# dhruvmetha/rapid-locomotion-rl

Measured on AMD Instinct MI355X. Metric: env-steps/sec, 4096 Mini Cheetah envs, 1/2/4/8 MI355X; PPO iters/sec, higher is better.
Workload: dtype f32; 1 GPU; 4096 Mini Cheetah envs flat terrain (4096 per GPU), PPO teacher policy (BASELINE configs[1]); envs_per_gpu=4096, global_envs=4096, global_batch_env_steps_per_iter=98304, parallelism=dp1, world_size=1, policy=ActorCritic 42/18/630->12, random init; teacher PPO + student adaptation update

## Files before the change

rapid-locomotion-rl_amd/csrc/lrl_gemm.h:

```cpp
#pragma once
#include <stdint.h>

#ifdef __HIPCC__
#define LRL_GHD __host__ __device__
#else
#define LRL_GHD
#endif

namespace lrl {

enum GemmEpi : int {
  EPI_STORE = 0,
  EPI_BIAS = 1,
  EPI_BIAS_ELU = 2,
  EPI_DELU = 3,
  EPI_PARTIAL = 4,
  EPI_BIAS_TANH = 5,
  EPI_DTANH = 6,
};

struct GemmP {
  const float* A;
  const float* B;
  float* C;
  const float* bias;
  const float* aux;
  const int64_t* a_rows;
  const int64_t* b_rows;
  float* bias_part;
  int M, N, K;
  int splits, kps;
  int avec, bvec;
  int groups;
  int64_t lda, ldb, ldc, ld_aux;
  int64_t ga, gb, gc, gbias, gaux;
  int64_t part_stride;
  const uint16_t* bpl;
  int64_t bpl_ld, bpl_ps, gbp;
};

struct PlaneJob {
  const float* W;
  int64_t ldw, gsrc;
  int rows, cols, trans, groups;
  uint16_t* dst;
};
constexpr int MAX_PLANE_JOBS = 8;
LRL_GHD inline int plane_kp(const PlaneJob& j) { return ((j.trans ? j.rows : j.cols) + 15) / 16 * 16; }
LRL_GHD inline int plane_n(const PlaneJob& j) { return j.trans ? j.cols : j.rows; }
LRL_GHD inline int64_t plane_elems(const PlaneJob& j) { return 3ll * j.groups * plane_n(j) * plane_kp(j); }
int x6_planes_launch(const PlaneJob* jobs, int n, void* stream);
bool gemm_x6p_enabled();
inline void gemm_use_planes(GemmP& p, const PlaneJob& j) {
  p.bpl = j.dst;
  p.bpl_ld = plane_kp(j);
  p.gbp = (int64_t)plane_n(j) * plane_kp(j);
  p.bpl_ps = p.gbp * j.groups;
}

enum GemmLayout : int { GEMM_NT = 0, GEMM_NN = 2, GEMM_TN = 3 };

int gemm_launch(const GemmP& p, int layout, int epi, int groups, void* stream);

struct GemmJob {
  GemmP p;
  int layout, epi, groups;
};
constexpr int MAX_MULTI_JOBS = 3;
int gemm_launch_multi(const GemmJob* jobs, int n, void* stream);

enum GemmFamily : int {
  FAM_NONE = 0, FAM_X6P = 1, FAM_X6T = 2, FAM_X6 = 3, FAM_X6D = 4, FAM_GLDS = 5, FAM_GLDS32 = 6, FAM_GLDS_TN = 7,
  FAM_THIN16 = 8, FAM_THIN32 = 9, FAM_STAGED = 10,
};
constexpr int gemm_path_id(int family, int bm, int bn, bool interior) {
  return family | (bm << 8) | (bn << 16) | (interior ? 1 << 24 : 0);
}
int gemm_last_path();

int gemm_pick_splits(int M, int N, int K, int groups);

}
```

rapid-locomotion-rl_amd/csrc/lrl_gemm.hip:

```cpp
#include <hip/hip_runtime.h>
#include <math.h>
#include <stdint.h>

#include <algorithm>
#include <tuple>
#include <type_traits>
#include <cstdio>
#include <cstdlib>

#include "../../include/lrl.h"
#include "lrl_gemm.h"

namespace lrl {

typedef float f32x16 __attribute__((ext_vector_type(16)));

#ifndef LRL_GBK
#define LRL_GBK 16
#endif
constexpr int GBK = LRL_GBK;
constexpr int KQ = GBK / 4;
constexpr int GTHREADS = 256;

static int g_path_off = 0;
static int path_off() { return __atomic_load_n(&g_path_off, __ATOMIC_RELAXED); }
static int env_switch(const char* name, int dflt) {
  const char* e = getenv(name);
  return e && e[0] >= '0' && e[0] <= '9' ? e[0] - '0' : dflt;
}

static thread_local int g_last_path = 0;
static inline void note_path(int family, int bm, int bn, bool interior = false) {
  g_last_path = gemm_path_id(family, bm, bn, interior);
}

template <int BM, int BN, int LAYOUT>
struct GemmTile {
  static constexpr bool AMC = (LAYOUT & 1) != 0;
  static constexpr bool BNC = (LAYOUT & 2) != 0;
  static constexpr int PK = GBK == 32 ? 1 : 2;
  static constexpr int PA = AMC ? 4 : PK;
  static constexpr int PB = BNC ? 4 : PK;
  static constexpr int IA = BM * GBK / 4, IB = BN * GBK / 4;
  static constexpr int NA = (IA + GTHREADS - 1) / GTHREADS;
  static constexpr int NB = (IB + GTHREADS - 1) / GTHREADS;
  static constexpr int WN = (BM >= 64 && BN >= 64) ? 2 : (BM == 32 ? 4 : 1);
  static constexpr int WM = 4 / WN;
  static constexpr int TM = BM / (32 * WM);
  static constexpr int TN = BN / (32 * WN);
  static_assert(TM >= 1 && TN >= 1, "tile shape");
};

static int tn_shape_tag(int M, int N, int groups) {
  if (M == 256 && N == 512) return 1;
  if (M == 128 && N == 256) return groups > 1 ? 2 : 6;
  if (M == 512 && N <= 64) return 3;
  if (M == 256 && N >= 600) return 4;
  if (M == 256 && N <= 64) return 5;
  return 0;
}

__device__ __forceinline__ float elu_f(float x) { return x > 0.f ? x : expm1f(x); }
__device__ __forceinline__ float tanh_f(float x) { return tanhf(x); }
__host__ __device__ constexpr bool epi_bias(int e) { return e == EPI_BIAS || e == EPI_BIAS_ELU || e == EPI_BIAS_TANH; }
__host__ __device__ constexpr bool epi_aux(int e) { return e == EPI_DELU || e == EPI_DTANH; }
template <int EPI>
__device__ __forceinline__ float epi_apply(float v, float bj, float x) {
  if constexpr (EPI == EPI_BIAS) return v + bj;
  else if constexpr (EPI == EPI_BIAS_ELU) return elu_f(v + bj);
  else if constexpr (EPI == EPI_BIAS_TANH) return tanh_f(v + bj);
  else if constexpr (EPI == EPI_DELU) return x > 0.f ? v : v * (x + 1.f);
  else if constexpr (EPI == EPI_DTANH) return v * (1.f - x * x);
  else return v;
}

template <int V>
using Int = std::integral_constant<int, V>;
template <int... V>
struct Ints {};
template <int... V, class F>
static int with_int(int v, Ints<V...>, F&& f) {
  int rc = LRL_E_INVALID;
  (void)((v == V && ((rc = f(Int<V>{})), true)) || ...);
  return rc;
}
template <int LAYOUT, bool STAGED>
struct Offered;
template <bool STAGED>
struct Offered<GEMM_NT, STAGED> { using epis = Ints<EPI_STORE, EPI_BIAS, EPI_BIAS_ELU, EPI_BIAS_TANH>; };
template <>
struct Offered<GEMM_NN, false> { using epis = Ints<EPI_STORE, EPI_DELU, EPI_DTANH>; };
template <>
struct Offered<GEMM_NN, true> { using epis = Ints<EPI_STORE, EPI_DELU, EPI_DTANH, EPI_PARTIAL>; };
template <bool STAGED>
struct Offered<GEMM_TN, STAGED> { using epis = Ints<EPI_PARTIAL>; };
using BatchMajor = Ints<GEMM_NT, GEMM_NN>;
using AnyLayout = Ints<GEMM_NT, GEMM_NN, GEMM_TN>;
template <bool STAGED = false, int... LAYOUTS, class F>
static int with_pair(int layout, int epi, Ints<LAYOUTS...> layouts, F&& f) {
  return with_int(layout, layouts, [&](auto L) {
    return with_int(epi, typename Offered<decltype(L)::value, STAGED>::epis{}, [&](auto E) { return f(L, E); });
  });
}

__device__ __forceinline__ float4 load4(const float* __restrict__ src, int vec) {
  if (vec == 4) return *reinterpret_cast<const float4*>(src);
  if (vec == 2) {
    const float2 a = reinterpret_cast<const float2*>(src)[0], b = reinterpret_cast<const float2*>(src)[1];
    return make_float4(a.x, a.y, b.x, b.y);
  }
  return make_float4(src[0], src[1], src[2], src[3]);
}

template <int R, int NI, bool RCONTIG>
struct Stager {
  static constexpr int ITEMS = R * GBK / 4;
  const float* rowp[NI];
  const float* P;
  const int64_t* rows;
  int64_t ld;
  int vec, r0, R_lim;

  __device__ __forceinline__ void init(const float* P_, int64_t ld_, const int64_t* rows_, int vec_, int r0_,
                                       int R_lim_) {
    P = P_; ld = ld_; rows = rows_; vec = vec_; r0 = r0_; R_lim = R_lim_;
    if (!RCONTIG) {
#pragma unroll
      for (int u = 0; u < NI; ++u) {
        const int i = threadIdx.x + u * GTHREADS;
        const int gr = r0 + i / KQ;
        rowp[u] = nullptr;
        if ((ITEMS % GTHREADS == 0 || i < ITEMS) && gr < R_lim)
          rowp[u] = P + (rows ? rows[gr] : (int64_t)gr) * ld + 4 * (i % KQ);
      }
    }
  }

  __device__ __forceinline__ void load(float4 (&reg)[NI], int k0, int k_lim) const {
#pragma unroll
    for (int u = 0; u < NI; ++u) {
      const int i = threadIdx.x + u * GTHREADS;
      float4 v = make_float4(0.f, 0.f, 0.f, 0.f);
      if (!RCONTIG) {
        const int k = k0 + 4 * (i % KQ);
        if (rowp[u]) {
          const float* src = rowp[u] + k0;
          if (k + 3 < k_lim) {
            v = load4(src, vec);
          } else {
            if (k + 0 < k_lim) v.x = src[0];
            if (k + 1 < k_lim) v.y = src[1];
            if (k + 2 < k_lim) v.z = src[2];
          }
        }
      } else if (ITEMS % GTHREADS == 0 || i < ITEMS) {
        const int r = 4 * (i % (R / 4)), k = k0 + i / (R / 4);
        const int gr = r0 + r;
        if (k < k_lim) {
          const int64_t row = rows ? rows[k] : (int64_t)k;
          const float* src = P + row * ld + gr;
          if (gr + 3 < R_lim) {
            v = load4(src, vec);
          } else {
            if (gr + 0 < R_lim) v.x = src[0];
            if (gr + 1 < R_lim) v.y = src[1];
            if (gr + 2 < R_lim) v.z = src[2];
          }
        }
      }
      reg[u] = v;
    }
  }

  __device__ __forceinline__ void load_fast(float4 (&reg)[NI], int k0) const {
#pragma unroll
    for (int u = 0; u < NI; ++u) {
      const int i = threadIdx.x + u * GTHREADS;
      if (ITEMS % GTHREADS != 0 && i >= ITEMS) continue;
      if (!RCONTIG) {
        reg[u] = *reinterpret_cast<const float4*>(rowp[u] + k0);
      } else {
        const int r = 4 * (i % (R / 4)), k = k0 + i / (R / 4);
        const int64_t row = rows ? rows[k] : (int64_t)k;
        reg[u] = *reinterpret_cast<const float4*>(P + row * ld + r0 + r);
      }
    }
  }
};

template <int R, int PAD, int NI, bool RCONTIG>
__device__ __forceinline__ void stage_store(float (*S)[R + PAD], const float4 (&reg)[NI]) {
  constexpr int ITEMS = R * GBK / 4;
#pragma unroll
  for (int u = 0; u < NI; ++u) {
    const int i = threadIdx.x + u * GTHREADS;
    if (ITEMS % GTHREADS != 0 && i >= ITEMS) {
    } else if (!RCONTIG) {
      const int r = i / KQ, k = 4 * (i % KQ);
      S[k + 0][r] = reg[u].x;
      S[k + 1][r] = reg[u].y;
      S[k + 2][r] = reg[u].z;
      S[k + 3][r] = reg[u].w;
    } else {
      const int r = 4 * (i % (R / 4)), k = i / (R / 4);
      *reinterpret_cast<float4*>(&S[k][r]) = reg[u];
    }
  }
}

template <int BM, int BN, int LAYOUT, int EPI>
__device__ __forceinline__ void gemm_staged_body(const GemmP& p, int vblock, int vgrid, uint8_t* smem) {
  using T = GemmTile<BM, BN, LAYOUT>;
  typedef float AStage[GBK][BM + T::PA];
  typedef float BStage[GBK][BN + T::PB];
  AStage* As = reinterpret_cast<AStage*>(smem);
  BStage* Bs = reinterpret_cast<BStage*>(smem + 2 * sizeof(AStage));
  const int mt = (p.M + BM - 1) / BM, nt = (p.N + BN - 1) / BN;
  int L;
  {
    const int nwg = vgrid, orig = vblock, xcd = orig & 7, q = nwg >> 3, r = nwg & 7;
    L = (xcd < r ? xcd * (q + 1) : r * (q + 1) + (xcd - r) * q) + (orig >> 3);
  }
  const int tn_ = L % nt, tm_ = (L / nt) % mt, zz = L / (nt * mt);
  const int groups = p.groups;
  const int g = zz / p.splits, s = zz - g * p.splits;
  const float* __restrict__ A = p.A + g * p.ga;
  const float* __restrict__ B = p.B + g * p.gb;
  const int m0 = tm_ * BM, n0 = tn_ * BN;
  const int kbeg = s * p.kps;
  const int kend = min(p.K, kbeg + p.kps);
  const int lane = threadIdx.x & 63, w = threadIdx.x >> 6;
  const int li = lane & 31, h = lane >> 5;
  constexpr int TM = T::TM, TN = T::TN;
  const int wm = (w / T::WN) * (BM / T::WM), wn = (w % T::WN) * (BN / T::WN);
  const int64_t* a_rows = T::AMC ? nullptr : p.a_rows;
  const int64_t* b_rows = T::BNC ? p.b_rows : nullptr;

#ifndef LRL_GEMM_SPLITACC
#define LRL_GEMM_SPLITACC 1
#endif
  constexpr int NACC = (LRL_GEMM_SPLITACC && TM * TN == 1) ? 2 : 1;
  f32x16 acc[TM][TN], acc2[TM][TN];
#pragma unroll
  for (int i = 0; i < TM; ++i)
#pragma unroll
    for (int j = 0; j < TN; ++j)
#pragma unroll
      for (int r = 0; r < 16; ++r) acc[i][j][r] = acc2[i][j][r] = 0.f;

  const bool do_bsum = EPI == EPI_PARTIAL && p.bias_part != nullptr && tn_ == 0;
  float bsum = 0.f;

  float4 ra[T::NA], rb[T::NB];
  Stager<BM, T::NA, T::AMC> sa;
  Stager<BN, T::NB, T::BNC> sb;
  sa.init(A, p.lda, a_rows, p.avec, m0, p.M);
  sb.init(B, p.ldb, b_rows, p.bvec, n0, p.N);
  const bool fast = m0 + BM <= p.M && n0 + BN <= p.N && ((kend - kbeg) % GBK) == 0 && p.avec == 4 && p.bvec == 4;
  float xaux[epi_aux(EPI) ? TM : 1][epi_aux(EPI) ? TN : 1][16];
  if constexpr (epi_aux(EPI)) {
    const float* __restrict__ ax = p.aux + g * p.gaux;
#pragma unroll
    for (int j = 0; j < TN; ++j) {
      const int col = min(n0 + wn + 32 * j + li, p.N - 1);
#pragma unroll
      for (int i = 0; i < TM; ++i)
#pragma unroll
        for (int r = 0; r < 16; ++r) {
          const int row = min(m0 + wm + 32 * i + (r & 3) + 8 * (r >> 2) + 4 * h, p.M - 1);
          xaux[i][j][r] = ax[(int64_t)row * p.ld_aux + col];
        }
    }
  }
  int k0 = kbeg;
  if (k0 < kend) {
    if (fast) {
      sa.load_fast(ra, k0);
      sb.load_fast(rb, k0);
    } else {
      sa.load(ra, k0, kend);
      sb.load(rb, k0, kend);
    }
    stage_store<BM, T::PA, T::NA, T::AMC>(As[0], ra);
    stage_store<BN, T::PB, T::NB, T::BNC>(Bs[0], rb);
  }
  __syncthreads();
  int buf = 0;
  for (; k0 < kend; k0 += GBK) {
    const int kn = k0 + GBK;
    if (kn < kend) {
      if (fast) {
        sa.load_fast(ra, kn);
        sb.load_fast(rb, kn);
      } else {
        sa.load(ra, kn, kend);
        sb.load(rb, kn, kend);
      }
    }
    if (do_bsum && threadIdx.x < BM) {
#pragma unroll
      for (int k = 0; k < GBK; ++k) bsum += As[buf][k][threadIdx.x];
    }
    float a[GBK / 2][TM], b[GBK / 2][TN];
#pragma unroll
    for (int kk = 0; kk < GBK / 2; ++kk) {
#pragma unroll
      for (int i = 0; i < TM; ++i) a[kk][i] = As[buf][2 * kk + h][wm + 32 * i + li];
#pragma unroll
      for (int j = 0; j < TN; ++j) b[kk][j] = Bs[buf][2 * kk + h][wn + 32 * j + li];
    }
    __builtin_amdgcn_sched_barrier(0);
    __builtin_amdgcn_s_setprio(1);
#pragma unroll
    for (int kk = 0; kk < GBK / 2; ++kk)
#pragma unroll
      for (int i = 0; i < TM; ++i)
#pragma unroll
        for (int j = 0; j < TN; ++j) {
          if (NACC == 2 && (kk & 1))
            acc2[i][j] = __builtin_amdgcn_mfma_f32_32x32x2f32(a[kk][i], b[kk][j], acc2[i][j], 0, 0, 0);
          else
            acc[i][j] = __builtin_amdgcn_mfma_f32_32x32x2f32(a[kk][i], b[kk][j], acc[i][j], 0, 0, 0);
        }
    __builtin_amdgcn_s_setprio(0);
    __builtin_amdgcn_sched_barrier(0);
    if (kn < kend) {
      stage_store<BM, T::PA, T::NA, T::AMC>(As[buf ^ 1], ra);
      stage_store<BN, T::PB, T::NB, T::BNC>(Bs[buf ^ 1], rb);
    }
    __syncthreads();
    buf ^= 1;
  }

  float* __restrict__ C = p.C + g * p.gc;
  if (EPI == EPI_PARTIAL) C += (int64_t)s * p.part_stride;
  const float* __restrict__ bias = p.bias ? p.bias + g * p.gbias : nullptr;
#pragma unroll
  for (int j = 0; j < TN; ++j) {
    const int col = n0 + wn + 32 * j + li;
    if (col >= p.N) continue;
    float bj = 0.f;
    if (epi_bias(EPI)) bj = bias[col];
#pragma unroll
    for (int i = 0; i < TM; ++i) {
#pragma unroll
      for (int r = 0; r < 16; ++r) {
        const int row = m0 + wm + 32 * i + (r & 3) + 8 * (r >> 2) + 4 * h;
        if (row < p.M) {
          const float v = NACC == 2 ? acc[i][j][r] + acc2[i][j][r] : acc[i][j][r];
          C[(int64_t)row * p.ldc + col] = epi_apply<EPI>(v, bj, epi_aux(EPI) ? xaux[i][j][r] : 0.f);
        }
      }
    }
  }
  if (do_bsum && threadIdx.x < BM && m0 + (int)threadIdx.x < p.M)
    p.bias_part[((int64_t)s * groups + g) * p.M + m0 + threadIdx.x] = bsum;
}
template <int BM, int BN, int LAYOUT, int EPI>
struct StagedBody {
  using T = GemmTile<BM, BN, LAYOUT>;
  static constexpr int LDS = 2 * GBK * (BM + T::PA + BN + T::PB) * (int)sizeof(float);
  static_assert((2 * GBK * (BM + T::PA) * sizeof(float)) % 16 == 0, "B stages 16-B aligned");
  static __device__ __forceinline__ void run(const GemmP& p, int vblock, int vgrid, uint8_t* smem) {
    gemm_staged_body<BM, BN, LAYOUT, EPI>(p, vblock, vgrid, smem);
  }
};
template <int BM, int BN, int LAYOUT, int EPI>
__global__ __launch_bounds__(GTHREADS) void gemm_kernel(GemmP p) {
  using Body = StagedBody<BM, BN, LAYOUT, EPI>;
  __shared__ __attribute__((aligned(16))) uint8_t S[Body::LDS];
  Body::run(p, blockIdx.x, gridDim.x, S);
}

typedef __attribute__((address_space(3))) void* lds_ptr_t;

template <int LAYOUT, int EPI, int BKD>
__global__ __launch_bounds__(GTHREADS) void gemm_glds_kernel(GemmP p) {
// ... 170 lines not shown
#pragma unroll
      for (int s = 0; s < 16; ++s) {
        const float av = (s & 3) == 0 ? cur[s >> 2].x : (s & 3) == 1 ? cur[s >> 2].y : (s & 3) == 2 ? cur[s >> 2].z : cur[s >> 2].w;
        if (s & 1) acc2 = __builtin_amdgcn_mfma_f32_32x32x2f32(av, breg[kb][s], acc2, 0, 0, 0);
        else acc = __builtin_amdgcn_mfma_f32_32x32x2f32(av, breg[kb][s], acc, 0, 0, 0);
      }
#pragma unroll
      for (int v = 0; v < 4; ++v) cur[v] = nxt[v];
    }
    ar = arn;
    if (w > 0) {
#pragma unroll
      for (int r = 0; r < 16; ++r) red[((w - 1) * 16 + r) * 64 + lane] = acc[r] + acc2[r];
    }
    __syncthreads();
    if (w == 0) {
      float bj = 0.f;
      if constexpr (epi_bias(EPI)) bj = colv ? p.bias[g * p.gbias + li] : 0.f;
#pragma unroll
      for (int r = 0; r < 16; ++r) {
        float v = acc[r] + acc2[r];
        v += red[r * 64 + lane];
        v += red[(16 + r) * 64 + lane];
        v += red[(32 + r) * 64 + lane];
        v = epi_apply<EPI>(v, bj, 0.f);
        const int orow = t * 32 + (r & 3) + 8 * (r >> 2) + 4 * h;
        if (colv && orow < M) C[(int64_t)orow * p.ldc + li] = v;
      }
    }
    __syncthreads();
  }
}

typedef float f32x4v __attribute__((ext_vector_type(4)));
template <int LAYOUT, int EPI, int NBK>
__global__ __launch_bounds__(GTHREADS, 2) void gemm_thin16_kernel(GemmP p) {
  __shared__ float red[3 * 8 * 64];
  constexpr bool BNC = (LAYOUT & 2) != 0;
  constexpr int KS = 2 * NBK;
  const int N = p.N, M = p.M;
  const int g = blockIdx.y;
  const float* __restrict__ A = p.A + g * p.ga;
  const float* __restrict__ B = p.B + g * p.gb;
  float* __restrict__ C = p.C + g * p.gc;
  const int lane = threadIdx.x & 63, w = threadIdx.x >> 6, i = lane & 15, h = lane >> 4;
  const int kbeg = w * 32 * NBK;
  float breg[KS][2][4];
#pragma unroll
  for (int s = 0; s < KS; ++s)
#pragma unroll
    for (int cb = 0; cb < 2; ++cb)
#pragma unroll
      for (int u = 0; u < 4; ++u) {
        const int k = kbeg + 16 * s + 4 * h + u, col = i + 16 * cb;
        breg[s][cb][u] = col < N ? (BNC ? B[(int64_t)k * p.ldb + col] : B[(int64_t)col * p.ldb + k]) : 0.f;
      }
  const int mt = (M + 15) >> 4;
  auto rowp = [&](int t) -> const float* {
    const int row = t * 16 + i;
    if (t >= mt || row >= M) return nullptr;
    return A + (p.a_rows ? p.a_rows[row] : (int64_t)row) * p.lda + kbeg + 4 * h;
  };
  auto load = [&](const float* ar, int s0, float4* dst) {
#pragma unroll
    for (int v = 0; v < 4; ++v)
      dst[v] = ar ? *reinterpret_cast<const float4*>(ar + 16 * (s0 + v)) : make_float4(0.f, 0.f, 0.f, 0.f);
  };
  const float* ar = rowp(blockIdx.x);
  float4 cur[4];
  load(ar, 0, cur);
  for (int t = blockIdx.x; t < mt; t += gridDim.x) {
    const float* arn = rowp(t + gridDim.x);
    f32x4v acc0 = {0.f, 0.f, 0.f, 0.f}, acc1 = {0.f, 0.f, 0.f, 0.f};
#pragma unroll
    for (int s0 = 0; s0 < KS; s0 += 4) {
      float4 nxt[4];
      if (s0 + 4 < KS) load(ar, s0 + 4, nxt);
      else load(arn, 0, nxt);
#pragma unroll
      for (int v = 0; v < 4; ++v) {
        const float av[4] = {cur[v].x, cur[v].y, cur[v].z, cur[v].w};
#pragma unroll
        for (int u = 0; u < 4; ++u) {
          acc0 = __builtin_amdgcn_mfma_f32_16x16x4f32(av[u], breg[s0 + v][0][u], acc0, 0, 0, 0);
          acc1 = __builtin_amdgcn_mfma_f32_16x16x4f32(av[u], breg[s0 + v][1][u], acc1, 0, 0, 0);
        }
      }
#pragma unroll
      for (int v = 0; v < 4; ++v) cur[v] = nxt[v];
    }
    ar = arn;
    if (w > 0) {
#pragma unroll
      for (int r = 0; r < 4; ++r) {
        red[((w - 1) * 8 + r) * 64 + lane] = acc0[r];
        red[((w - 1) * 8 + 4 + r) * 64 + lane] = acc1[r];
      }
    }
    __syncthreads();
    if (w == 0) {
#pragma unroll
      for (int cb = 0; cb < 2; ++cb) {
        const int col = i + 16 * cb;
        float bj = 0.f;
        if constexpr (epi_bias(EPI)) bj = col < N ? p.bias[g * p.gbias + col] : 0.f;
#pragma unroll
        for (int r = 0; r < 4; ++r) {
          float v = cb ? acc1[r] : acc0[r];
          v += red[(4 * cb + r) * 64 + lane];
          v += red[(8 + 4 * cb + r) * 64 + lane];
          v += red[(16 + 4 * cb + r) * 64 + lane];
          v = epi_apply<EPI>(v, bj, 0.f);
          const int orow = t * 16 + 4 * h + r;
          if (col < N && orow < M) C[(int64_t)orow * p.ldc + col] = v;
        }
      }
    }
    __syncthreads();
  }
}

static bool thin16_enabled() {
  static const int on = env_switch("LRL_THIN16", 1);
  return on != 0 && !(path_off() & 32);
}

template <int LAYOUT, int EPI, int NBK>
static int launch_thin_k(const GemmP& p, int groups, hipStream_t st) {
  static int ncu = 0;
  if (!ncu) {
    int dev = 0;
    hipDeviceProp_t prop;
    if (hipGetDevice(&dev) != hipSuccess || hipGetDeviceProperties(&prop, dev) != hipSuccess) return LRL_E_HIP;
    ncu = prop.multiProcessorCount;
  }
  if (thin16_enabled()) {
    const int mt = (p.M + 15) / 16;
    const int gx = std::max(1, std::min(mt, 2 * ncu / std::max(1, groups)));
    hipLaunchKernelGGL((gemm_thin16_kernel<LAYOUT, EPI, NBK>), dim3(gx, groups), dim3(GTHREADS), 0, st, p);
    note_path(FAM_THIN16, 16, 32);
    return 0;
  }
  const int mt = (p.M + 31) / 32;
  const int gx = std::max(1, std::min(mt, 2 * ncu / std::max(1, groups)));
  hipLaunchKernelGGL((gemm_thin_kernel<LAYOUT, EPI, NBK>), dim3(gx, groups), dim3(GTHREADS), 0, st, p);
  note_path(FAM_THIN32, 32, 32);
  return 0;
}
template <int LAYOUT, int EPI>
static int launch_thin(const GemmP& p, int groups, hipStream_t st) {
  switch (p.K / 128) {
    case 4: return launch_thin_k<LAYOUT, EPI, 4>(p, groups, st);
    case 8: return launch_thin_k<LAYOUT, EPI, 8>(p, groups, st);
  }
  return LRL_E_INVALID;
}

template <int NST, int BN, int SHAPE>
__global__ __launch_bounds__(GTHREADS, 2) void gemm_glds_tn_kernel(GemmP p) {
  constexpr int BM = 128, BKD = 16, IMGA = BKD * BM, IMGB = BKD * BN, TN = BN / 64;
  constexpr int NB_DMA = IMGB / 256;
  extern __shared__ __attribute__((aligned(16))) float S[];
  const int mt = p.M / BM, nt = (p.N + BN - 1) / BN;
  int L;
  {
    const int nwg = gridDim.x, orig = blockIdx.x, xcd = orig & 7, q = nwg >> 3, r = nwg & 7;
    L = (xcd < r ? xcd * (q + 1) : r * (q + 1) + (xcd - r) * q) + (orig >> 3);
  }
  const int tn_ = L % nt, tm_ = (L / nt) % mt, zz = L / (nt * mt);
  const int g = zz / p.splits, sp = zz - g * p.splits;
  const int m0 = tm_ * BM, n0 = tn_ * BN;
  const int kbeg = sp * p.kps, kend = min(p.K, kbeg + p.kps);
  const int ns = (kend - kbeg) / BKD;
  const float* __restrict__ A = p.A + g * p.ga;
  const float* __restrict__ B = p.B + g * p.gb;
  const int lane = threadIdx.x & 63;
  const int w = __builtin_amdgcn_readfirstlane(threadIdx.x >> 6);
  const int li = lane & 31, h = lane >> 5;
  const int wm = (w >> 1) * 64, wn = (w & 1) * (BN / 2);
  constexpr int STG = IMGA + IMGB;
  int* rows = reinterpret_cast<int*>(S + NST * STG);
  if (p.b_rows) {
    for (int i = threadIdx.x; i < kend - kbeg; i += GTHREADS) rows[i] = (int)p.b_rows[kbeg + i];
    __syncthreads();
  }
  const uint32_t s_lds = (uint32_t)(uintptr_t)(lds_ptr_t)S;
  auto dma = [&](const float* src, uint32_t lds_off) {
    uint32_t keep;
    asm volatile("s_mov_b32 %0, m0\n\ts_mov_b32 m0, %2\n\ts_nop 0\n\tglobal_load_lds_dwordx4 %1, off\n\ts_mov_b32 m0, %0"
                 : "=&s"(keep)
                 : "v"(src), "s"(lds_off)
                 : "memory");
  };
  auto issue = [&](int st, int s) {
    const int kl = s * BKD;
    const uint32_t sbase = s_lds + (uint32_t)(st * STG * 4);
#pragma unroll
    for (int i = 0; i < 2; ++i) {
      const int d = 4 * i + w, kr = kl + 2 * d + h;
      dma(A + (int64_t)(kbeg + kr) * p.lda + m0 + 4 * li, __builtin_amdgcn_readfirstlane(sbase + d * 1024));
    }
#pragma unroll
    for (int i = 0; i < NB_DMA / 4; ++i) {
      constexpr int CPR = BN / 4;
      const int d = 4 * i + w, kr = kl + d * (64 / CPR) + lane / CPR;
      const int64_t brow = p.b_rows ? (int64_t)rows[kr] : (int64_t)(kbeg + kr);
      dma(B + brow * p.ldb + n0 + 4 * (lane % CPR), __builtin_amdgcn_readfirstlane(sbase + IMGA * 4 + d * 1024));
    }
  };
  const bool do_bsum = p.bias_part != nullptr && tn_ == 0;
  float bsum = 0.f;
  f32x16 acc[2][TN];
#pragma unroll
  for (int a = 0; a < 2; ++a)
#pragma unroll
    for (int c = 0; c < TN; ++c)
#pragma unroll
      for (int r = 0; r < 16; ++r) acc[a][c][r] = 0.f;
  static_assert(NST == 3, "the counted waits below assume a 3-deep ring");
  if (ns > 0) issue(0, 0);
  if (ns > 1) issue(1, 1);
  for (int s = 0; s < ns; ++s) {
    if (s + 1 < ns) {
      if constexpr (NB_DMA == 8) asm volatile("s_waitcnt vmcnt(4)" ::: "memory");
      else asm volatile("s_waitcnt vmcnt(3)" ::: "memory");
    } else {
      asm volatile("s_waitcnt vmcnt(0)" ::: "memory");
    }
    __builtin_amdgcn_s_barrier();
    if (s + 2 < ns) issue((s + 2) % NST, s + 2);
    const float* As = S + (s % NST) * STG;
    const float* Bs = As + IMGA;
    if (do_bsum && threadIdx.x < BM) {
#pragma unroll
      for (int k = 0; k < BKD; ++k) bsum += As[k * BM + threadIdx.x];
    }
    float av[8][2], bv[8][TN];
#pragma unroll
    for (int t = 0; t < 8; ++t) {
#pragma unroll
      for (int a = 0; a < 2; ++a) av[t][a] = As[(2 * t + h) * BM + wm + 32 * a + li];
#pragma unroll
      for (int c = 0; c < TN; ++c) bv[t][c] = Bs[(2 * t + h) * BN + wn + 32 * c + li];
    }
    asm volatile("s_waitcnt lgkmcnt(0)" ::: "memory");
    __builtin_amdgcn_sched_barrier(0);
    __builtin_amdgcn_s_setprio(1);
#pragma unroll
    for (int t = 0; t < 8; ++t)
#pragma unroll
      for (int a = 0; a < 2; ++a)
#pragma unroll
        for (int c = 0; c < TN; ++c)
          acc[a][c] = __builtin_amdgcn_mfma_f32_32x32x2f32(av[t][a], bv[t][c], acc[a][c], 0, 0, 0);
    __builtin_amdgcn_s_setprio(0);
    __builtin_amdgcn_sched_barrier(0);
  }
  float* __restrict__ C = p.C + g * p.gc + (int64_t)sp * p.part_stride;
#pragma unroll
  for (int c = 0; c < TN; ++c) {
    const int col = n0 + wn + 32 * c + li;
    if (col >= p.N) continue;
#pragma unroll
    for (int a = 0; a < 2; ++a)
#pragma unroll
      for (int r = 0; r < 16; ++r) {
        const int row = m0 + wm + 32 * a + (r & 3) + 8 * (r >> 2) + 4 * h;
        C[(int64_t)row * p.ldc + col] = acc[a][c][r];
      }
  }
  if (do_bsum && threadIdx.x < BM)
    p.bias_part[((int64_t)sp * p.groups + g) * p.M + m0 + threadIdx.x] = bsum;
}

template <int BN, int SHAPE>
static int launch_glds_tn_tag(const GemmP& p, int groups, hipStream_t st) {
  const size_t lds = (size_t)3 * 16 * (128 + BN) * sizeof(float) + (p.b_rows ? (size_t)p.kps * sizeof(int) : 0);
  static bool attr = false;
  if (!attr) {
    if (hipFuncSetAttribute(reinterpret_cast<const void*>(&gemm_glds_tn_kernel<3, BN, SHAPE>),
                            hipFuncAttributeMaxDynamicSharedMemorySize, 160 * 1024) != hipSuccess)
      return LRL_E_HIP;
    attr = true;
  }
  dim3 gt((p.M / 128) * ((p.N + BN - 1) / BN) * groups * p.splits);
  hipLaunchKernelGGL((gemm_glds_tn_kernel<3, BN, SHAPE>), gt, dim3(GTHREADS), lds, st, p);
  note_path(FAM_GLDS_TN, 128, BN);
  return hipGetLastError() == hipSuccess ? 0 : LRL_E_HIP;
}

template <int BN>
static int launch_glds_tn(const GemmP& p, int groups, hipStream_t st) {
  switch (tn_shape_tag(p.M, p.N, groups)) {
    case 1: return launch_glds_tn_tag<BN, 1>(p, groups, st);
    case 2: return launch_glds_tn_tag<BN, 2>(p, groups, st);
    case 3: return launch_glds_tn_tag<BN, 3>(p, groups, st);
    case 4: return launch_glds_tn_tag<BN, 4>(p, groups, st);
    case 5: return launch_glds_tn_tag<BN, 5>(p, groups, st);
    case 6: return launch_glds_tn_tag<BN, 6>(p, groups, st);
    default: return launch_glds_tn_tag<BN, 0>(p, groups, st);
  }
}

constexpr int XBK = 16;
#ifndef LRL_X6_PIPE
#define LRL_X6_PIPE 1
#endif
#ifndef LRL_X6_PIPE_VALU
#define LRL_X6_PIPE_VALU 4
#endif

__device__ __forceinline__ uint32_t x6_hi_pair(uint32_t u0, uint32_t u1) {
  return __builtin_amdgcn_perm(u1, u0, 0x07060302u);
}
__device__ __forceinline__ void x6_split2(float x0, float x1, uint32_t& h, uint32_t& m, uint32_t& l) {
  uint32_t u0 = __float_as_uint(x0), u1 = __float_as_uint(x1);
  h = x6_hi_pair(u0, u1);
  float r0 = x0 - __uint_as_float(u0 & 0xffff0000u), r1 = x1 - __uint_as_float(u1 & 0xffff0000u);
  u0 = __float_as_uint(r0);
  u1 = __float_as_uint(r1);
  m = x6_hi_pair(u0, u1);
  r0 = r0 - __uint_as_float(u0 & 0xffff0000u);
  r1 = r1 - __uint_as_float(u1 & 0xffff0000u);
  l = x6_hi_pair(__float_as_uint(r0), __float_as_uint(r1));
}
__device__ __forceinline__ int x6_off(int r, int c) { return r * XBK + 8 * (c ^ ((r >> 3) & 1)); }

typedef short bf16x8_t __attribute__((ext_vector_type(8)));

__device__ __forceinline__ f32x16 x6_mma(const bf16x8_t (&a)[3], const bf16x8_t (&b)[3], f32x16 c) {
  c = __builtin_amdgcn_mfma_f32_32x32x16_bf16(a[2], b[0], c, 0, 0, 0);
  c = __builtin_amdgcn_mfma_f32_32x32x16_bf16(a[1], b[1], c, 0, 0, 0);
  c = __builtin_amdgcn_mfma_f32_32x32x16_bf16(a[0], b[2], c, 0, 0, 0);
  c = __builtin_amdgcn_mfma_f32_32x32x16_bf16(a[1], b[0], c, 0, 0, 0);
  c = __builtin_amdgcn_mfma_f32_32x32x16_bf16(a[0], b[1], c, 0, 0, 0);
  c = __builtin_amdgcn_mfma_f32_32x32x16_bf16(a[0], b[0], c, 0, 0, 0);
  return c;
}

template <int R, bool KC, bool KGATHER = false>
struct X6Op {
  static constexpr int PLANE = R * XBK;
  static constexpr int NI = KC ? R / 64 : 1;
  static constexpr int KR = KC ? 4 : R / 16;
  static constexpr int NV = KC ? 4 * NI : KR;
  const float* rowp[NI];
  const float* P;
  const int64_t* krows;
  int64_t ld;
  int ldi, roff;
  int rr, kb;
  bool rok;
  bool vec4;

  __device__ __forceinline__ void init(const float* P_, int64_t ld_, const int64_t* rows, const int64_t* krows_,
                                       int r0, int R_lim, bool vec4_ = true) {
    P = P_; ld = ld_; krows = krows_; vec4 = vec4_;
    const int t = threadIdx.x;
    if (KC) {
#pragma unroll
      for (int u = 0; u < NI; ++u) {
        const int r = (t >> 2) + 64 * u, gr = r0 + r;
        rowp[u] = gr < R_lim ? P_ + (rows ? rows[gr] : (int64_t)gr) * ld_ + 4 * (t & 3) : nullptr;
      }
    } else {
      rr = t % R;
      kb = __builtin_amdgcn_readfirstlane(KR * (t / R));
      rok = r0 + rr < R_lim;
      ldi = (int)ld_;
      roff = r0 + rr;
    }
  }
  __device__ __forceinline__ void load(float (&v)[NV], int k0, int k_lim, bool fast) const {
    if (KC) {
#pragma unroll
      for (int u = 0; u < NI; ++u) {
        const int k = k0 + 4 * (threadIdx.x & 3);
        float4 q = make_float4(0.f, 0.f, 0.f, 0.f);
        if (fast) {
          q = *reinterpret_cast<const float4*>(rowp[u] + k0);
        } else if (rowp[u]) {
          const float* s = rowp[u] + k0;
          if (k + 3 < k_lim && vec4) {
            q = *reinterpret_cast<const float4*>(s);
          } else if (k + 3 < k_lim) {
            q = make_float4(s[0], s[1], s[2], s[3]);
          } else {
            if (k + 0 < k_lim) q.x = s[0];
            if (k + 1 < k_lim) q.y = s[1];
            if (k + 2 < k_lim) q.z = s[2];
          }
        }
        v[4 * u] = q.x; v[4 * u + 1] = q.y; v[4 * u + 2] = q.z; v[4 * u + 3] = q.w;
      }
    } else {
#pragma unroll
      for (int e = 0; e < KR; ++e) {
        const int k = k0 + kb + e;
        if constexpr (KGATHER) {
          const int64_t o = krows[k] * ld + roff;
          if (fast) v[e] = P[o];
          else v[e] = (rok && k < k_lim) ? P[o] : 0.f;
        } else if (fast) {
          v[e] = P[k * ldi + roff];
        } else {
          v[e] = (rok && k < k_lim) ? P[k * ldi + roff] : 0.f;
        }
      }
    }
  }
  __device__ __forceinline__ void store(const float (&v)[NV], uint16_t* img) const {
    const int t = threadIdx.x;
    if (KC) {
#pragma unroll
      for (int u = 0; u < NI; ++u) {
        const int r = (t >> 2) + 64 * u, j = t & 3;
        uint32_t h0, m0, l0, h1, m1, l1;
        x6_split2(v[4 * u], v[4 * u + 1], h0, m0, l0);
        x6_split2(v[4 * u + 2], v[4 * u + 3], h1, m1, l1);
        const int off = x6_off(r, j >> 1) + 4 * (j & 1);
        *reinterpret_cast<uint2*>(img + off) = make_uint2(h0, h1);
        *reinterpret_cast<uint2*>(img + PLANE + off) = make_uint2(m0, m1);
        *reinterpret_cast<uint2*>(img + 2 * PLANE + off) = make_uint2(l0, l1);
      }
    } else if (KR == 8) {
      uint32_t h[4], m[4], l[4];
#pragma unroll
      for (int e = 0; e < 4; ++e) x6_split2(v[2 * e], v[2 * e + 1], h[e], m[e], l[e]);
      const int off = x6_off(rr, kb >> 3);
      *reinterpret_cast<uint4*>(img + off) = make_uint4(h[0], h[1], h[2], h[3]);
      *reinterpret_cast<uint4*>(img + PLANE + off) = make_uint4(m[0], m[1], m[2], m[3]);
      *reinterpret_cast<uint4*>(img + 2 * PLANE + off) = make_uint4(l[0], l[1], l[2], l[3]);
    } else {
      uint32_t h[2], m[2], l[2];
#pragma unroll
      for (int e = 0; e < 2; ++e) x6_split2(v[2 * e], v[2 * e + 1], h[e], m[e], l[e]);
      const int off = x6_off(rr, kb >> 3) + (kb & 4);
      *reinterpret_cast<uint2*>(img + off) = make_uint2(h[0], h[1]);
      *reinterpret_cast<uint2*>(img + PLANE + off) = make_uint2(m[0], m[1]);
      *reinterpret_cast<uint2*>(img + 2 * PLANE + off) = make_uint2(l[0], l[1]);
    }
  }
  __device__ __forceinline__ static float vsum(const float (&v)[NV]) {
    float s = 0.f;
#pragma unroll
    for (int e = 0; e < NV; ++e) s += v[e];
    return s;
  }
};

template <int BM, int BN, int LAYOUT, int EPI, bool FAST, bool BGATHER>
__device__ __forceinline__ void gemm_x6_body(const GemmP& p, int vblock, int vgrid, uint8_t* smem) {
  constexpr bool AKC = (LAYOUT & 1) == 0, BKC = (LAYOUT & 2) == 0;
  constexpr int PA = BM * XBK, PB = BN * XBK, STG = 3 * (PA + PB);
  constexpr int TM = BM / 64, TN = BN / 64;
  uint16_t* S = reinterpret_cast<uint16_t*>(smem);
  const int mt = (p.M + BM - 1) / BM, nt = (p.N + BN - 1) / BN;
  int L;
  {
    const int nwg = vgrid, orig = vblock, xcd = orig & 7, q = nwg >> 3, r = nwg & 7;
    L = (xcd < r ? xcd * (q + 1) : r * (q + 1) + (xcd - r) * q) + (orig >> 3);
  }
  const int tn_ = L % nt, tm_ = (L / nt) % mt, zz = L / (nt * mt);
  const int g = zz / p.splits, sp = zz - g * p.splits;
  const int m0 = tm_ * BM, n0 = tn_ * BN;
  const int kbeg = sp * p.kps, kend = min(p.K, kbeg + p.kps);
  const int lane = threadIdx.x & 63, w = threadIdx.x >> 6, li = lane & 31, h = lane >> 5;
  const int wm = (w >> 1) * (BM / 2), wn = (w & 1) * (BN / 2);
  X6Op<BM, AKC> oa;
  X6Op<BN, BKC, BGATHER && !BKC> ob;
  oa.init(p.A + g * p.ga, p.lda, AKC ? p.a_rows : nullptr, nullptr, m0, p.M, p.avec == 4);
  ob.init(p.B + g * p.gb, p.ldb, nullptr, BKC ? nullptr : p.b_rows, n0, p.N, p.bvec == 4);
  constexpr bool fast = FAST;
  const bool do_bsum = EPI == EPI_PARTIAL && p.bias_part != nullptr && tn_ == 0;
  float bsum = 0.f;
  f32x16 acc[TM][TN];
#pragma unroll
  for (int i = 0; i < TM; ++i)
#pragma unroll
    for (int j = 0; j < TN; ++j)
#pragma unroll
      for (int r = 0; r < 16; ++r) acc[i][j][r] = 0.f;
  using OA = decltype(oa);
  using OB = decltype(ob);
  auto compute = [&](const uint16_t* As) {
    const uint16_t* Bs = As + 3 * PA;
    bf16x8_t a[TM][3], b[TN][3];
#pragma unroll
    for (int i = 0; i < TM; ++i)
#pragma unroll
      for (int pl = 0; pl < 3; ++pl)
        a[i][pl] = *reinterpret_cast<const bf16x8_t*>(As + pl * PA + x6_off(wm + 32 * i + li, h));
#pragma unroll
    for (int j = 0; j < TN; ++j)
#pragma unroll
      for (int pl = 0; pl < 3; ++pl)
        b[j][pl] = *reinterpret_cast<const bf16x8_t*>(Bs + pl * PB + x6_off(wn + 32 * j + li, h));
#pragma unroll
    for (int i = 0; i < TM; ++i)
#pragma unroll
      for (int j = 0; j < TN; ++j) acc[i][j] = x6_mma(a[i], b[j], acc[i][j]);
  };
  if constexpr (LRL_X6_PIPE && FAST) {
  float va[2][OA::NV], vb[2][OB::NV];
  const int ns = (kend - kbeg + XBK - 1) / XBK;
  if (ns > 0) {
    oa.load(va[0], kbeg, kend, fast);
    ob.load(vb[0], kbeg, kend, fast);
    if (ns > 1) {
      oa.load(va[1], kbeg + XBK, kend, fast);
      ob.load(vb[1], kbeg + XBK, kend, fast);
    }
    if (do_bsum) bsum += OA::vsum(va[0]);
    oa.store(va[0], S);
    ob.store(vb[0], S + 3 * PA);
    if (ns > 2) {
      oa.load(va[0], kbeg + 2 * XBK, kend, fast);
      ob.load(vb[0], kbeg + 2 * XBK, kend, fast);
    }
  }
  __syncthreads();
  auto step = [&](int s, auto par, auto full) {
    constexpr int P = decltype(par)::value;
    constexpr bool F = decltype(full)::value;
    compute(S + P * STG);
    if (F || s + 1 < ns) {
      if (do_bsum) bsum += OA::vsum(va[P ^ 1]);
      oa.store(va[P ^ 1], S + (P ^ 1) * STG);
      ob.store(vb[P ^ 1], S + (P ^ 1) * STG + 3 * PA);
    }
    if (F || s + 3 < ns) {
      oa.load(va[P ^ 1], kbeg + (s + 3) * XBK, kend, fast);
      ob.load(vb[P ^ 1], kbeg + (s + 3) * XBK, kend, fast);
    }
    if constexpr (F) {
      constexpr int NMF = TM * TN * 6;
      __builtin_amdgcn_sched_group_barrier(0x100, 3 * (TM + TN), 0);
#pragma unroll
      for (int q = 0; q < NMF; ++q) {
        __builtin_amdgcn_sched_group_barrier(0x008, 1, 0);
        __builtin_amdgcn_sched_group_barrier(0x002, LRL_X6_PIPE_VALU, 0);
      }
    }
    __syncthreads();
  };
  using I0 = std::integral_constant<int, 0>;
  using I1 = std::integral_constant<int, 1>;
  using BT = std::integral_constant<bool, true>;
  using BF = std::integral_constant<bool, false>;
  int s = 0;
  for (; s + 4 < ns; s += 2) {
    step(s, I0{}, BT{});
    step(s + 1, I1{}, BT{});
  }
  for (; s < ns; s += 2) {
    step(s, I0{}, BF{});
    if (s + 1 < ns) step(s + 1, I1{}, BF{});
  }
  } else {
  float va[OA::NV], vb[OB::NV];
  if (kbeg < kend) {
    oa.load(va, kbeg, kend, fast);
    ob.load(vb, kbeg, kend, fast);
    if (do_bsum) bsum += OA::vsum(va);
    oa.store(va, S);
    ob.store(vb, S + 3 * PA);
  }
  __syncthreads();
  int buf = 0;
  for (int k0 = kbeg; k0 < kend; k0 += XBK) {
    const bool more = k0 + XBK < kend;
    if (more) {
      oa.load(va, k0 + XBK, kend, fast);
      ob.load(vb, k0 + XBK, kend, fast);
    }
    compute(S + buf * STG);
    if (more) {
      if (do_bsum) bsum += OA::vsum(va);
      oa.store(va, S + (buf ^ 1) * STG);
      ob.store(vb, S + (buf ^ 1) * STG + 3 * PA);
    }
    __syncthreads();
    buf ^= 1;
  }
  }

  float* __restrict__ C = p.C + g * p.gc;
  if (EPI == EPI_PARTIAL) C += (int64_t)sp * p.part_stride;
  const float* __restrict__ bias = p.bias ? p.bias + g * p.gbias : nullptr;
  const float* __restrict__ ax = epi_aux(EPI) ? p.aux + g * p.gaux : nullptr;
#pragma unroll
  for (int j = 0; j < TN; ++j) {
    const int col = n0 + wn + 32 * j + li;
    if (!FAST && col >= p.N) continue;
    float bj = 0.f;
    if (epi_bias(EPI)) bj = bias[col];
#pragma unroll
    for (int i = 0; i < TM; ++i)
#pragma unroll
      for (int q = 0; q < 4; ++q) {
        const int row0 = m0 + wm + 32 * i + 8 * q + 4 * h;
        const int ldc = (int)p.ldc, ldx = (int)p.ld_aux;
        float* __restrict__ crow = C + (int64_t)row0 * p.ldc + col;
        float xa[4];
        if constexpr (epi_aux(EPI)) {
          const float* __restrict__ xrow = ax + (int64_t)row0 * p.ld_aux + col;
#pragma unroll
          for (int r = 0; r < 4; ++r) xa[r] = (FAST || row0 + r < p.M) ? xrow[r * ldx] : 0.f;
        }
#pragma unroll
        for (int r = 0; r < 4; ++r) {
          if (FAST || row0 + r < p.M) crow[r * ldc] = epi_apply<EPI>(acc[i][j][4 * q + r], bj, epi_aux(EPI) ? xa[r] : 0.f);
        }
        asm volatile("" ::: "memory");
      }
  }
  if constexpr (EPI == EPI_PARTIAL && !AKC) {
    if (do_bsum) {
      float* red = reinterpret_cast<float*>(S);
      red[threadIdx.x] = bsum;
      __syncthreads();
      if (threadIdx.x < BM && m0 + (int)threadIdx.x < p.M) {
        float s = 0.f;
#pragma unroll
        for (int q = 0; q < GTHREADS / BM; ++q) s += red[q * BM + threadIdx.x];
        p.bias_part[((int64_t)sp * p.groups + g) * p.M + m0 + threadIdx.x] = s;
      }
    }
  }
}
template <int BM, int BN, int LAYOUT, int EPI, bool FAST, bool BGATHER>
struct X6Body {
  static constexpr int LDS = 2 * 3 * (BM + BN) * XBK * (int)sizeof(uint16_t);
  static __device__ __forceinline__ void run(const GemmP& p, int vblock, int vgrid, uint8_t* smem) {
    gemm_x6_body<BM, BN, LAYOUT, EPI, FAST, BGATHER>(p, vblock, vgrid, smem);
  }
};
template <int BM, int BN, int LAYOUT, int EPI, bool FAST, bool BGATHER, int TAG = 0>
__global__ __launch_bounds__(GTHREADS, 3) void gemm_x6_kernel(GemmP p) {
  using Body = X6Body<BM, BN, LAYOUT, EPI, FAST, BGATHER>;
  __shared__ __attribute__((aligned(16))) uint8_t S[Body::LDS];
  Body::run(p, blockIdx.x, gridDim.x, S);
}

static bool x6_interior(const GemmP& p, int layout, int bm, int bn) {
  const bool akc = (layout & 1) == 0, bkc = (layout & 2) == 0;
  return p.M % bm == 0 && p.N % bn == 0 && p.K % XBK == 0 && p.kps % XBK == 0 && (!akc || p.avec == 4) &&
         (!bkc || p.bvec == 4);
}
template <int BM, int BN>
static int launch_x6_tile(const GemmP& p, int layout, int epi, int groups, hipStream_t st) {
  dim3 grid(((p.M + BM - 1) / BM) * ((p.N + BN - 1) / BN) * groups * p.splits);
  const bool interior = x6_interior(p, layout, BM, BN);
  const bool bg = p.b_rows != nullptr;
  if (layout == GEMM_TN) {
    auto tn = [&](auto F, auto G, auto T) {
      hipLaunchKernelGGL((gemm_x6_kernel<BM, BN, GEMM_TN, EPI_PARTIAL, F(), G(), T()>), grid, dim3(GTHREADS), 0, st, p);
    };
    const std::true_type yes;
    const std::false_type no;
    const int tag = (BM == 128 && BN == 128 && interior) ? tn_shape_tag(p.M, p.N, groups) : 0;
    if (tag == 1) tn(yes, no, Int<1>{});
    else if (tag == 2) tn(yes, no, Int<2>{});
    else if (tag == 4 && bg) tn(yes, yes, Int<4>{});
    else if (tag == 4) tn(yes, no, Int<4>{});
    else if (tag == 6) tn(yes, no, Int<6>{});
    else if (interior && bg) tn(yes, yes, Int<0>{});
    else if (interior) tn(yes, no, Int<0>{});
    else if (bg) tn(no, yes, Int<0>{});
    else tn(no, no, Int<0>{});
  } else {
    const int rc = with_pair(layout, epi, BatchMajor{}, [&](auto L, auto E) {
      if (interior) hipLaunchKernelGGL((gemm_x6_kernel<BM, BN, L(), E(), true, false>), grid, dim3(GTHREADS), 0, st, p);
      else hipLaunchKernelGGL((gemm_x6_kernel<BM, BN, L(), E(), false, false>), grid, dim3(GTHREADS), 0, st, p);
      return 0;
    });
    if (rc) return rc;
  }
  note_path(FAM_X6, BM, BN, interior);
  return hipGetLastError() == hipSuccess ? 0 : LRL_E_HIP;
}

static bool x6_enabled() {
  static const int on = env_switch("LRL_GEMM_X6", 1);
  return on != 0 && !(path_off() & 16);
}

static int try_x6d(const GemmP& p, int layout, int epi, int groups, int bm, int bn, hipStream_t st);
static bool x6d_fits(const GemmP& p, int layout, int bm, int bn);

static bool x6_tile(const GemmP& p, int layout, int epi, int groups, int& bm, int& bn) {
  if (!x6_enabled()) return false;
  static const int min_side = getenv("LRL_X6_MIN") ? atoi(getenv("LRL_X6_MIN")) : 16;
  if (p.N < min_side || (layout == GEMM_TN && p.M < min_side)) return false;
  const int64_t lim = int64_t(1) << 31;
  if ((layout & 1) && (int64_t)p.K * p.lda >= lim) return false;
  if ((layout & 2) && p.b_rows == nullptr && (int64_t)p.K * p.ldb >= lim) return false;
  if ((int64_t)p.M * p.ldc >= lim || (epi_aux(epi) && (int64_t)p.M * p.ld_aux >= lim)) return false;
  if (layout == GEMM_TN) {
    if (epi != EPI_PARTIAL || p.M < 16 || p.N < 16 || p.kps % XBK) return false;
    bm = p.M <= 64 ? 64 : 128;
    bn = p.N <= 64 ? 64 : 128;
    return true;
  }
  if (p.splits != 1 || p.N < 16 || p.M < 64 || epi == EPI_PARTIAL) return false;
  if (p.K < 32) return false;
  if (p.N <= 32 && p.K % 128 == 0 && (p.K / 128 == 4 || p.K / 128 == 8) && p.avec == 4 && p.M >= 256) return false;
  static const int small_wg = getenv("LRL_X6_SMALL_WG") ? atoi(getenv("LRL_X6_SMALL_WG")) : 1024;
  bn = p.N > 64 ? 128 : 64;
  if (bn == 128 && (int64_t)((p.M + 63) / 64) * ((p.N + 127) / 128) * groups < small_wg) bn = 64;
  const int64_t wg128 = (int64_t)((p.M + 127) / 128) * ((p.N + bn - 1) / bn) * groups;
  bm = wg128 >= 512 ? 128 : 64;
  return true;
}

static int try_x6(const GemmP& p, int layout, int epi, int groups, hipStream_t st) {
  int bm, bn;
  if (!x6_tile(p, layout, epi, groups, bm, bn)) return 0;
  if (int dr = try_x6d(p, layout, epi, groups, bm, bn, st)) return dr;
  int rc;
  if (bm == 128 && bn == 128) rc = launch_x6_tile<128, 128>(p, layout, epi, groups, st);
  else if (bm == 128) rc = launch_x6_tile<128, 64>(p, layout, epi, groups, st);
  else if (bn == 128) rc = launch_x6_tile<64, 128>(p, layout, epi, groups, st);
  else rc = launch_x6_tile<64, 64>(p, layout, epi, groups, st);
  return rc ? rc : 1;
}

template <int BM, int EPI, bool GATHER>
__global__ __launch_bounds__(GTHREADS, 2) void gemm_x6p_kernel(GemmP p) {
  constexpr int BN = 128, NST = 3, TM = BM / 64, TN = 2;
  constexpr int AIMG = BM * 64, BIMG = BN * 32, STB = AIMG + 3 * BIMG;
  constexpr int NA = BM / 64, NB = 3;
  constexpr int NPW = NA + NB;
  static_assert(NPW == 4 || NPW == 5, "vmcnt table");
  __shared__ __attribute__((aligned(16))) uint8_t S[NST * STB];
  const int mt = p.M / BM, nt = p.N / BN;
  int L;
  {
    const int nwg = gridDim.x, orig = blockIdx.x, xcd = orig & 7, q = nwg >> 3, r = nwg & 7;
    L = (xcd < r ? xcd * (q + 1) : r * (q + 1) + (xcd - r) * q) + (orig >> 3);
  }
  const int tn_ = L % nt, tm_ = (L / nt) % mt, g = L / (nt * mt);
  const int m0 = tm_ * BM, n0 = tn_ * BN;
  const int lane = threadIdx.x & 63;
  const int w = __builtin_amdgcn_readfirstlane(threadIdx.x >> 6);
  const int li = lane & 31, h = lane >> 5;
  const int wm = (w >> 1) * (BM / 2), wn = (w & 1) * (BN / 2);
  const float* __restrict__ A = p.A + g * p.ga;
  const uint16_t* __restrict__ Bp = p.bpl + g * p.gbp;
  const float* asrc[NA];
#pragma unroll
  for (int d = 0; d < NA; ++d) {
    const int r = (w * NA + d) * 16 + (lane >> 2), ch = (lane & 3) ^ ((r >> 2) & 3);
    asrc[d] = A + (GATHER ? p.a_rows[m0 + r] : (int64_t)(m0 + r)) * p.lda + 4 * ch;
  }
  const uint16_t* bsrc[NB];
#pragma unroll
  for (int d = 0; d < NB; ++d) {
    const int j = w * NB + d, r = (j & 3) * 32 + (lane >> 1), ch = (lane & 1) ^ ((r >> 3) & 1);
    bsrc[d] = Bp + (j >> 2) * p.bpl_ps + (int64_t)(n0 + r) * p.bpl_ld + 8 * ch;
  }
  const uint32_t s_lds = (uint32_t)(uintptr_t)(lds_ptr_t)S;
  auto dma = [&](const void* src, uint32_t lds_off) {
    uint32_t keep;
    asm volatile("s_mov_b32 %0, m0\n\ts_mov_b32 m0, %2\n\ts_nop 0\n\tglobal_load_lds_dwordx4 %1, off\n\ts_mov_b32 m0, %0"
                 : "=&s"(keep)
                 : "v"(src), "s"(lds_off)
                 : "memory");
  };
  auto issue = [&](int st, int k0) {
    const uint32_t base = s_lds + (uint32_t)(st * STB);
#pragma unroll
    for (int d = 0; d < NA; ++d) dma(asrc[d] + k0, __builtin_amdgcn_readfirstlane(base + (w * NA + d) * 1024));
#pragma unroll
    for (int d = 0; d < NB; ++d) dma(bsrc[d] + k0, __builtin_amdgcn_readfirstlane(base + AIMG + (w * NB + d) * 1024));
  };

  f32x16 acc[TM][TN];
#pragma unroll
  for (int i = 0; i < TM; ++i)
#pragma unroll
    for (int j = 0; j < TN; ++j)
#pragma unroll
      for (int r = 0; r < 16; ++r) acc[i][j][r] = 0.f;

  const int ns = p.K / 16;
  issue(0, 0);
  if (ns > 1) issue(1, 16);
  for (int s = 0; s < ns; ++s) {
    if (s + 1 < ns) {
      if constexpr (NPW == 5) asm volatile("s_waitcnt vmcnt(5)" ::: "memory");
      else asm volatile("s_waitcnt vmcnt(4)" ::: "memory");
    } else {
      asm volatile("s_waitcnt vmcnt(0)" ::: "memory");
    }
    __builtin_amdgcn_s_barrier();
    if (s + 2 < ns) issue((s + 2) % NST, (s + 2) * 16);
    const uint8_t* As = S + (s % NST) * STB;
    const uint8_t* Bs = As + AIMG;
    bf16x8_t a[TM][3], b[TN][3];
#pragma unroll
    for (int j = 0; j < TN; ++j) {
      const int r = wn + 32 * j + li, off = r * 32 + 16 * (h ^ ((r >> 3) & 1));
#pragma unroll
      for (int pl = 0; pl < 3; ++pl) b[j][pl] = *reinterpret_cast<const bf16x8_t*>(Bs + pl * BIMG + off);
    }
#pragma unroll
    for (int i = 0; i < TM; ++i) {
      const int r = wm + 32 * i + li, sw = (r >> 2) & 3;
      const float4 x0 = *reinterpret_cast<const float4*>(As + r * 64 + 16 * ((2 * h) ^ sw));
      const float4 x1 = *reinterpret_cast<const float4*>(As + r * 64 + 16 * ((2 * h + 1) ^ sw));
      uint32_t hh[4], mm[4], ll[4];
      x6_split2(x0.x, x0.y, hh[0], mm[0], ll[0]);
      x6_split2(x0.z, x0.w, hh[1], mm[1], ll[1]);
      x6_split2(x1.x, x1.y, hh[2], mm[2], ll[2]);
      x6_split2(x1.z, x1.w, hh[3], mm[3], ll[3]);
      uint4 vh = make_uint4(hh[0], hh[1], hh[2], hh[3]), vm = make_uint4(mm[0], mm[1], mm[2], mm[3]),
            vl = make_uint4(ll[0], ll[1], ll[2], ll[3]);
      a[i][0] = *reinterpret_cast<bf16x8_t*>(&vh);
      a[i][1] = *reinterpret_cast<bf16x8_t*>(&vm);
      a[i][2] = *reinterpret_cast<bf16x8_t*>(&vl);
    }
#pragma unroll
    for (int i = 0; i < TM; ++i)
#pragma unroll
      for (int j = 0; j < TN; ++j) acc[i][j] = x6_mma(a[i], b[j], acc[i][j]);
  }

  float* __restrict__ C = p.C + g * p.gc;
  const float* __restrict__ bias = p.bias ? p.bias + g * p.gbias : nullptr;
  const float* __restrict__ ax = epi_aux(EPI) ? p.aux + g * p.gaux : nullptr;
#pragma unroll
  for (int j = 0; j < TN; ++j) {
    const int col = n0 + wn + 32 * j + li;
    float bj = 0.f;
    if (epi_bias(EPI)) bj = bias[col];
#pragma unroll
    for (int i = 0; i < TM; ++i)
#pragma unroll
      for (int q = 0; q < 4; ++q) {
        const int row0 = m0 + wm + 32 * i + 8 * q + 4 * h;
        float* __restrict__ crow = C + (int64_t)row0 * p.ldc + col;
        float xa[4];
        if constexpr (epi_aux(EPI)) {
          const float* __restrict__ xrow = ax + (int64_t)row0 * p.ld_aux + col;
#pragma unroll
          for (int r = 0; r < 4; ++r) xa[r] = xrow[r * p.ld_aux];
        }
#pragma unroll
        for (int r = 0; r < 4; ++r) crow[r * p.ldc] = epi_apply<EPI>(acc[i][j][4 * q + r], bj, epi_aux(EPI) ? xa[r] : 0.f);
      }
  }
}

constexpr int X6T_MAX_GATHER_KPS = 1024;
template <int BN, bool BGATHER>
__device__ __forceinline__ void gemm_x6t_body(const GemmP& p, int vblock, int vgrid, uint8_t* S) {
  constexpr int BM = 128, NST = 3, TM = 2, TN = BN / 64;
  constexpr int IMG = 16 * 128 * 4, STB = IMG + 16 * BN * 4;
  constexpr int NAP = IMG / 1024, NBP = BN / 16;
  constexpr int NPW = (NAP + NBP) / 4;
  constexpr int KPP = 256 / BN;
  const int mt = p.M / BM, nt = (p.N + BN - 1) / BN;
  int L;
  {
    const int nwg = vgrid, orig = vblock, xcd = orig & 7, q = nwg >> 3, r = nwg & 7;
    L = (xcd < r ? xcd * (q + 1) : r * (q + 1) + (xcd - r) * q) + (orig >> 3);
  }
  const int tn_ = L % nt, tm_ = (L / nt) % mt, zz = L / (nt * mt);
  const int g = zz / p.splits, sp = zz - g * p.splits;
  const int m0 = tm_ * BM, n0 = tn_ * BN;
  const int kbeg = sp * p.kps, kend = min(p.K, kbeg + p.kps);
  const int lane = threadIdx.x & 63;
  const int w = __builtin_amdgcn_readfirstlane(threadIdx.x >> 6);
  const int li = lane & 31, h = lane >> 5;
  const int wm = (w >> 1) * (BM / 2), wn = (w & 1) * (BN / 2);
  const float* __restrict__ A = p.A + g * p.ga;
  const float* __restrict__ Bm = p.B + g * p.gb;
  const float* src[NPW];
  int64_t kstep[NPW];
  int bkr[NPW];
  int* xrows = reinterpret_cast<int*>(S + NST * STB);
  if constexpr (BGATHER) {
    for (int t = threadIdx.x; t < kend - kbeg; t += GTHREADS) xrows[t] = (int)p.b_rows[kbeg + t];
    __syncthreads();
  }
#pragma unroll
  for (int d = 0; d < NPW; ++d) {
    const int j = NPW * w + d;
    if (j < NAP) {
      const int kr = 2 * j + (lane >> 5), ch = (lane & 31) ^ (8 * ((kr >> 3) & 1));
      src[d] = A + (int64_t)(kbeg + kr) * p.lda + m0 + 4 * ch;
      kstep[d] = (int64_t)16 * p.lda;
      bkr[d] = -1;
    } else {
      const int kr = KPP * (j - NAP) + lane / (BN / 4), ch = (lane % (BN / 4)) ^ (8 * ((kr >> 3) & 1));
      src[d] = BGATHER ? Bm + n0 + 4 * ch : Bm + (int64_t)(kbeg + kr) * p.ldb + n0 + 4 * ch;
      kstep[d] = (int64_t)16 * p.ldb;
      bkr[d] = kr;
    }
  }
  const uint32_t s_lds = (uint32_t)(uintptr_t)(lds_ptr_t)S;
  auto dma = [&](const void* src, uint32_t lds_off) {
    uint32_t keep;
    asm volatile("s_mov_b32 %0, m0\n\ts_mov_b32 m0, %2\n\ts_nop 0\n\tglobal_load_lds_dwordx4 %1, off\n\ts_mov_b32 m0, %0"
                 : "=&s"(keep)
                 : "v"(src), "s"(lds_off)
                 : "memory");
  };
  auto issue = [&](int st, int s) {
    const uint32_t base = s_lds + (uint32_t)(st * STB);
#pragma unroll
    for (int d = 0; d < NPW; ++d) {
      const float* sr = (BGATHER && bkr[d] >= 0) ? src[d] + (int64_t)xrows[16 * s + bkr[d]] * p.ldb : src[d] + s * kstep[d];
      dma(sr, __builtin_amdgcn_readfirstlane(base + (NPW * w + d) * 1024));
    }
  };
  const bool do_bsum = p.bias_part != nullptr && tn_ == 0 && wn == 0;
  float bsum[TM] = {0.f, 0.f};
  f32x16 acc[TM][TN];
#pragma unroll
  for (int i = 0; i < TM; ++i)
#pragma unroll
    for (int j = 0; j < TN; ++j)
#pragma unroll
      for (int r = 0; r < 16; ++r) acc[i][j][r] = 0.f;

  const int ns = (kend - kbeg) / 16;
  if (ns > 0) issue(0, 0);
  if (ns > 1) issue(1, 1);
  const int sw = 32 * h;
  static_assert(NPW == 3 || NPW == 4, "vmcnt below");
  for (int s = 0; s < ns; ++s) {
    if (s + 1 < ns) {
      if constexpr (NPW == 4) asm volatile("s_waitcnt vmcnt(4)" ::: "memory");
      else asm volatile("s_waitcnt vmcnt(3)" ::: "memory");
    } else {
      asm volatile("s_waitcnt vmcnt(0)" ::: "memory");
    }
    __builtin_amdgcn_s_barrier();
    if (s + 2 < ns) issue((s + 2) % NST, s + 2);
    const float* As = reinterpret_cast<const float*>(S + (s % NST) * STB);
    const float* Bs = As + IMG / 4;
    bf16x8_t a[TM][3], b[TN][3];
    auto gather_split = [&](const float* img, int pitch, int r, bf16x8_t (&o)[3], float* vs) {
      const float* p0 = img + 8 * h * pitch + (r ^ sw);
      float v[8];
#pragma unroll
      for (int t = 0; t < 8; ++t) v[t] = p0[pitch * t];
      if (vs) {
        float s8 = 0.f;
#pragma unroll
        for (int t = 0; t < 8; ++t) s8 += v[t];
        *vs += s8;
      }
      uint32_t hh[4], mm[4], ll[4];
#pragma unroll
      for (int e = 0; e < 4; ++e) x6_split2(v[2 * e], v[2 * e + 1], hh[e], mm[e], ll[e]);
      uint4 vh = make_uint4(hh[0], hh[1], hh[2], hh[3]), vm = make_uint4(mm[0], mm[1], mm[2], mm[3]),
            vl = make_uint4(ll[0], ll[1], ll[2], ll[3]);
      o[0] = *reinterpret_cast<bf16x8_t*>(&vh);
      o[1] = *reinterpret_cast<bf16x8_t*>(&vm);
      o[2] = *reinterpret_cast<bf16x8_t*>(&vl);
    };
#pragma unroll
    for (int i = 0; i < TM; ++i) gather_split(As, 128, wm + 32 * i + li, a[i], do_bsum ? &bsum[i] : nullptr);
#pragma unroll
    for (int j = 0; j < TN; ++j) gather_split(Bs, BN, wn + 32 * j + li, b[j], nullptr);
#pragma unroll
    for (int i = 0; i < TM; ++i)
#pragma unroll
      for (int j = 0; j < TN; ++j) acc[i][j] = x6_mma(a[i], b[j], acc[i][j]);
  }

  float* __restrict__ C = p.C + g * p.gc + (int64_t)sp * p.part_stride;
#pragma unroll
  for (int j = 0; j < TN; ++j) {
    const int col = n0 + wn + 32 * j + li;
    if (col >= p.N) continue;
#pragma unroll
    for (int i = 0; i < TM; ++i)
#pragma unroll
      for (int q = 0; q < 4; ++q) {
        const int row0 = m0 + wm + 32 * i + 8 * q + 4 * h;
        float* __restrict__ crow = C + (int64_t)row0 * p.ldc + col;
#pragma unroll
        for (int r = 0; r < 4; ++r) crow[r * p.ldc] = acc[i][j][4 * q + r];
      }
  }
  if (p.bias_part != nullptr && tn_ == 0) {
    __syncthreads();
    float* red = reinterpret_cast<float*>(S);
    if (wn == 0) {
#pragma unroll
      for (int i = 0; i < TM; ++i) red[h * BM + wm + 32 * i + li] = bsum[i];
    }
    __syncthreads();
    if (threadIdx.x < BM) {
      float s = 0.f;
      s += red[threadIdx.x];
      s += red[BM + threadIdx.x];
      p.bias_part[((int64_t)sp * p.groups + g) * p.M + m0 + threadIdx.x] = s;
    }
  }
}
template <int BN, bool BGATHER>
struct X6tBody {
  static constexpr int LDS = 3 * (16 * 128 * 4 + 16 * BN * 4) + (BGATHER ? 4 * X6T_MAX_GATHER_KPS : 0);
// ... 565 lines not shown
```

rapid-locomotion-rl_amd/csrc/lrl_ppo.hip:

```cpp
#include <hip/hip_runtime.h>
#include <math.h>
#include <stdint.h>
#include <stdlib.h>
#include <string.h>

#include <algorithm>
#include <initializer_list>
#include <mutex>
#include <vector>

#include "../../include/lrl.h"
#include "../../include/lrl_philox.h"
#include "lrl_gemm.h"
#include "lrl_launch.h"

namespace lrl {

constexpr float LOG_SQRT_2PI = 0.91893853320467274178f;
constexpr int HEAD_ROWS = 32;
constexpr int HEAD_THREADS = 256;
constexpr int HEAD_W = 128;
constexpr int MAX_ACT = 16;
constexpr int HEAD_NA = 12;
constexpr int MAX_LAT = 32;

__device__ __forceinline__ float delu(float h) { return h > 0.f ? 1.f : h + 1.f; }

constexpr int PREP_R = 4;
__global__ void ppo_prep_kernel(const float* __restrict__ obs, const int64_t* __restrict__ rows, int B, int no,
                                int xs, float* __restrict__ X) {
  const int64_t i = (int64_t)blockIdx.x * blockDim.x + threadIdx.x;
  const int64_t ng = ((int64_t)B + PREP_R - 1) / PREP_R;
  if (i >= ng * xs) return;
  const int g = (int)(i / xs), c = (int)(i - (int64_t)g * xs);
  int64_t src[PREP_R];
  float v[PREP_R];
#pragma unroll
  for (int u = 0; u < PREP_R; ++u) {
    const int b = g * PREP_R + u;
    src[u] = b < B ? (rows ? rows[b] : (int64_t)b) : -1;
  }
#pragma unroll
  for (int u = 0; u < PREP_R; ++u) v[u] = (c < no && src[u] >= 0) ? obs[src[u] * no + c] : 0.f;
#pragma unroll
  for (int u = 0; u < PREP_R; ++u) {
    const int b = g * PREP_R + u;
    if (b < B) X[(int64_t)b * xs + c] = v[u];
  }
}

inline unsigned prep_blocks(int64_t rows, int xs) {
  return (unsigned)((((rows + PREP_R - 1) / PREP_R) * xs + 255) / 256);
}

struct HeadArgs {
  const float* h3;
  float* dh3;
  const float *w4a, *b4a, *w4c, *b4c, *stdv;
  const float *actions, *old_mu, *old_sigma, *tv, *ret, *adv, *old_logp;
  const int64_t* rows;
  int B, na;
  float clip, ent_coef, vcoef;
  int clipped_value;
  float* part;
  int part_len;
};

__host__ __device__ constexpr int hp_w4a(int) { return 0; }
__host__ __device__ constexpr int hp_b4a(int na) { return na * HEAD_W; }
__host__ __device__ constexpr int hp_w4c(int na) { return na * HEAD_W + na; }
__host__ __device__ constexpr int hp_b4c(int na) { return na * HEAD_W + na + HEAD_W; }
__host__ __device__ constexpr int hp_std(int na) { return na * HEAD_W + na + HEAD_W + 1; }
__host__ __device__ constexpr int hp_kl(int na) { return na * HEAD_W + na + HEAD_W + 1 + na; }
__host__ __device__ constexpr int hp_len(int na) { return hp_kl(na) + 3; }

template <int NA, bool TANH>
__global__ __launch_bounds__(HEAD_THREADS) void ppo_head_kernel(HeadArgs a) {
  constexpr int HP = 2 * HEAD_W + 4;
  constexpr int NAP = (NA + 3) / 4 * 4;
  static_assert(NA <= 16 && HEAD_W % 16 == 0, "float4 rows");
  constexpr int NG = (HEAD_ROWS * NA + HEAD_THREADS - 1) / HEAD_THREADS;
  __shared__ __attribute__((aligned(16))) float H[HEAD_ROWS][HP];
  __shared__ __attribute__((aligned(16))) float W4[NA + 1][HEAD_W];
  __shared__ float MU[HEAD_ROWS][NA + 1];
  __shared__ float VP[HEAD_ROWS][8];
  __shared__ __attribute__((aligned(16))) float LP[HEAD_ROWS][NAP];
  __shared__ float KT[HEAD_ROWS][NA];
  __shared__ float DR[HEAD_ROWS][2];
  __shared__ float SC[HEAD_ROWS][3];
  __shared__ float SD[3][NA];
  __shared__ float GA[3][HEAD_ROWS][NA];
  __shared__ float GR[4][HEAD_ROWS];
  __shared__ int64_t RW[HEAD_ROWS];
  const int t = threadIdx.x;
  const int r0 = blockIdx.x * HEAD_ROWS;
  const int nrows = min(HEAD_ROWS, a.B - r0);
  if (t < HEAD_ROWS) RW[t] = t < nrows ? a.rows[r0 + t] : a.rows[r0];
  if (t < NA) {
    const float sd = a.stdv[t];
    SD[0][t] = sd;
    SD[1][t] = logf(sd);
    SD[2][t] = 1.f / (sd * sd);
  }
  {
    constexpr int NV = HEAD_ROWS * 2 * HEAD_W / 4 / HEAD_THREADS;
    float4 v[NV];
#pragma unroll
    for (int u = 0; u < NV; ++u) {
      const int i = t + u * HEAD_THREADS, r = i / (HEAD_W / 2), c = 4 * (i % (HEAD_W / 2));
      v[u] = r < nrows ? *reinterpret_cast<const float4*>(a.h3 + (int64_t)(r0 + r) * (2 * HEAD_W) + c)
                       : make_float4(0.f, 0.f, 0.f, 0.f);
    }
#pragma unroll
    for (int u = 0; u < NV; ++u) {
      const int i = t + u * HEAD_THREADS, r = i / (HEAD_W / 2), c = 4 * (i % (HEAD_W / 2));
      *reinterpret_cast<float4*>(&H[r][c]) = v[u];
    }
  }
  for (int i = t; i < (NA + 1) * HEAD_W; i += HEAD_THREADS) {
    const int j = i / HEAD_W, k = i - j * HEAD_W;
    W4[j][k] = j < NA ? a.w4a[j * HEAD_W + k] : a.w4c[k];
  }
  __syncthreads();
  float ga[3][NG], gr = 0.f;
#pragma unroll
  for (int u = 0; u < NG; ++u) {
    const int i = t + u * HEAD_THREADS;
    const int r = i / NA, j = i - r * NA;
    const bool ok = i < HEAD_ROWS * NA;
    const int64_t o = RW[ok ? r : 0] * NA + j;
    ga[0][u] = ok ? a.actions[o] : 0.f;
    ga[1][u] = ok ? a.old_mu[o] : 0.f;
    ga[2][u] = ok ? a.old_sigma[o] : 1.f;
  }
  if (t < 4 * HEAD_ROWS) {
    const int q = t / HEAD_ROWS, r = t - q * HEAD_ROWS;
    const float* src = q == 0 ? a.adv : q == 1 ? a.old_logp : q == 2 ? a.tv : a.ret;
    gr = src[RW[r]];
  }
  {
    const int r = t & (HEAD_ROWS - 1), q = t / HEAD_ROWS;
    const float4* hr = reinterpret_cast<const float4*>(&H[r][0]);
    auto dot4 = [](float s, float4 h, float4 w) {
      s = fmaf(h.x, w.x, s);
      s = fmaf(h.y, w.y, s);
      s = fmaf(h.z, w.z, s);
      return fmaf(h.w, w.w, s);
    };
    for (int j = q; j < NA; j += 8) {
      const float4* wr = reinterpret_cast<const float4*>(&W4[j][0]);
      float s = 0.f;
#pragma unroll 8
      for (int k4 = 0; k4 < HEAD_W / 4; ++k4) s = dot4(s, hr[k4], wr[k4]);
      MU[r][j] = s + a.b4a[j];
    }
    const float4* wv = reinterpret_cast<const float4*>(&W4[NA][q * (HEAD_W / 8)]);
    const float4* hv = hr + (HEAD_W + q * (HEAD_W / 8)) / 4;
    float s = 0.f;
#pragma unroll
    for (int k4 = 0; k4 < HEAD_W / 32; ++k4) s = dot4(s, hv[k4], wv[k4]);
    VP[r][q] = s;
  }
#pragma unroll
  for (int u = 0; u < NG; ++u) {
    const int i = t + u * HEAD_THREADS;
    if (i < HEAD_ROWS * NA) {
      const int r = i / NA, j = i - r * NA;
      GA[0][r][j] = ga[0][u];
      GA[1][r][j] = ga[1][u];
      GA[2][r][j] = ga[2][u];
    }
  }
  if (t < 4 * HEAD_ROWS) GR[t / HEAD_ROWS][t & (HEAD_ROWS - 1)] = gr;
  __syncthreads();
  for (int i = t; i < HEAD_ROWS * NA; i += HEAD_THREADS) {
    const int r = i / NA, j = i - r * NA;
    float lp = 0.f, kt = 0.f, d = 0.f;
    if (r < nrows) {
      const float s = SD[0][j], mu = MU[r][j];
      d = GA[0][r][j] - mu;
      lp = -(d * d) / (2.f * (s * s)) - SD[1][j] - LOG_SQRT_2PI;
      const float so = GA[2][r][j], dm = GA[1][r][j] - mu;
      kt = logf(s / so + 1.e-5f) + (so * so + dm * dm) / (2.f * (s * s)) - 0.5f;
    }
    MU[r][j] = d;
    LP[r][j] = lp;
    KT[r][j] = kt;
  }
  __syncthreads();
  const float invB = 1.f / (float)a.B;
  if (t < HEAD_ROWS) {
    const int r = t;
    float kl = 0.f, surr_loss = 0.f, vloss = 0.f, dv = 0.f, dlogp = 0.f;
    if (r < nrows) {
      const float v = (((VP[r][0] + VP[r][1]) + (VP[r][2] + VP[r][3])) + ((VP[r][4] + VP[r][5]) + (VP[r][6] + VP[r][7]))) +
                      a.b4c[0];
      float logp = 0.f;
#pragma unroll
      for (int j = 0; j < NA; ++j) {
        logp += LP[r][j];
        kl += KT[r][j];
      }
      const float adv = GR[0][r];
      const float ratio = expf(logp - GR[1][r]);
      const float surr = -adv * ratio;
      const float rc = fminf(fmaxf(ratio, 1.f - a.clip), 1.f + a.clip);
      const float surr_c = -adv * rc;
      surr_loss = fmaxf(surr, surr_c);
      const float ga = surr > surr_c ? invB : (surr == surr_c ? 0.5f * invB : 0.f);
      const float gb = surr_c > surr ? invB : (surr == surr_c ? 0.5f * invB : 0.f);
      const bool in_rng = ratio >= 1.f - a.clip && ratio <= 1.f + a.clip;
      const float dratio = -adv * ga + (in_rng ? -adv * gb : 0.f);
      dlogp = dratio * ratio;
      const float tv = GR[2][r], ret = GR[3][r];
      const float gv = a.vcoef * invB;
      if (a.clipped_value) {
        const float dvt = v - tv;
        const float vc = tv + fminf(fmaxf(dvt, -a.clip), a.clip);
        const float l1 = (v - ret) * (v - ret), l2 = (vc - ret) * (vc - ret);
        vloss = fmaxf(l1, l2);
        const float g1 = l1 > l2 ? gv : (l1 == l2 ? 0.5f * gv : 0.f);
        const float g2 = l2 > l1 ? gv : (l1 == l2 ? 0.5f * gv : 0.f);
        const bool vin = dvt >= -a.clip && dvt <= a.clip;
        dv = g1 * 2.f * (v - ret) + (vin ? g2 * 2.f * (vc - ret) : 0.f);
      } else {
        vloss = (ret - v) * (ret - v);
        dv = gv * 2.f * (v - ret);
      }
    }
    DR[r][0] = dlogp;
    DR[r][1] = dv;
    SC[r][0] = kl;
    SC[r][1] = surr_loss;
    SC[r][2] = vloss;
  }
  __syncthreads();
  for (int i = t; i < HEAD_ROWS * NA; i += HEAD_THREADS) {
    const int r = i / NA, j = i - r * NA;
    float dm = 0.f, ds = 0.f;
    if (r < nrows) {
      const float d = MU[r][j], dl = DR[r][0], s = SD[0][j], ivar = SD[2][j];
      dm = dl * (d * ivar);
      ds = dl * (d * d * ivar - 1.f) / s - a.ent_coef * invB / s;
    }
    LP[r][j] = dm;
    KT[r][j] = ds;
  }
  __syncthreads();
  float* P = a.part + (int64_t)blockIdx.x * a.part_len;
  {
    const int k = t;
    if (k < HEAD_W) {
      float wk[NA], accw[NA];
#pragma unroll
      for (int j = 0; j < NA; ++j) {
        wk[j] = W4[j][k];
        accw[j] = 0.f;
      }
#pragma unroll 2
      for (int r = 0; r < nrows; ++r) {
        const float h = H[r][k];
        float dmr[NAP];
#pragma unroll
        for (int j4 = 0; j4 < NAP / 4; ++j4) {
          const float4 v = reinterpret_cast<const float4*>(&LP[r][0])[j4];
          dmr[4 * j4] = v.x; dmr[4 * j4 + 1] = v.y; dmr[4 * j4 + 2] = v.z; dmr[4 * j4 + 3] = v.w;
        }
        float s = 0.f;
#pragma unroll
        for (int j = 0; j < NA; ++j) {
          const float dm = dmr[j];
          s = fmaf(dm, wk[j], s);
          accw[j] = fmaf(dm, h, accw[j]);
        }
        a.dh3[(int64_t)(r0 + r) * (2 * HEAD_W) + k] = s * (TANH ? 1.f - h * h : delu(h));
      }
#pragma unroll
      for (int j = 0; j < NA; ++j) P[hp_w4a(NA) + j * HEAD_W + k] = accw[j];
    } else {
      const int kk = k - HEAD_W;
      const float wk = W4[NA][kk];
      float accc = 0.f;
      for (int r = 0; r < nrows; ++r) {
        const float h = H[r][k];
        const float d = DR[r][1];
        accc = fmaf(d, h, accc);
        a.dh3[(int64_t)(r0 + r) * (2 * HEAD_W) + k] = (d * wk) * (TANH ? 1.f - h * h : delu(h));
      }
      P[hp_w4c(NA) + kk] = accc;
    }
  }
  if (t < NA) {
    float sb = 0.f, ss = 0.f;
    for (int r = 0; r < nrows; ++r) {
      sb += LP[r][t];
      ss += KT[r][t];
    }
    P[hp_b4a(NA) + t] = sb;
    P[hp_std(NA) + t] = ss;
  } else if (t == 16) {
    float sb = 0.f;
    for (int r = 0; r < nrows; ++r) sb += DR[r][1];
    P[hp_b4c(NA)] = sb;
  } else if (t >= 32 && t < 35) {
    const int c = t - 32;
    float s = 0.f;
    for (int r = 0; r < nrows; ++r) s += SC[r][c];
    P[hp_kl(NA) + c] = s;
  }
}

struct ActHeadArgs {
  const float* h3;
  const float *w4a, *b4a, *w4c, *b4c, *stdv;
  const float *obs, *priv, *hist, *eps;
  int n, na, no, np;
  uint64_t seed, counter;
  int64_t row_offset;
  float *actions, *mu, *values, *logp;
  lrl_rollout_store store;
  int store_row, do_store;
  float* xa_out;
};

__device__ __forceinline__ void copy_rows(const float* __restrict__ src, int64_t sld, float* __restrict__ dst,
                                          int64_t dld, int nrows, int cols, int t) {
  if (((((uintptr_t)src | (uintptr_t)dst) & 7) == 0) && (((sld | dld | cols) & 1) == 0)) {
    const int c2 = cols / 2, n = nrows * c2;
    for (int i0 = t; i0 < n; i0 += 8 * HEAD_THREADS) {
      float2 v[8];
#pragma unroll
      for (int u = 0; u < 8; ++u) {
        const int i = i0 + u * HEAD_THREADS, r = i / c2, c = i - r * c2;
        if (i < n) v[u] = reinterpret_cast<const float2*>(src + r * sld)[c];
      }
#pragma unroll
      for (int u = 0; u < 8; ++u) {
        const int i = i0 + u * HEAD_THREADS, r = i / c2, c = i - r * c2;
        if (i < n) reinterpret_cast<float2*>(dst + r * dld)[c] = v[u];
      }
    }
  } else {
    const int n = nrows * cols;
    for (int i0 = t; i0 < n; i0 += 8 * HEAD_THREADS) {
      float v[8];
#pragma unroll
      for (int u = 0; u < 8; ++u) {
        const int i = i0 + u * HEAD_THREADS, r = i / cols, c = i - r * cols;
        if (i < n) v[u] = src[r * sld + c];
      }
#pragma unroll
      for (int u = 0; u < 8; ++u) {
        const int i = i0 + u * HEAD_THREADS, r = i / cols, c = i - r * cols;
        if (i < n) dst[r * dld + c] = v[u];
      }
    }
  }
}

constexpr int ACT_ROWS = 16, ACT_Q = HEAD_THREADS / ACT_ROWS;
__global__ __launch_bounds__(HEAD_THREADS) void act_head_kernel(ActHeadArgs a) {
  constexpr int HP = 2 * HEAD_W + 1;
  __shared__ float H[ACT_ROWS][HP];
  __shared__ float W4[MAX_ACT + 1][HEAD_W];
  __shared__ float MU[ACT_ROWS][MAX_ACT + 1];
  __shared__ float VP[ACT_ROWS][ACT_Q];
  const int t = threadIdx.x, na = a.na;
  const int r0 = blockIdx.x * ACT_ROWS;
  const int nrows = min(ACT_ROWS, a.n - r0);
  {
    constexpr int NV = ACT_ROWS * 2 * HEAD_W / 4 / HEAD_THREADS;
    float4 v[NV];
#pragma unroll
    for (int u = 0; u < NV; ++u) {
      const int i = t + u * HEAD_THREADS, r = i / (HEAD_W / 2), c = 4 * (i % (HEAD_W / 2));
      v[u] = r < nrows ? *reinterpret_cast<const float4*>(a.h3 + (int64_t)(r0 + r) * (2 * HEAD_W) + c)
                       : make_float4(0.f, 0.f, 0.f, 0.f);
    }
#pragma unroll
    for (int u = 0; u < NV; ++u) {
      const int i = t + u * HEAD_THREADS, r = i / (HEAD_W / 2), c = 4 * (i % (HEAD_W / 2));
      *reinterpret_cast<float4*>(&H[r][c]) = v[u];
    }
  }
  for (int i = t; i < (na + 1) * HEAD_W; i += HEAD_THREADS) {
    const int j = i / HEAD_W, k = i - j * HEAD_W;
    W4[j][k] = j < na ? a.w4a[j * HEAD_W + k] : a.w4c[k];
  }
  __syncthreads();
  {
    const int r = t & (ACT_ROWS - 1), q = t / ACT_ROWS;
    for (int j = q; j < na; j += ACT_Q) {
      float s = 0.f;
      for (int k = 0; k < HEAD_W; ++k) s = fmaf(H[r][k], W4[j][k], s);
      MU[r][j] = s + a.b4a[j];
    }
    float s = 0.f;
    for (int k = q * (HEAD_W / ACT_Q); k < (q + 1) * (HEAD_W / ACT_Q); ++k) s = fmaf(H[r][HEAD_W + k], W4[na][k], s);
    VP[r][q] = s;
  }
  __syncthreads();
  const int64_t so = (int64_t)a.store_row * a.n;
  for (int i = t; i < nrows * na; i += HEAD_THREADS) {
    const int r = i / na, j = i - r * na, g = r0 + r;
    float e;
    if (a.eps) {
      e = a.eps[(int64_t)g * na + j];
    } else {
      lrl_u32x4 u = lrl_philox((uint32_t)(a.row_offset + g), (uint32_t)a.counter, (LRL_RNG_POLICY << 16) ^ (uint32_t)(a.counter >> 32),
                               (uint32_t)(j >> 1), a.seed);
      const float u1 = fmaxf(lrl_u01(u.v[0]), 1e-7f), u2 = lrl_u01(u.v[1]);
      const float rad = sqrtf(-2.f * logf(u1)), th = 6.283185307179586f * u2;
      e = (j & 1) ? rad * sinf(th) : rad * cosf(th);
    }
    const float m = MU[r][j], sd = a.stdv[j];
    const float act = m + sd * e;
    const float d = act - m;
    MU[r][j] = -(d * d) / (2.f * (sd * sd)) - logf(sd) - LOG_SQRT_2PI;
    a.actions[(int64_t)g * na + j] = act;
    if (a.mu) a.mu[(int64_t)g * na + j] = m;
    if (a.do_store) {
      const int64_t o = (so + g) * na + j;
      a.store.actions[o] = act;
      a.store.mu[o] = m;
      a.store.sigma[o] = sd;
    }
  }
  __syncthreads();
  if (t < nrows) {
    const int g = r0 + t;
    float lp = 0.f;
    for (int j = 0; j < na; ++j) lp += MU[t][j];
    float vs[ACT_Q];
#pragma unroll
    for (int q = 0; q < ACT_Q; ++q) vs[q] = VP[t][q];
#pragma unroll
    for (int w = ACT_Q / 2; w >= 1; w /= 2)
#pragma unroll
      for (int q = 0; q < w; ++q) vs[q] = vs[2 * q] + vs[2 * q + 1];
    const float v = vs[0] + a.b4c[0];
    if (a.values) a.values[g] = v;
    if (a.logp) a.logp[g] = lp;
    if (a.do_store) {
      a.store.values[so + g] = v;
      a.store.logp[so + g] = lp;
    }
  }
  if (a.do_store) {
    const int64_t b = so + r0;
    copy_rows(a.obs + (int64_t)r0 * a.no, a.no, a.store.obs + b * a.no, a.no, nrows, a.no, t);
    if (a.priv)
      copy_rows(a.priv + (int64_t)r0 * a.np, a.np, a.store.priv + b * a.np, a.np, nrows, a.np, t);
    if (a.hist && a.store.hist) {
      const int hd = a.store.hist_dim, ld = a.store.hist_ld > hd ? a.store.hist_ld : hd;
      copy_rows(a.hist + (int64_t)r0 * hd, hd, a.store.hist + b * ld, ld, nrows, hd, t);
    }
  }
}

constexpr int FA_R = 16, FA_THREADS = 256;
constexpr int FA_D = 2;
constexpr int FA_XP = 260;
constexpr int FA_BIGP = 1028;
constexpr int FA_MIDP = 516;
constexpr int FA_HW_FLOATS = (HEAD_NA + 1) * HEAD_W;
constexpr int FA_LDS_FLOATS = FA_R * (FA_XP + FA_BIGP + FA_MIDP) + FA_HW_FLOATS;
constexpr int FA_ENC_MIDP = 260;
constexpr int FA_ENC_LDS_FLOATS = FA_R * (FA_XP + FA_XP + FA_ENC_MIDP);

#ifdef LRL_ACT_PROFILE
__device__ unsigned long long g_act_prof[12];
#define FA_PROF_DECL unsigned long long fa_t = clock64();
#define FA_PROF(i)                                                  \
  if (threadIdx.x == 0) {                                           \
    const unsigned long long t_ = clock64();                        \
    atomicAdd(&g_act_prof[i], t_ - fa_t);                           \
    fa_t = t_;                                                      \
  }
#else
#define FA_PROF_DECL
#define FA_PROF(i)
#endif

typedef float fa_f32x4 __attribute__((ext_vector_type(4)));

struct FaLayer {
  const float* A;
  int pa, ga, K;
  const float* W;
  int ldw, Kw, Nw;
  int64_t gw;
  const float* b;
  float* C;
  int pc, coff, Ng, groups;
  int elu, vec;
};

template <int NB, bool VEC>
__device__ __forceinline__ void fa_tiles(const FaLayer& L, int t0) {
  const int lane = threadIdx.x & 63, i = lane & 15, q = lane >> 4;
  const int tpg = L.Ng >> 4, g = t0 / tpg;
  const float* A = L.A + i * L.pa + g * L.ga + 8 * q;
  const float* W = L.W + g * L.gw;
  const float* rowp[NB];
  bool rok[NB];
#pragma unroll
  for (int j = 0; j < NB; ++j) {
    const int n = (t0 + j - g * tpg) * 16 + i;
    rok[j] = n < L.Nw;
    rowp[j] = W + (int64_t)(rok[j] ? n : L.Nw - 1) * L.ldw;
  }
  fa_f32x4 acc[NB];
#pragma unroll
  for (int j = 0; j < NB; ++j) acc[j] = fa_f32x4{0.f, 0.f, 0.f, 0.f};
  auto load_b = [&](float4 (&bv)[NB][2], int k0) {
    const int k = k0 + 8 * q;
#pragma unroll
    for (int j = 0; j < NB; ++j) {
      if constexpr (VEC) {
        const int k1 = min(k, L.Kw - 4), k2 = min(k + 4, L.Kw - 4);
        float4 v0 = *reinterpret_cast<const float4*>(rowp[j] + k1);
        float4 v1 = *reinterpret_cast<const float4*>(rowp[j] + k2);
        const bool o0 = rok[j] && k < L.Kw, o1 = rok[j] && k + 4 < L.Kw;
        bv[j][0] = o0 ? v0 : make_float4(0.f, 0.f, 0.f, 0.f);
        bv[j][1] = o1 ? v1 : make_float4(0.f, 0.f, 0.f, 0.f);
      } else {
        float v[8];
#pragma unroll
        for (int u = 0; u < 8; ++u) {
          const float x = rowp[j][min(k + u, L.Kw - 1)];
          v[u] = (rok[j] && k + u < L.Kw) ? x : 0.f;
        }
        bv[j][0] = make_float4(v[0], v[1], v[2], v[3]);
        bv[j][1] = make_float4(v[4], v[5], v[6], v[7]);
      }
    }
  };
  const int nck = L.K >> 5;
  float4 ring[FA_D][NB][2];
#pragma unroll
  for (int d = 0; d < FA_D; ++d) load_b(ring[d], 32 * min(d, nck - 1));
  for (int c0 = 0; c0 < nck; c0 += FA_D) {
#pragma unroll
    for (int d = 0; d < FA_D; ++d) {
      const int c = c0 + d;
      if (c < nck) {
        const float4 a0 = *reinterpret_cast<const float4*>(A + 32 * c);
        const float4 a1 = *reinterpret_cast<const float4*>(A + 32 * c + 4);
        const float av[8] = {a0.x, a0.y, a0.z, a0.w, a1.x, a1.y, a1.z, a1.w};
#pragma unroll
        for (int u = 0; u < 8; ++u) {
#pragma unroll
          for (int j = 0; j < NB; ++j) {
            const float4& bq = ring[d][j][u >> 2];
            const float b = (u & 3) == 0 ? bq.x : (u & 3) == 1 ? bq.y : (u & 3) == 2 ? bq.z : bq.w;
            acc[j] = __builtin_amdgcn_mfma_f32_16x16x4f32(av[u], b, acc[j], 0, 0, 0);
          }
        }
        load_b(ring[d], 32 * min(c + FA_D, nck - 1));
      }
    }
  }
#pragma unroll
  for (int j = 0; j < NB; ++j) {
    const int n = (t0 + j - g * tpg) * 16 + i;
    if (n < L.Nw) {
      const float bias = L.b[g * L.Nw + n];
      float* c = L.C + (4 * q) * L.pc + L.coff + g * L.Ng + n;
#pragma unroll
      for (int r = 0; r < 4; ++r) {
        float v = acc[j][r] + bias;
        if (L.elu) v = v > 0.f ? v : expm1f(v);
        c[r * L.pc] = v;
      }
    }
  }
}

template <int NBC, bool VEC>
__device__ __forceinline__ void fa_layer(const FaLayer& L) {
  const int w = threadIdx.x >> 6, T = L.groups * (L.Ng >> 4);
  const int tpw = T >= 4 ? T / 4 : 1;
  if (w * tpw >= T) return;
  const int t0 = w * tpw;
  if constexpr (NBC == 16) {
    fa_tiles<8, VEC>(L, t0);
    fa_tiles<8, VEC>(L, t0 + 8);
  } else if constexpr (NBC > 0) {
    fa_tiles<NBC, VEC>(L, t0);
  } else {
    switch (tpw) {
      case 1: fa_tiles<1, VEC>(L, t0); break;
      case 2: fa_tiles<2, VEC>(L, t0); break;
      case 4: fa_tiles<4, VEC>(L, t0); break;
      case 8: fa_tiles<8, VEC>(L, t0); break;
      case 16: fa_tiles<8, VEC>(L, t0); fa_tiles<8, VEC>(L, t0 + 8); break;
      default:
        for (int t = t0; t < t0 + tpw; ++t) fa_tiles<1, VEC>(L, t);
    }
  }
}

struct FusedActArgs {
  const float* w;
  lrl_ppo_net net;
  const float *obs, *priv, *hist, *eps;
  int n, xs;
  uint32_t vec;
  uint64_t seed, counter;
  int64_t row_offset;
  float *actions, *mu, *values, *logp;
  lrl_rollout_store store;
  int store_row, do_store;
  float* xa_out;
};

template <bool PRESET, bool ENC_ONLY = false>
__global__ __launch_bounds__(FA_THREADS) void act_fused_kernel(FusedActArgs a) {
  extern __shared__ __attribute__((aligned(16))) float fa_lds[];
  float* X = fa_lds;
  float* BIG = X + FA_R * FA_XP;
  float* MID = BIG + FA_R * (ENC_ONLY ? FA_XP : FA_BIGP);
  float* HW = MID + FA_R * FA_MIDP;
  FA_PROF_DECL
  const lrl_ppo_net& nt = a.net;
  const int t = threadIdx.x, r0 = blockIdx.x * FA_R, nrows = min(FA_R, a.n - r0);
  const int no = nt.num_obs, np = nt.num_priv, PP = 36, EP2 = nt.enc_h1 + 4;
  for (int e = t; e < FA_R * a.xs; e += FA_THREADS) {
    const int r = e / a.xs, c = e - r * a.xs;
    X[r * FA_XP + c] = (r < nrows && c < no) ? a.obs[(int64_t)(r0 + r) * no + c] : 0.f;
  }
  for (int e = t; e < FA_R * 32; e += FA_THREADS) {
    const int r = e >> 5, c = e & 31;
    MID[r * PP + c] = (r < nrows && c < np) ? a.priv[(int64_t)(r0 + r) * np + c] : 0.f;
  }
  if constexpr (!ENC_ONLY)
    for (int e = t; e < FA_HW_FLOATS; e += FA_THREADS)
      HW[e] = e < HEAD_NA * HEAD_W ? a.w[nt.w4a + e] : a.w[nt.w4c + (e - HEAD_NA * HEAD_W)];
  __syncthreads();
  FA_PROF(0)
  const float* w = a.w;
  FaLayer L;
  L = FaLayer{MID, PP, 0, 32, w + nt.e1w, np, np, nt.enc_h0, 0, w + nt.e1b, BIG, FA_XP, 0, nt.enc_h0, 1, 1, 0};
  fa_layer<PRESET ? 4 : 0, false>(L);
  __syncthreads();
  FA_PROF(1)
  L = FaLayer{BIG, FA_XP, 0, nt.enc_h0, w + nt.e2w, nt.enc_h0, nt.enc_h0, nt.enc_h1, 0, w + nt.e2b, MID, EP2, 0,
              nt.enc_h1, 1, 1, (int)(a.vec >> 1) & 1};
  if (PRESET || (a.vec & 2u)) fa_layer<PRESET ? 2 : 0, true>(L);
  else fa_layer<0, false>(L);
  __syncthreads();
  FA_PROF(2)
  L = FaLayer{MID, EP2, 0, nt.enc_h1, w + nt.e3w, nt.enc_h1, nt.enc_h1, nt.latent, 0, w + nt.e3b, X, FA_XP, no,
              (nt.latent + 15) / 16 * 16, 1, 0, (int)(a.vec >> 2) & 1};
  if (PRESET || (a.vec & 4u)) fa_layer<PRESET ? 1 : 0, true>(L);
  else fa_layer<0, false>(L);
  __syncthreads();
  FA_PROF(3)
  if constexpr (ENC_ONLY) {
    const int q4 = a.xs >> 2;
    for (int e = t; e < nrows * q4; e += FA_THREADS) {
      const int r = e / q4, c = 4 * (e - r * q4);
      *reinterpret_cast<float4*>(a.xa_out + (int64_t)(r0 + r) * a.xs + c) = *reinterpret_cast<const float4*>(X + r * FA_XP + c);
    }
    return;
  }
  const int nx = no + nt.latent;
  L = FaLayer{X, FA_XP, 0, a.xs, w + nt.w1, nx, nx, 2 * nt.ac_h0, 0, w + nt.b1, BIG, FA_BIGP, 0, 2 * nt.ac_h0, 1, 1,
              (int)(a.vec >> 3) & 1};
  if (PRESET || (a.vec & 8u)) fa_layer<PRESET ? 16 : 0, true>(L);
  else fa_layer<0, false>(L);
  __syncthreads();
  FA_PROF(4)
  L = FaLayer{BIG, FA_BIGP, nt.ac_h0, nt.ac_h0, w + nt.w2, nt.ac_h0, nt.ac_h0, nt.ac_h1, (int64_t)nt.ac_h1 * nt.ac_h0,
              w + nt.b2, MID, FA_MIDP, 0, nt.ac_h1, 2, 1, (int)(a.vec >> 4) & 1};
  if (PRESET || (a.vec & 16u)) fa_layer<PRESET ? 8 : 0, true>(L);
  else fa_layer<0, false>(L);
  __syncthreads();
  FA_PROF(5)
  L = FaLayer{MID, FA_MIDP, nt.ac_h1, nt.ac_h1, w + nt.w3, nt.ac_h1, nt.ac_h1, nt.ac_h2, (int64_t)nt.ac_h2 * nt.ac_h1,
              w + nt.b3, BIG, FA_XP, 0, nt.ac_h2, 2, 1, (int)(a.vec >> 5) & 1};
  if (PRESET || (a.vec & 32u)) fa_layer<PRESET ? 4 : 0, true>(L);
  else fa_layer<0, false>(L);
  __syncthreads();
  FA_PROF(6)
  constexpr int NA = HEAD_NA;
  float* MU = X;
  if (t < FA_R * (NA + 1)) {
    const int r = t / (NA + 1), j = t - r * (NA + 1);
    const float* h = BIG + r * FA_XP + (j < NA ? 0 : HEAD_W);
    const float* wr = HW + j * HEAD_W;
    float s = 0.f;
#pragma unroll 8
    for (int k = 0; k < HEAD_W; ++k) s = fmaf(h[k], wr[k], s);
    s += j < NA ? w[nt.b4a + j] : w[nt.b4c];
    MU[r * 16 + j] = s;
  }
  __syncthreads();
  FA_PROF(7)
  const int64_t so = (int64_t)a.store_row * a.n;
  if (t < FA_R * NA) {
    const int r = t / NA, j = t - r * NA, g = r0 + r;
    if (r < nrows) {
      float e;
      if (a.eps) {
        e = a.eps[(int64_t)g * NA + j];
      } else {
        lrl_u32x4 u = lrl_philox((uint32_t)(a.row_offset + g), (uint32_t)a.counter,
                                 (LRL_RNG_POLICY << 16) ^ (uint32_t)(a.counter >> 32), (uint32_t)(j >> 1), a.seed);
        const float u1 = fmaxf(lrl_u01(u.v[0]), 1e-7f), u2 = lrl_u01(u.v[1]);
        const float rad = sqrtf(-2.f * logf(u1)), th = 6.283185307179586f * u2;
        e = (j & 1) ? rad * sinf(th) : rad * cosf(th);
      }
      const float m = MU[r * 16 + j], sd = w[nt.std_off + j];
      const float act = m + sd * e;
      const float d = act - m;
      MU[r * 16 + j] = -(d * d) / (2.f * (sd * sd)) - logf(sd) - LOG_SQRT_2PI;
      a.actions[(int64_t)g * NA + j] = act;
      if (a.mu) a.mu[(int64_t)g * NA + j] = m;
      if (a.do_store) {
        const int64_t o = (so + g) * NA + j;
        a.store.actions[o] = act;
        a.store.mu[o] = m;
        a.store.sigma[o] = sd;
      }
    }
  }
  __syncthreads();
  if (t < nrows) {
    const int g = r0 + t;
    float lp = 0.f;
    for (int j = 0; j < NA; ++j) lp += MU[t * 16 + j];
    const float v = MU[t * 16 + NA];
    if (a.values) a.values[g] = v;
    if (a.logp) a.logp[g] = lp;
    if (a.do_store) {
      a.store.values[so + g] = v;
      a.store.logp[so + g] = lp;
    }
  }
  FA_PROF(8)
  if (a.do_store) {
    const int64_t b = so + r0;
    copy_rows(a.obs + (int64_t)r0 * no, no, a.store.obs + b * no, no, nrows, no, t);
    copy_rows(a.priv + (int64_t)r0 * np, np, a.store.priv + b * np, np, nrows, np, t);
    if (a.hist && a.store.hist) {
      const int hd = a.store.hist_dim, ld = a.store.hist_ld > hd ? a.store.hist_ld : hd;
      copy_rows(a.hist + (int64_t)r0 * hd, hd, a.store.hist + b * ld, ld, nrows, hd, t);
    }
  }
  FA_PROF(9)
}

struct AdaptHeadArgs {
  const float* hd2;
  int ldh;
  const float* tgt;
  int ldt;
  float* dhd2;
  const float *w, *b;
  int B, H, L;
  float* part;
  int part_len;
};

template <int CH, int CL>
__global__ __launch_bounds__(HEAD_THREADS) void adapt_head_kernel(AdaptHeadArgs a) {
  const int H = CH ? CH : a.H, L = CL ? CL : a.L;
  __shared__ float HS[HEAD_ROWS][MAX_LAT + 1];
  __shared__ float DP[HEAD_ROWS][MAX_LAT + 1];
  __shared__ float WS[MAX_LAT][MAX_LAT + 1];
  __shared__ float TG[HEAD_ROWS][MAX_LAT + 1];
  __shared__ float ERR[HEAD_ROWS];
  const int t = threadIdx.x;
  const int r0 = blockIdx.x * HEAD_ROWS;
  const int nrows = min(HEAD_ROWS, a.B - r0);
  for (int i = t; i < HEAD_ROWS * H; i += HEAD_THREADS) {
    const int r = i / H, c = i - r * H;
    HS[r][c] = r < nrows ? a.hd2[(int64_t)(r0 + r) * a.ldh + c] : 0.f;
  }
  for (int i = t; i < L * H; i += HEAD_THREADS) WS[i / H][i % H] = a.w[i];
  for (int i = t; i < HEAD_ROWS * L; i += HEAD_THREADS) {
    const int r = i / L, j = i - r * L;
    TG[r][j] = r < nrows ? a.tgt[(int64_t)(r0 + r) * a.ldt + j] : 0.f;
  }
  __syncthreads();
  const float scale = 2.f / ((float)a.B * (float)L);
  for (int i = t; i < HEAD_ROWS * L; i += HEAD_THREADS) {
    const int r = i / L, j = i - r * L;
    float d = 0.f;
    if (r < nrows) {
      float s = 0.f;
      for (int k = 0; k < H; ++k) s = fmaf(HS[r][k], WS[j][k], s);
      const float pred = s + a.b[j];
      d = pred - TG[r][j];
    }
    TG[r][j] = d * d;
    DP[r][j] = scale * d;
  }
  __syncthreads();
  if (t < HEAD_ROWS) {
    float e = 0.f;
    for (int j = 0; j < L; ++j) e += TG[t][j];
    ERR[t] = e;
  }
  __syncthreads();
  float* P = a.part + (int64_t)blockIdx.x * a.part_len;
  for (int i = t; i < nrows * H; i += HEAD_THREADS) {
    const int r = i / H, k = i - r * H;
    float s = 0.f;
    for (int j = 0; j < L; ++j) s = fmaf(DP[r][j], WS[j][k], s);
    a.dhd2[(int64_t)(r0 + r) * a.ldh + k] = s * delu(HS[r][k]);
  }
  const int nr = CH ? HEAD_ROWS : nrows;
  for (int i = t; i < L * H; i += HEAD_THREADS) {
    const int j = i / H, k = i - j * H;
    float s = 0.f;
    for (int r = 0; r < nr; ++r) s = fmaf(DP[r][j], HS[r][k], s);
    P[i] = s;
  }
  if (t < L) {
    float s = 0.f;
    for (int r = 0; r < nr; ++r) s += DP[r][t];
    P[L * H + t] = s;
  } else if (t == 64) {
    float s = 0.f;
    for (int r = 0; r < nr; ++r) s += ERR[r];
    P[L * H + L] = s;
  }
}

struct Seg {
  const float* src;
  float* dst;
  int64_t len, stride;
  int parts;
  float scale;
  int lpg;
  int blk0, nblk;
};
constexpr int MAX_SEGS = 24;
struct SegList {
  Seg s[MAX_SEGS];
  int n;
};

__global__ __launch_bounds__(256) void seg_reduce_kernel(SegList L) {
  int si = 0;
  while (si + 1 < L.n && (int)blockIdx.x >= L.s[si + 1].blk0) ++si;
  const Seg& sg = L.s[si];
  const int lpg = sg.lpg, pg = 1 << lpg, E = 256 >> lpg;
  const int e = threadIdx.x & (E - 1), g = threadIdx.x >> (8 - lpg);
  __shared__ float red[256];
  for (int64_t base = (int64_t)(blockIdx.x - sg.blk0) * E; base < sg.len; base += (int64_t)sg.nblk * E) {
    const int64_t i = base + e;
    float acc = 0.f;
    if (i < sg.len) {
      const float* p = sg.src + i;
      int q = g;
      for (; q + 7 * pg < sg.parts; q += 8 * pg) {
        float v[8];
#pragma unroll
        for (int u = 0; u < 8; ++u) v[u] = __builtin_nontemporal_load(p + (int64_t)(q + u * pg) * sg.stride);
#pragma unroll
        for (int u = 0; u < 8; ++u) acc += v[u];
      }
      for (; q < sg.parts; q += pg) acc += p[(int64_t)q * sg.stride];
    }
    if (pg == 1) {
      if (i < sg.len) sg.dst[i] = acc * sg.scale;
      continue;
    }
    red[threadIdx.x] = acc;
    __syncthreads();
    if (g == 0 && i < sg.len) {
      float t = 0.f;
      for (int k = 0; k < pg; ++k) t += red[k * E + e];
      sg.dst[i] = t * sg.scale;
    }
    __syncthreads();
  }
}

constexpr int NORM_BLOCKS = 256;
__global__ void sumsq_kernel(const float* __restrict__ g, int64_t n, double* __restrict__ part) {
  double s = 0.0;
  for (int64_t i = (int64_t)blockIdx.x * blockDim.x + threadIdx.x; i < n; i += (int64_t)gridDim.x * blockDim.x) {
    const double x = g[i];
    s += x * x;
  }
  for (int off = 32; off > 0; off >>= 1) s += __shfl_down(s, off, 64);
  __shared__ double red[4];
  if ((threadIdx.x & 63) == 0) red[threadIdx.x >> 6] = s;
  __syncthreads();
  if (threadIdx.x == 0) part[blockIdx.x] = (red[0] + red[1]) + (red[2] + red[3]);
}

__global__ void ppo_finalize_kernel(const double* __restrict__ part, int nparts, const float* __restrict__ kl_slot,
                                    float grad_scale, float max_norm, float desired_kl, int adaptive, double bc1,
                                    float inv_B, lrl_ppo_ctrl* ctrl) {
  __shared__ double red[64];
  double s = 0.0;
  for (int i = threadIdx.x; i < nparts; i += 64) s += part[i];
  red[threadIdx.x] = s;
  __syncthreads();
  if (threadIdx.x != 0) return;
  double tot = 0.0;
  for (int i = 0; i < 64; ++i) tot += red[i];
  const float total_norm = (float)sqrt(tot) * grad_scale;
  float clip = max_norm / (total_norm + 1e-6f);
  clip = fminf(clip, 1.f);
  double lr = ctrl->lr;
  const float kl = kl_slot[0] * grad_scale;
  if (adaptive) {
    const double k = (double)kl;
    if (k > (double)desired_kl * 2.0) lr = fmax(1e-5, lr / 1.5);
    else if (k < (double)desired_kl / 2.0 && k > 0.0) lr = fmin(1e-2, lr * 1.5);
  }
  ctrl->lr = lr;
  ctrl->mb[3] = kl;
  ctrl->clip_scale = clip;
  ctrl->total_norm = total_norm;
  ctrl->step_size = (float)(lr / bc1);
  ctrl->loss_sum[0] += (double)ctrl->mb[0];
  ctrl->loss_sum[1] += (double)ctrl->mb[1];
}

__global__ void adam_kernel(float* __restrict__ p, const float* __restrict__ g, float* __restrict__ m,
                            float* __restrict__ v, int64_t n, float grad_scale, const lrl_ppo_ctrl* __restrict__ ctrl,
                            float step_size_host, float one_minus_b1, float b2, float one_minus_b2, float bc2_sqrt,
                            float eps, lrl_ppo_ctrl* acc_ctrl) {
  const float clip = ctrl ? ctrl->clip_scale : 1.f;
  const float step = ctrl ? ctrl->step_size : step_size_host;
  for (int64_t i = (int64_t)blockIdx.x * blockDim.x + threadIdx.x; i < n; i += (int64_t)gridDim.x * blockDim.x) {
    float gi = g[i] * grad_scale;
    gi = gi * clip;
    float mi = m[i];
    mi = mi + one_minus_b1 * (gi - mi);
    float vi = v[i] * b2;
    vi = vi + one_minus_b2 * gi * gi;
    m[i] = mi;
    v[i] = vi;
    const float denom = sqrtf(vi) / bc2_sqrt + eps;
    p[i] = p[i] + (-step) * (mi / denom);
  }
  if (acc_ctrl && blockIdx.x == 0 && threadIdx.x == 0) acc_ctrl->loss_sum[2] += (double)acc_ctrl->mb[2];
}

__global__ void pad_cols_kernel(const float* __restrict__ W, int rows, int h, int hp, float* __restrict__ Wp) {
  const int64_t n = (int64_t)rows * hp;
  for (int64_t i = (int64_t)blockIdx.x * blockDim.x + threadIdx.x; i < n; i += (int64_t)gridDim.x * blockDim.x) {
    const int r = (int)(i / hp), c = (int)(i - (int64_t)r * hp);
    Wp[i] = c < h ? W[(int64_t)r * h + c] : 0.f;
  }
}


static int xs_of(const lrl_ppo_net& n) {
  if (n.plain) return (n.num_obs + 15) / 16 * 16;
  const int nx = n.num_obs + n.latent;
  return nx <= 64 ? 64 : (nx + 15) / 16 * 16;
}
constexpr int LATS = 32;
constexpr int HD2S = 32;
static int hist_pad(int h) { return (h + 15) / 16 * 16; }

enum MainPlane { PL_W1, PL_W2, PL_W3, PL_E2, PL_W2T, PL_W3T, PL_E2T, PL_MAIN };
constexpr int PL_FWD = PL_E2 + 1;
enum AdaptPlane { PL_D1, PL_AE2, PL_D2T, PL_ADAPT };

struct Layer {
  int64_t w, b;
  int out, in;
  int64_t ldw;
  int kf;
  int groups;
  int fwd, bwd;
};
static Layer layer(int64_t w, int64_t b, int out, int in, int groups = 1, int fwd = -1, int bwd = -1) {
  return Layer{w, b, out, in, in, in, groups, fwd, bwd};
}
struct Net {
  Layer enc[3];
  Layer body[3];
  Layer ad[3];
  Layer tgt[3];
  Layer mean;
  Layer dlat;
};
static Net layers_of(const lrl_ppo_net& n, bool actor_only = false) {
  Net L{};
  const int g = actor_only ? 1 : 2;
  L.body[0] = layer(n.w1, n.b1, g * n.ac_h0, n.num_obs + n.latent, 1, PL_W1);
  L.body[0].kf = xs_of(n);
  L.body[1] = layer(n.w2, n.b2, n.ac_h1, n.ac_h0, g, PL_W2, PL_W2T);
  L.body[2] = layer(n.w3, n.b3, n.ac_h2, n.ac_h1, g, PL_W3, PL_W3T);
  L.mean = layer(n.w4a, n.b4a, n.num_actions, n.ac_h2);
  if (n.plain) return L;
  L.enc[0] = layer(n.e1w, n.e1b, n.enc_h0, n.num_priv);
  L.enc[1] = layer(n.e2w, n.e2b, n.enc_h1, n.enc_h0, 1, PL_E2, PL_E2T);
  L.enc[2] = layer(n.e3w, n.e3b, n.latent, n.enc_h1);
  for (int i = 0; i < 3; ++i) L.tgt[i] = L.enc[i];
  L.tgt[1].fwd = PL_AE2;
  L.tgt[1].bwd = -1;
  L.ad[0] = layer(n.d1w, n.d1b, n.ad_h0, n.num_hist, 1, PL_D1);
  L.ad[1] = layer(n.d2w, n.d2b, n.ad_h1, n.ad_h0, 1, -1, PL_D2T);
  L.ad[2] = layer(n.d3w, n.d3b, n.latent, n.ad_h1);
  L.dlat = L.body[0];
  L.dlat.w += n.num_obs;
  L.dlat.in = n.latent;
  L.dlat.bwd = -1;
  return L;
}

static PlaneJob plane_job(const float* B, int64_t ldb, int layout, int N, int K, int groups, int64_t gb) {
  PlaneJob j{};
  j.W = B; j.ldw = ldb; j.gsrc = gb; j.groups = groups; j.trans = layout == GEMM_NN ? 1 : 0;
  j.rows = j.trans ? K : N; j.cols = j.trans ? N : K;
  return j;
}
static void layer_planes(const Layer& l, const float* w, PlaneJob* j) {
  const float* W = w ? w + l.w : nullptr;
  const int64_t gb = l.groups > 1 ? l.out * l.ldw : 0;
  if (l.fwd >= 0) j[l.fwd] = plane_job(W, l.ldw, GEMM_NT, l.out, l.in, l.groups, gb);
  if (l.bwd >= 0) j[l.bwd] = plane_job(W, l.ldw, GEMM_NN, l.in, l.out, l.groups, gb);
}
static int64_t place_planes(PlaneJob* j, int n, uint16_t* base) {
  int64_t off = 0;
  for (int i = 0; i < n; ++i) {
    j[i].dst = base ? base + off : nullptr;
    off += (plane_elems(j[i]) + 127) / 128 * 128;
  }
  return off;
}
static int64_t main_plane_jobs(const lrl_ppo_net& n, const float* w, uint16_t* base, PlaneJob (&j)[PL_MAIN]) {
  const Net L = layers_of(n);
  for (auto& l : L.enc) layer_planes(l, w, j);
  for (auto& l : L.body) layer_planes(l, w, j);
  return place_planes(j, PL_MAIN, base);
}
static int64_t adapt_plane_jobs(const lrl_ppo_net& n, const float* w, const float* we, uint16_t* base,
                                PlaneJob (&j)[PL_ADAPT]) {
  const Net L = layers_of(n);
  for (auto& l : L.ad) layer_planes(l, w, j);
  for (auto& l : L.tgt) layer_planes(l, we, j);
  return place_planes(j, PL_ADAPT, base);
}

struct In { const float* p; int64_t ld; };
struct Buf { float* p; int64_t ld; operator In() const { return In{p, ld}; } };
static Buf cols_from(Buf b, int col) { return Buf{b.p ? b.p + col : nullptr, b.ld}; }

struct Arena {
  char* base;
// ... 56 lines not shown
    p.wd1p = a.take(n.ad_h0, hist_pad(n.num_hist));
    ph1 += part_floats_of(L.enc[2], B) + part_floats_of(L.enc[1], B) + part_floats_of(L.enc[0], B);
    ph3 = part_floats_of(L.ad[1], B) + part_floats_of(L.ad[0], B) +
          (int64_t)hb * (n.latent * n.ad_h1 + n.latent + 1) + 64 * 4;
  }
  p.part_floats = std::max(ph1, ph3);
  p.part = a.take(p.part_floats);
  if (!n.plain) {
    PlaneJob m[PL_MAIN], d[PL_ADAPT];
    const int64_t elems = std::max(main_plane_jobs(n, nullptr, nullptr, m), adapt_plane_jobs(n, nullptr, nullptr, nullptr, d));
    p.wpl = reinterpret_cast<uint16_t*>(a.take((elems + 1) / 2));
  }
  p.bytes = a.off;
  return p;
}

static Plan make_act_plan(const lrl_ppo_net& n, int rows, char* base) {
  Plan p{};
  Arena a{base};
  take_forward(a, p, n, rows, 2);
  if (!n.plain) {
    PlaneJob j[PL_MAIN];
    main_plane_jobs(n, nullptr, nullptr, j);
    p.wpl = reinterpret_cast<uint16_t*>(a.take((place_planes(j, PL_FWD, nullptr) + 1) / 2));
  }
  p.bytes = a.off;
  return p;
}

static Plan make_student_plan(const lrl_ppo_net& n, int rows, char* base) {
  Plan p{};
  Arena a{base};
  p.xa = a.take(rows, xs_of(n));
  p.hd1 = a.take(rows, n.ad_h0);
  p.hd2 = a.take(rows, HD2S);
  p.h1 = a.take(rows, n.ac_h0);
  p.h2 = a.take(rows, n.ac_h1);
  p.h3 = a.take(rows, n.ac_h2);
  p.wd1p = a.take(n.ad_h0, hist_pad(n.num_hist));
  p.bytes = a.off;
  return p;
}

static int check_net(const lrl_ppo_net* n) {
  if (!n) return lrl_set_error(LRL_E_INVALID, "lrl_ppo: null net");
  if (n->ac_h2 != HEAD_W) return lrl_set_error(LRL_E_INVALID, "lrl_ppo: last actor/critic hidden width must be 128");
  if ((n->activation != 0 && n->activation != 1) || (n->plain != 0 && n->plain != 1))
    return lrl_set_error(LRL_E_INVALID, "lrl_ppo: activation / plain must be 0 or 1");
  if (n->plain) {
    if (n->activation != 1) return lrl_set_error(LRL_E_INVALID, "lrl_ppo: a plain net must use tanh (activation = 1)");
    if (n->num_actions != 3 && n->num_actions != HEAD_NA)
      return lrl_set_error(LRL_E_INVALID, "lrl_ppo: a plain net's num_actions must be 3 or 12");
    if (n->latent || n->enc_h0 || n->enc_h1 || n->ad_h0 || n->ad_h1 || n->adapt_begin != n->adapt_end)
      return lrl_set_error(LRL_E_INVALID, "lrl_ppo: a plain net has no encoder, latent or adaptation module");
    if (n->num_obs <= 0 || n->ac_h0 <= 0 || n->ac_h1 <= 0)
      return lrl_set_error(LRL_E_INVALID, "lrl_ppo: a plain net needs num_obs, ac_h0, ac_h1 > 0");
    return 0;
  }
  if (n->activation != 0)
    return lrl_set_error(LRL_E_INVALID, "lrl_ppo: tanh is implemented for plain nets only (activation = 1 needs plain = 1)");
  if (n->num_actions != HEAD_NA) return lrl_set_error(LRL_E_INVALID, "lrl_ppo: num_actions must be 12");
  if (n->latent > MAX_LAT || n->ad_h1 > MAX_LAT) return lrl_set_error(LRL_E_INVALID, "lrl_ppo: latent/adaptation widths > 32");
  return 0;
}

struct GemmTimer {
  bool on = false;
  std::vector<std::pair<hipEvent_t, hipEvent_t>> ev;
  size_t used = 0;
};
static GemmTimer g_timer;
static hipEvent_t timer_event() {
  hipEvent_t e = nullptr;
  if (hipEventCreate(&e) != hipSuccess) return nullptr;
  return e;
}
static void timer_begin(hipStream_t st) {
  if (!g_timer.on) return;
  if (g_timer.used == g_timer.ev.size()) g_timer.ev.emplace_back(timer_event(), timer_event());
  auto& pr = g_timer.ev[g_timer.used];
  if (pr.first) (void)hipEventRecord(pr.first, st);
}
static void timer_end(hipStream_t st) {
  if (!g_timer.on) return;
  auto& pr = g_timer.ev[g_timer.used++];
  if (pr.second) (void)hipEventRecord(pr.second, st);
}

struct SplitK { GemmP p; Seg s[2]; };
static bool splitk_job(int M, int N, int K, int groups, int splits, In dY, int64_t gy, In X, int64_t gx,
                       const int64_t* rows, float* dw, float* db, float*& part, const float* end, SplitK& o) {
  if (!splits) splits = gemm_pick_splits(M, N, K, groups);
  const int64_t gmn = (int64_t)groups * M * N, gm = (int64_t)groups * M;
  if (splitk_floats(M, N, splits, groups) > end - part) return false;
  GemmP p{};
  p.A = dY.p; p.lda = dY.ld; p.ga = gy; p.B = X.p; p.ldb = X.ld; p.gb = gx; p.b_rows = rows;
  p.M = M; p.N = N; p.K = K; p.splits = splits; p.kps = (K + splits - 1) / splits;
  p.gc = (int64_t)M * N; p.ldc = N; p.part_stride = gmn;
  p.C = part;
  p.bias_part = part + splits * gmn;
  o.p = p;
  o.s[0] = Seg{part, dw, gmn, gmn, splits, 1.f};
  o.s[1] = Seg{p.bias_part, db, gm, gm, splits, 1.f};
  part = p.bias_part + splits * gm;
  return true;
}

struct G {
  hipStream_t st;
  const float* w;
  int m;
  float* part = nullptr;
  float* part_end = nullptr;
  int rc = 0;
  const PlaneJob* planes = nullptr;
  bool tanh_act = false;
  GemmJob* jobs = nullptr;
  int njobs = 0, max_jobs = 0;
  void with(const PlaneJob* chain) { planes = chain; }
  void collect(GemmJob* list, int first, int max) { jobs = list; njobs = first; max_jobs = max; }
  void launch(GemmP& p, int image, int layout, int epi, int groups) {
    if (planes && image >= 0) gemm_use_planes(p, planes[image]);
    if (!jobs) rc = gemm_launch(p, layout, epi, groups, st);
    else if (njobs < max_jobs) jobs[njobs++] = GemmJob{p, layout, epi, groups};
    else rc = LRL_E_INVALID;
  }
  void forward(const Layer& l, In x, const int64_t* rows, Buf y, bool act, const float* Wsub = nullptr) {
    if (rc) return;
    GemmP p{};
    p.A = x.p; p.lda = x.ld; p.a_rows = rows; p.B = Wsub ? Wsub : w + l.w; p.ldb = l.ldw; p.C = y.p; p.ldc = y.ld;
    p.bias = w + l.b;
    p.M = m; p.N = l.out; p.K = l.kf; p.splits = 1;
    if (l.groups > 1) { p.ga = l.in; p.gb = l.out * l.ldw; p.gc = l.out; p.gbias = l.out; }
    launch(p, l.fwd, GEMM_NT, act ? (tanh_act ? EPI_BIAS_TANH : EPI_BIAS_ELU) : EPI_BIAS, l.groups);
  }
  void backward_data(const Layer& l, In dY, Buf dX, In aux) {
    if (rc) return;
    GemmP p{};
    p.A = dY.p; p.lda = dY.ld; p.B = w + l.w; p.ldb = l.ldw; p.C = dX.p; p.ldc = dX.ld; p.aux = aux.p; p.ld_aux = aux.ld;
    p.M = m; p.N = l.in; p.K = l.out; p.splits = 1;
    if (l.groups > 1) { p.ga = l.out; p.gb = l.out * l.ldw; p.gc = l.in; p.gaux = l.in; }
    launch(p, l.bwd, GEMM_NN, aux.p ? (tanh_act ? EPI_DTANH : EPI_DELU) : EPI_STORE, l.groups);
  }
  void weight_grad(const Layer& l, In dY, In X, const int64_t* rows, float* grads, SegList& L) {
    if (rc) return;
    const bool grouped = l.groups > 1;
    SplitK k;
    if (L.n + 2 > MAX_SEGS || !splitk_job(l.out, l.in, m, l.groups, 0, dY, grouped ? l.out : 0, X, grouped ? l.in : 0,
                                          rows, grads + l.w, grads + l.b, part, part_end, k)) {
      rc = LRL_E_INVALID;
      return;
    }
    launch(k.p, -1, GEMM_TN, EPI_PARTIAL, l.groups);
    if (rc) return;
    L.s[L.n++] = k.s[0];
    L.s[L.n++] = k.s[1];
    part = reinterpret_cast<float*>(((reinterpret_cast<uintptr_t>(part) + 255) / 256) * 256);
  }
};

static int launch_jobs(const GemmJob* all, const int* idx, int n, hipStream_t st) {
  GemmJob js[MAX_MULTI_JOBS];
  if (n > MAX_MULTI_JOBS) return LRL_E_INVALID;
  for (int i = 0; i < n; ++i) js[i] = all[idx[i]];
  if (n > 1) {
    const int r = gemm_launch_multi(js, n, st);
    if (r) return r < 0 ? r : 0;
  }
  for (int i = 0; i < n; ++i)
    if (int rc = gemm_launch(js[i].p, js[i].layout, js[i].epi, js[i].groups, st)) return rc;
  return 0;
}

static int bwd_multi_mode() {
  const char* e = getenv("LRL_PPO_BWD_MULTI");
  return e && e[0] >= '0' && e[0] <= '3' ? e[0] - '0' : 1;
}

struct Fork {
  hipStream_t st = nullptr;
  hipEvent_t go = nullptr, done = nullptr;
};
static Fork* fork_for_device(hipStream_t caller) {
  const char* e = getenv("LRL_PPO_FORK");
  if (e && e[0] == '0') return nullptr;
  static Fork forks[64];
  static std::mutex mu;
  int dev = 0;
  if (caller) {
    hipDevice_t d = 0;
    if (hipStreamGetDevice(caller, &d) != hipSuccess) return nullptr;
    dev = (int)d;
  } else if (hipGetDevice(&dev) != hipSuccess) {
    return nullptr;
  }
  if (dev < 0 || dev >= 64) return nullptr;
  std::lock_guard<std::mutex> lock(mu);
  Fork& f = forks[dev];
  if (!f.st) {
    int cur = 0;
    if (hipGetDevice(&cur) != hipSuccess) return nullptr;
    const bool sw = cur != dev;
    if (sw && hipSetDevice(dev) != hipSuccess) return nullptr;
    Fork nf;
    const bool ok = hipStreamCreateWithFlags(&nf.st, hipStreamNonBlocking) == hipSuccess &&
                    hipEventCreateWithFlags(&nf.go, hipEventDisableTiming) == hipSuccess &&
                    hipEventCreateWithFlags(&nf.done, hipEventDisableTiming) == hipSuccess;
    if (sw) (void)hipSetDevice(cur);
    if (!ok) return nullptr;
    f = nf;
  }
  return &f;
}

static void launch_seg(const SegList& L0, hipStream_t st) {
  SegList L = L0;
  int total = 0;
  for (int i = 0; i < L.n; ++i) {
    Seg& s = L.s[i];
    int lpg = 0;
    while (lpg < 6 && (4 << (lpg + 1)) <= s.parts && (s.len << lpg) < 2048 * 256) ++lpg;
    s.lpg = lpg;
    s.nblk = (int)std::min<int64_t>((s.len + (256 >> lpg) - 1) / (256 >> lpg), 2048);
    s.blk0 = total;
    total += s.nblk;
  }
  if (total > 0) hipLaunchKernelGGL(seg_reduce_kernel, dim3(total), dim3(256), 0, st, L);
}

template <int NJ>
static int split_planes(PlaneJob (&j)[NJ], int n, bool on, hipStream_t st) {
  if (on) return x6_planes_launch(j, n, st);
  for (auto& q : j) q.dst = nullptr;
  return 0;
}

static void prep_x(const lrl_ppo_net& n, const float* obs, const int64_t* rows, int m, Buf xa, hipStream_t st) {
  hipLaunchKernelGGL(ppo_prep_kernel, dim3(prep_blocks(m, (int)xa.ld)), dim3(256), 0, st, obs, rows, m, n.num_obs,
                     (int)xa.ld, xa.p);
}
static void encoder_forward(G& g, const Layer (&e)[3], In priv, const int64_t* rows, const Plan& P, Buf latent) {
  g.forward(e[0], priv, rows, P.he1, true);
  g.forward(e[1], P.he1, nullptr, P.he2, true);
  g.forward(e[2], P.he2, nullptr, latent, false);
}
static void body_forward(G& g, const Layer (&b)[3], const Plan& P) {
  g.forward(b[0], P.xa, nullptr, P.h1, true);
  g.forward(b[1], P.h1, nullptr, P.h2, true);
  g.forward(b[2], P.h2, nullptr, P.h3, true);
}
static void adaptation_l1_forward(G& g, Layer l, In hist, const int64_t* rows, const Plan& P) {
  const int h = l.in, hpad = hist_pad(h);
  if (hist.ld >= hpad && hist.ld % 4 == 0 && ((uintptr_t)hist.p & 15) == 0 && hpad != h) {
    const int64_t cnt = (int64_t)l.out * hpad;
    hipLaunchKernelGGL(pad_cols_kernel, dim3((unsigned)std::min<int64_t>((cnt + 255) / 256, 1024)), dim3(256), 0, g.st,
                       g.w + l.w, l.out, h, hpad, P.wd1p.p);
    l.kf = hpad;
    l.ldw = hpad;
    g.forward(l, hist, rows, P.hd1, true, P.wd1p.p);
  } else {
    l.fwd = -1;
    g.forward(l, hist, rows, P.hd1, true);
  }
}

static void launch_loss_head(const lrl_ppo_net& n, const float* w, float* grads, const lrl_ppo_batch* bt,
                             const lrl_ppo_hparams* hp, lrl_ppo_ctrl* ctrl, const Plan& P, float*& part, SegList& L,
                             hipStream_t st) {
  const int B = bt->batch, na = n.num_actions, hb = (B + HEAD_ROWS - 1) / HEAD_ROWS;
  HeadArgs ha{};
  ha.h3 = P.h3.p; ha.dh3 = P.dh3.p;
  ha.w4a = w + n.w4a; ha.b4a = w + n.b4a; ha.w4c = w + n.w4c; ha.b4c = w + n.b4c; ha.stdv = w + n.std_off;
  ha.actions = bt->actions; ha.old_mu = bt->mu; ha.old_sigma = bt->sigma; ha.tv = bt->values; ha.ret = bt->returns;
  ha.adv = bt->adv; ha.old_logp = bt->logp; ha.rows = bt->rows;
  ha.B = B; ha.na = na; ha.clip = hp->clip_param; ha.ent_coef = hp->entropy_coef; ha.vcoef = hp->value_loss_coef;
  ha.clipped_value = hp->use_clipped_value_loss;
  ha.part = part; ha.part_len = hp_len(na);
  if (n.plain && na == 3) hipLaunchKernelGGL((ppo_head_kernel<3, true>), dim3(hb), dim3(HEAD_THREADS), 0, st, ha);
  else if (n.plain) hipLaunchKernelGGL((ppo_head_kernel<HEAD_NA, true>), dim3(hb), dim3(HEAD_THREADS), 0, st, ha);
  else hipLaunchKernelGGL((ppo_head_kernel<HEAD_NA, false>), dim3(hb), dim3(HEAD_THREADS), 0, st, ha);
  const int64_t pl = hp_len(na);
  const float invB = 1.f / (float)B;
  L.s[L.n++] = Seg{part + hp_w4a(na), grads + n.w4a, (int64_t)na * HEAD_W, pl, hb, 1.f};
  L.s[L.n++] = Seg{part + hp_b4a(na), grads + n.b4a, na, pl, hb, 1.f};
  L.s[L.n++] = Seg{part + hp_w4c(na), grads + n.w4c, HEAD_W, pl, hb, 1.f};
  L.s[L.n++] = Seg{part + hp_b4c(na), grads + n.b4c, 1, pl, hb, 1.f};
  L.s[L.n++] = Seg{part + hp_std(na), grads + n.std_off, na, pl, hb, 1.f};
  L.s[L.n++] = Seg{part + hp_kl(na), grads + n.kl_slot, 1, pl, hb, invB};
  L.s[L.n++] = Seg{part + hp_kl(na) + 1, &ctrl->mb[1], 1, pl, hb, invB};
  L.s[L.n++] = Seg{part + hp_kl(na) + 2, &ctrl->mb[0], 1, pl, hb, invB};
  part += ((hb * pl + 63) / 64) * 64;
}

}

using namespace lrl;

static bool act_planes_on() {
  const char* e = getenv("LRL_ACT_PLANES");
  return e && e[0] == '1' && gemm_x6p_enabled();
}

static bool fused_envelope(const lrl_ppo_net& n, bool body) {
  auto run_ok = [](int groups, int Ng) {
    if (Ng % 16) return false;
    const int T = groups * (Ng / 16), tpg = Ng / 16;
    const int tpw = T >= 4 ? T / 4 : 1;
    if (T >= 4 && T % 4) return false;
    return tpg % std::min(tpw, 8) == 0;
  };
  if (!(xs_of(n) % 32 == 0 && xs_of(n) <= 256 && n.num_priv <= 32 && n.enc_h0 <= 256 && n.enc_h0 % 32 == 0 &&
        n.enc_h1 % 32 == 0 && n.enc_h1 + 4 <= (body ? FA_MIDP : FA_ENC_MIDP) && n.latent <= 32 && run_ok(1, n.enc_h0) &&
        run_ok(1, n.enc_h1) && run_ok(1, (n.latent + 15) / 16 * 16)))
    return false;
  return !body || (n.ac_h0 % 32 == 0 && n.ac_h1 % 32 == 0 && 2 * n.ac_h0 <= 1024 && 2 * n.ac_h1 <= 512 &&
                   2 * n.ac_h2 <= 256 && run_ok(1, 2 * n.ac_h0) && run_ok(2, n.ac_h1) && run_ok(2, n.ac_h2));
}
static bool act_enc_fused(const lrl_ppo_net& n) {
  const char* e = getenv("LRL_ACT_ENC_FUSED");
  return !(e && e[0] == '0') && fused_envelope(n, false);
}
static bool fused_act_fits(const lrl_ppo_net& n) {
  const char* e = getenv("LRL_ACT_FUSED");
  return e && e[0] == '1' && fused_envelope(n, true);
}
static void launch_act_fused(FusedActArgs& fa, bool body, hipStream_t st) {
  const lrl_ppo_net& n = fa.net;
  auto al = [&](int64_t off, int ld) { return (reinterpret_cast<uintptr_t>(fa.w + off) & 15) == 0 && ld % 4 == 0; };
  fa.vec = (al(n.e2w, n.enc_h0) ? 2u : 0u) | (al(n.e3w, n.enc_h1) ? 4u : 0u);
  if (body)
    fa.vec |= (al(n.w1, n.num_obs + n.latent) ? 8u : 0u) | (al(n.w2, n.ac_h0) ? 16u : 0u) | (al(n.w3, n.ac_h1) ? 32u : 0u);
  const bool preset = n.enc_h0 == 256 && n.enc_h1 == 128 && n.latent <= 32 &&
                      (body ? n.ac_h0 == 512 && n.ac_h1 == 256 && n.ac_h2 == 128 && fa.vec == 62u : fa.vec == 6u);
  const dim3 grid((fa.n + FA_R - 1) / FA_R), block(FA_THREADS);
  const size_t lds = (body ? FA_LDS_FLOATS : FA_ENC_LDS_FLOATS) * sizeof(float);
  if (body && preset) hipLaunchKernelGGL(act_fused_kernel<true>, grid, block, lds, st, fa);
  else if (body) hipLaunchKernelGGL(act_fused_kernel<false>, grid, block, lds, st, fa);
  else if (preset) hipLaunchKernelGGL((act_fused_kernel<true, true>), grid, block, lds, st, fa);
  else hipLaunchKernelGGL((act_fused_kernel<false, true>), grid, block, lds, st, fa);
}

extern "C" int64_t lrl_ppo_act_workspace_bytes(const lrl_ppo_net* net, int32_t n) {
  if (check_net(net) || n <= 0) return -1;
  return make_act_plan(*net, n, nullptr).bytes;
}

extern "C" int lrl_debug_act_profile(unsigned long long* out, int reset) {
#ifdef LRL_ACT_PROFILE
  if (hipMemcpyFromSymbol(out, HIP_SYMBOL(g_act_prof), sizeof(unsigned long long) * 12) != hipSuccess) return -2;
  if (reset) {
    unsigned long long z[12] = {0};
    if (hipMemcpyToSymbol(HIP_SYMBOL(g_act_prof), z, sizeof(z)) != hipSuccess) return -2;
  }
  return 12;
#else
  (void)out;
  (void)reset;
  return 0;
#endif
}

extern "C" int32_t lrl_ppo_act(const lrl_ppo_net* net, const float* params, const float* obs, const float* priv,
                               const float* hist, int32_t n, const float* eps, uint64_t seed, uint64_t counter,
                               int64_t row_offset, float* actions, float* mu, float* values, float* logp, const lrl_rollout_store* store,
                               int32_t store_row, void* workspace, void* stream) {
  if (int rc = check_net(net)) return rc;
  if (!params || !obs || (!priv && !net->plain) || !actions || !workspace || n <= 0)
    return lrl_set_error(LRL_E_INVALID, "lrl_ppo_act: null argument or n <= 0");
  if (store && (!store->obs || (!store->priv && priv) || !store->actions || !store->values || !store->logp ||
                !store->mu || !store->sigma || store->hist_dim < 0 ||
                (store->hist_ld != 0 && store->hist_ld < store->hist_dim)))
    return lrl_set_error(LRL_E_INVALID, "lrl_ppo_act: incomplete rollout store");
  const lrl_ppo_net& nt = *net;
  hipStream_t st = static_cast<hipStream_t>(stream);
  auto io = [&](auto& a) {
    a.obs = obs; a.priv = priv; a.hist = hist; a.eps = eps; a.n = n;
    a.seed = seed; a.counter = counter; a.row_offset = row_offset;
    a.actions = actions; a.mu = mu; a.values = values; a.logp = logp;
    if (store) a.store = *store;
    a.store_row = store_row; a.do_store = store ? 1 : 0;
  };
  const bool full = !nt.plain;
  if (full && fused_act_fits(nt)) {
    static const bool ok = [] {
      auto set = [](const void* f) {
        return hipFuncSetAttribute(f, hipFuncAttributeMaxDynamicSharedMemorySize, FA_LDS_FLOATS * sizeof(float)) ==
               hipSuccess;
      };
      return set(reinterpret_cast<const void*>(act_fused_kernel<true>)) &&
             set(reinterpret_cast<const void*>(act_fused_kernel<false>));
    }();
    if (!ok) return lrl_set_error(LRL_E_HIP, "lrl_ppo_act: fused kernel LDS attribute");
    FusedActArgs fa{};
    fa.w = params; fa.net = nt; fa.xs = xs_of(nt);
    io(fa);
    launch_act_fused(fa, true, st);
    return hipGetLastError() == hipSuccess ? 0 : lrl_set_error(LRL_E_HIP, "lrl_ppo_act: launch failed");
  }
  Plan P = make_act_plan(nt, n, static_cast<char*>(workspace));
  G g{st, params, n};
  g.tanh_act = nt.plain;
  const Net L = layers_of(nt);
  PlaneJob pj[PL_MAIN];
  if (full) {
    main_plane_jobs(nt, params, P.wpl, pj);
    if (int rc = split_planes(pj, PL_FWD, act_planes_on(), st)) return lrl_set_error(rc, "lrl_ppo_act: planes launch failed");
    g.with(pj);
  }
  if (full && act_enc_fused(nt)) {
    FusedActArgs fa{};
    fa.w = params; fa.net = nt; fa.obs = obs; fa.priv = priv; fa.n = n; fa.xs = (int)P.xa.ld; fa.xa_out = P.xa.p;
    launch_act_fused(fa, false, st);
  } else {
    prep_x(nt, obs, nullptr, n, P.xa, st);
    if (full) encoder_forward(g, L.enc, In{priv, nt.num_priv}, nullptr, P, cols_from(P.xa, nt.num_obs));
  }
  body_forward(g, L.body, P);
  if (g.rc) return lrl_set_error(g.rc, "lrl_ppo_act: GEMM launch failed");
  ActHeadArgs ah{};
  ah.h3 = P.h3.p; ah.w4a = params + nt.w4a; ah.b4a = params + nt.b4a; ah.w4c = params + nt.w4c; ah.b4c = params + nt.b4c;
  ah.stdv = params + nt.std_off; ah.na = nt.num_actions; ah.no = nt.num_obs; ah.np = nt.num_priv;
  io(ah);
  hipLaunchKernelGGL(act_head_kernel, dim3((n + ACT_ROWS - 1) / ACT_ROWS), dim3(HEAD_THREADS), 0, st, ah);
  return hipGetLastError() == hipSuccess ? 0 : lrl_set_error(LRL_E_HIP, "lrl_ppo_act: launch failed");
}

extern "C" int64_t lrl_ppo_act_student_workspace_bytes(const lrl_ppo_net* net, int32_t n) {
  if (check_net(net) || net->plain || n <= 0) return -1;
  return make_student_plan(*net, n, nullptr).bytes;
}

extern "C" int32_t lrl_ppo_act_student(const lrl_ppo_net* net, const float* params, const float* obs,
                                       const float* hist, int32_t hist_ld, int32_t n, float* mean, float* latent,
                                       void* workspace, void* stream) {
  if (int rc = check_net(net)) return rc;
  if (net->plain) return lrl_set_error(LRL_E_INVALID, "lrl_ppo_act_student: a plain net has no adaptation module");
  if (!params || !obs || !hist || !mean || !workspace || n <= 0)
    return lrl_set_error(LRL_E_INVALID, "lrl_ppo_act_student: null argument or n <= 0");
  const lrl_ppo_net& nt = *net;
  const int hld = hist_ld ? hist_ld : nt.num_hist;
  if (hld < nt.num_hist) return lrl_set_error(LRL_E_INVALID, "lrl_ppo_act_student: hist_ld < num_hist");
  Plan P = make_student_plan(nt, n, static_cast<char*>(workspace));
  hipStream_t st = static_cast<hipStream_t>(stream);
  G g{st, params, n};
  const Net L = layers_of(nt, true);
  const Buf lat = cols_from(P.xa, nt.num_obs);
  prep_x(nt, obs, nullptr, n, P.xa, st);
  adaptation_l1_forward(g, L.ad[0], In{hist, hld}, nullptr, P);
  g.forward(L.ad[1], P.hd1, nullptr, P.hd2, true);
  g.forward(L.ad[2], P.hd2, nullptr, lat, false);
  body_forward(g, L.body, P);
  g.forward(L.mean, P.h3, nullptr, Buf{mean, nt.num_actions}, false);
  if (g.rc) return lrl_set_error(g.rc, "lrl_ppo_act_student: GEMM launch failed");
  if (latent &&
      hipMemcpy2DAsync(latent, (size_t)nt.latent * 4, lat.p, (size_t)lat.ld * 4, (size_t)nt.latent * 4, n,
                       hipMemcpyDeviceToDevice, st) != hipSuccess)
    return lrl_set_error(LRL_E_HIP, "lrl_ppo_act_student: latent copy failed");
  return hipGetLastError() == hipSuccess ? 0 : lrl_set_error(LRL_E_HIP, "lrl_ppo_act_student: launch failed");
}

extern "C" int64_t lrl_ppo_workspace_bytes(const lrl_ppo_net* net, int32_t batch) {
  if (check_net(net) || batch <= 0) return -1;
  return make_plan(*net, batch, nullptr).bytes;
}

extern "C" int32_t lrl_ppo_forward_backward(const lrl_ppo_net* net, const float* params, float* grads,
                                            const lrl_ppo_batch* bt, const lrl_ppo_hparams* hp, void* workspace,
                                            lrl_ppo_ctrl* ctrl, void* stream) {
  if (int rc = check_net(net)) return rc;
  if (!bt || !hp || !params || !grads || !workspace || !ctrl || bt->batch <= 0)
    return lrl_set_error(LRL_E_INVALID, "lrl_ppo_forward_backward: null argument");
  const lrl_ppo_net& n = *net;
  const int B = bt->batch;
  const bool full = !n.plain;
  Plan P = make_plan(n, B, static_cast<char*>(workspace));
  hipStream_t st = static_cast<hipStream_t>(stream);
  G g{st, params, B, P.part, P.part + P.part_floats};
  g.tanh_act = n.plain;
  const Net net_l = layers_of(n);
  const Layer(&enc)[3] = net_l.enc;
  const Layer(&body)[3] = net_l.body;
  PlaneJob pj[PL_MAIN];
  if (full) {
    main_plane_jobs(n, params, P.wpl, pj);
    if (int rc = split_planes(pj, PL_MAIN, gemm_x6p_enabled(), st))
      return lrl_set_error(rc, "lrl_ppo_forward_backward: planes launch failed");
    g.with(pj);
  }
  const In priv{bt->priv, n.num_priv};
  prep_x(n, bt->obs, bt->rows, B, P.xa, st);
  if (full) encoder_forward(g, enc, priv, bt->rows, P, cols_from(P.xa, n.num_obs));
  body_forward(g, body, P);
  if (g.rc) return lrl_set_error(g.rc, "lrl_ppo_forward_backward: forward GEMM launch failed");
  SegList L{};
  launch_loss_head(n, params, grads, bt, hp, ctrl, P, g.part, L, st);
  g.backward_data(body[2], P.dh3, P.dh2, P.h2);
  g.backward_data(body[1], P.dh2, P.dh1, P.h1);
  if (full) g.backward_data(net_l.dlat, P.dh1, P.dlat, In{});
  enum { DWE3, DHE2, DWE2, DHE1, DWE1, DW3, DW2, DW1, NJOBS };
  GemmJob jobs[NJOBS];
  const int first = full ? 0 : DW3;
  g.collect(jobs, first, NJOBS);
  if (full) {
    g.weight_grad(enc[2], P.dlat, P.he2, nullptr, grads, L);
    g.backward_data(enc[2], P.dlat, P.dhe2, P.he2);
    g.weight_grad(enc[1], P.dhe2, P.he1, nullptr, grads, L);
    g.backward_data(enc[1], P.dhe2, P.dhe1, P.he1);
    g.weight_grad(enc[0], P.dhe1, priv, bt->rows, grads, L);
  }
  g.weight_grad(body[2], P.dh3, P.h2, nullptr, grads, L);
  g.weight_grad(body[1], P.dh2, P.h1, nullptr, grads, L);
  g.weight_grad(body[0], P.dh1, P.xa, nullptr, grads, L);
  int rc = g.rc ? g.rc : (g.njobs == NJOBS ? 0 : LRL_E_INVALID);
  if (rc) return lrl_set_error(rc, "lrl_ppo_forward_backward: backward GEMM launch failed");
  struct Set { int n, i[MAX_MULTI_JOBS]; };
  Set sets[NJOBS];
  int ns = 0;
  const int mode = full ? bwd_multi_mode() : 0;
  if (mode == 0) {
    for (int i = first; i < NJOBS; ++i) sets[ns++] = Set{1, {i}};
  } else if (g_timer.on) {
    sets[ns++] = Set{3, {DWE3, DHE2, DW3}};
    sets[ns++] = Set{2, {DWE2, DHE1}};
    sets[ns++] = Set{1, {DW2}};
    sets[ns++] = Set{2, {DWE1, DW1}};
  } else {
    static const int hosts[3][3] = {{DW3, DW1, DW2}, {DW3, DW2, DW1}, {DW2, DW1, DW3}};
    const int* host = hosts[mode - 1];
    sets[ns++] = Set{3, {DWE3, DHE2, host[0]}};
    sets[ns++] = Set{3, {DWE2, DHE1, host[1]}};
    sets[ns++] = Set{2, {DWE1, host[2]}};
  }
  Fork* fk = mode == 0 && full ? fork_for_device(st) : nullptr;
  if (fk && (hipEventRecord(fk->go, st) != hipSuccess || hipStreamWaitEvent(fk->st, fk->go, 0) != hipSuccess))
    return lrl_set_error(LRL_E_HIP, "lrl_ppo_forward_backward: stream fork failed");
  for (int s = 0; s < ns && !rc; ++s) {
    const int lead = sets[s].i[0];
    const bool timed = full && sets[s].n == 1 && lead == DW2;
    if (timed) timer_begin(st);
    rc = launch_jobs(jobs, sets[s].i, sets[s].n, fk && lead < DW3 ? fk->st : st);
    if (timed) timer_end(st);
    if (fk && lead == DWE1 && hipEventRecord(fk->done, fk->st) != hipSuccess)
      return lrl_set_error(LRL_E_HIP, "lrl_ppo_forward_backward: stream fork failed");
  }
  if (fk && hipStreamWaitEvent(st, fk->done, 0) != hipSuccess)
    return lrl_set_error(LRL_E_HIP, "lrl_ppo_forward_backward: stream join failed");
  if (rc) return lrl_set_error(rc, "lrl_ppo_forward_backward: backward GEMM launch failed");
  launch_seg(L, st);
  return hipGetLastError() == hipSuccess ? 0 : lrl_set_error(LRL_E_HIP, "lrl_ppo_forward_backward: launch failed");
}

extern "C" int32_t lrl_ppo_optimizer_step(const lrl_ppo_net* net, float* params, const float* grads, float* exp_avg,
                                          float* exp_avg_sq, int64_t step, float grad_scale,
                                          const lrl_ppo_hparams* hp, void* workspace, lrl_ppo_ctrl* ctrl,
                                          void* stream) {
  if (int rc = check_net(net)) return rc;
  if (!params || !grads || !exp_avg || !exp_avg_sq || !hp || !workspace || !ctrl || step < 1)
    return lrl_set_error(LRL_E_INVALID, "lrl_ppo_optimizer_step: bad argument");
  const lrl_ppo_net& n = *net;
  hipStream_t st = static_cast<hipStream_t>(stream);
  double* norm_part = static_cast<double*>(workspace);
  const int64_t len = n.main_end - n.main_begin;
  hipLaunchKernelGGL(sumsq_kernel, dim3(NORM_BLOCKS), dim3(256), 0, st, grads + n.main_begin, len, norm_part);
  const double bc1 = 1.0 - pow((double)hp->beta1, (double)step);
  const double bc2 = 1.0 - pow((double)hp->beta2, (double)step);
  hipLaunchKernelGGL(ppo_finalize_kernel, dim3(1), dim3(64), 0, st, norm_part, NORM_BLOCKS,
                     grads + n.kl_slot, grad_scale, hp->max_grad_norm, hp->desired_kl, hp->adaptive_schedule, bc1,
                     0.f, ctrl);
  const int blocks = (int)std::min<int64_t>((len + 255) / 256, 2048);
  hipLaunchKernelGGL(adam_kernel, dim3(blocks), dim3(256), 0, st, params + n.main_begin, grads + n.main_begin,
                     exp_avg + n.main_begin, exp_avg_sq + n.main_begin, len, grad_scale, ctrl, 0.f,
                     (float)(1.0 - (double)hp->beta1), hp->beta2, (float)(1.0 - (double)hp->beta2), (float)sqrt(bc2),
                     hp->eps, (lrl_ppo_ctrl*)nullptr);
  return hipGetLastError() == hipSuccess ? 0 : lrl_set_error(LRL_E_HIP, "lrl_ppo_optimizer_step: launch failed");
}

extern "C" int32_t lrl_ppo_adaptation_forward_backward(const lrl_ppo_net* net, const float* params,
                                                       const float* enc_params, float* grads, const lrl_ppo_batch* bt,
                                                       void* workspace, lrl_ppo_ctrl* ctrl, void* stream) {
  if (int rc = check_net(net)) return rc;
  if (net->plain)
    return lrl_set_error(LRL_E_INVALID, "lrl_ppo_adaptation_forward_backward: a plain net has no adaptation module");
  if (!bt || !params || !grads || !workspace || !ctrl || bt->batch <= 0)
    return lrl_set_error(LRL_E_INVALID, "lrl_ppo_adaptation_forward_backward: null argument");
  const lrl_ppo_net& n = *net;
  const int B = bt->batch;
  const int hld = bt->hist_ld ? bt->hist_ld : n.num_hist;
  if (hld < n.num_hist) return lrl_set_error(LRL_E_INVALID, "lrl_ppo_adaptation: hist_ld < num_hist");
  Plan P = make_plan(n, B, static_cast<char*>(workspace));
  hipStream_t st = static_cast<hipStream_t>(stream);
  G g{st, params, B, P.part, P.part + P.part_floats};
  const Net net_l = layers_of(n);
  const Layer(&ad)[3] = net_l.ad;
  const float* we = enc_params ? enc_params : params;
  PlaneJob pj[PL_ADAPT];
  adapt_plane_jobs(n, params, we, P.wpl, pj);
  if (int rc = split_planes(pj, PL_ADAPT, gemm_x6p_enabled(), st))
    return lrl_set_error(rc, "lrl_ppo_adaptation: planes launch failed");
  g.with(pj);
  g.w = we;
  encoder_forward(g, net_l.tgt, In{bt->priv, n.num_priv}, bt->rows, P, P.tgt);
  g.w = params;
  const In hist{bt->hist, hld};
  adaptation_l1_forward(g, ad[0], hist, bt->rows, P);
  g.forward(ad[1], P.hd1, nullptr, P.hd2, true);
  if (g.rc) return lrl_set_error(g.rc, "lrl_ppo_adaptation: forward GEMM launch failed");
  SegList L{};
  float*& part = g.part;
  const int hb = (B + HEAD_ROWS - 1) / HEAD_ROWS;
  AdaptHeadArgs aa{};
  aa.hd2 = P.hd2.p; aa.ldh = HD2S; aa.tgt = P.tgt.p; aa.ldt = LATS; aa.dhd2 = P.dhd2.p; aa.w = params + n.d3w;
  aa.b = params + n.d3b;
  aa.B = B; aa.H = n.ad_h1; aa.L = n.latent; aa.part = part; aa.part_len = n.latent * n.ad_h1 + n.latent + 1;
  if (aa.H == 32 && aa.L == 18)
    hipLaunchKernelGGL((adapt_head_kernel<32, 18>), dim3(hb), dim3(HEAD_THREADS), 0, st, aa);
  else
    hipLaunchKernelGGL((adapt_head_kernel<0, 0>), dim3(hb), dim3(HEAD_THREADS), 0, st, aa);
  {
    const int64_t pl = aa.part_len;
    L.s[L.n++] = Seg{part, grads + n.d3w, (int64_t)n.latent * n.ad_h1, pl, hb, 1.f};
    L.s[L.n++] = Seg{part + n.latent * n.ad_h1, grads + n.d3b, n.latent, pl, hb, 1.f};
    L.s[L.n++] = Seg{part + n.latent * n.ad_h1 + n.latent, &ctrl->mb[2], 1, pl, hb,
                     1.f / ((float)B * (float)n.latent)};
    part += ((hb * pl + 63) / 64) * 64;
  }
  g.weight_grad(ad[1], P.dhd2, P.hd1, nullptr, grads, L);
  g.backward_data(ad[1], P.dhd2, P.dhd1, P.hd1);
  g.weight_grad(ad[0], P.dhd1, hist, bt->rows, grads, L);
  if (g.rc) return lrl_set_error(g.rc, "lrl_ppo_adaptation: backward GEMM launch failed");
  launch_seg(L, st);
  return hipGetLastError() == hipSuccess ? 0 : lrl_set_error(LRL_E_HIP, "lrl_ppo_adaptation: launch failed");
}

extern "C" int32_t lrl_ppo_adaptation_step(const lrl_ppo_net* net, float* params, const float* grads, float* exp_avg,
                                           float* exp_avg_sq, int64_t step, double lr, float grad_scale,
                                           const lrl_ppo_hparams* hp, lrl_ppo_ctrl* ctrl, void* stream) {
  if (int rc = check_net(net)) return rc;
  if (net->plain) return lrl_set_error(LRL_E_INVALID, "lrl_ppo_adaptation_step: a plain net has no adaptation module");
  if (!params || !grads || !exp_avg || !exp_avg_sq || !hp || step < 1)
    return lrl_set_error(LRL_E_INVALID, "lrl_ppo_adaptation_step: bad argument");
  const lrl_ppo_net& n = *net;
  hipStream_t st = static_cast<hipStream_t>(stream);
  const double bc1 = 1.0 - pow((double)hp->beta1, (double)step);
  const double bc2 = 1.0 - pow((double)hp->beta2, (double)step);
  const int64_t len = n.adapt_end - n.adapt_begin;
  const int blocks = (int)std::min<int64_t>((len + 255) / 256, 2048);
  hipLaunchKernelGGL(adam_kernel, dim3(blocks), dim3(256), 0, st, params + n.adapt_begin, grads + n.adapt_begin,
                     exp_avg + n.adapt_begin, exp_avg_sq + n.adapt_begin, len, grad_scale,
                     (const lrl_ppo_ctrl*)nullptr, (float)(lr / bc1), (float)(1.0 - (double)hp->beta1), hp->beta2,
                     (float)(1.0 - (double)hp->beta2), (float)sqrt(bc2), hp->eps, ctrl);
  return hipGetLastError() == hipSuccess ? 0 : lrl_set_error(LRL_E_HIP, "lrl_ppo_adaptation_step: launch failed");
}

static int use_test_planes(GemmP& p, int layout, int groups, float* workspace, int64_t workspace_floats,
                           hipStream_t st) {
  PlaneJob j = plane_job(p.B, p.ldb, layout, p.N, p.K, groups, p.gb);
  j.dst = reinterpret_cast<uint16_t*>(workspace);
  if (!workspace || plane_elems(j) > 2 * workspace_floats)
    return lrl_set_error(LRL_E_INVALID, "lrl_gemm_f32(_ex): workspace too small for the planes");
  if (int rc = x6_planes_launch(&j, 1, st)) return lrl_set_error(rc, "lrl_gemm_f32(_ex): planes launch failed");
  gemm_use_planes(p, j);
  return 0;
}

extern "C" int32_t lrl_gemm_f32(int32_t layout, int32_t epi, int32_t M, int32_t N, int32_t K, const float* A,
                                int64_t lda, const float* B, int64_t ldb, float* C, int64_t ldc, const float* bias,
                                const float* aux, int64_t ld_aux, const int64_t* rows, float* workspace,
                                int64_t workspace_floats, void* stream) {
  hipStream_t st = static_cast<hipStream_t>(stream);
  if ((epi == EPI_BIAS_TANH && (layout & 0xff) != GEMM_NT) || (epi == EPI_DTANH && (layout & 0xff) != GEMM_NN))
    return lrl_set_error(LRL_E_INVALID, "lrl_gemm_f32: epi 5 is an NT epilogue, epi 6 an NN one");
  if (epi == EPI_DTANH && !aux) return lrl_set_error(LRL_E_INVALID, "lrl_gemm_f32: epi 6 needs aux");
  if (layout == GEMM_TN) {
    if (ldc != N) return lrl_set_error(LRL_E_INVALID, "lrl_gemm_f32: TN needs ldc == N");
    int splits = 0;
    if (const char* e = getenv("LRL_GEMM_SPLITS")) splits = std::max(atoi(e), 0);
    SplitK k;
    float* part = workspace;
    if (!splitk_job(M, N, K, 1, splits, In{A, lda}, 0, In{B, ldb}, 0, rows, C, const_cast<float*>(bias), part,
                    workspace + workspace_floats, k))
      return lrl_set_error(LRL_E_INVALID, "lrl_gemm_f32: workspace too small");
    if (int rc = gemm_launch(k.p, GEMM_TN, EPI_PARTIAL, 1, st)) return lrl_set_error(rc, "lrl_gemm_f32: launch failed");
    SegList L{};
    L.s[L.n++] = k.s[0];
    if (bias) L.s[L.n++] = k.s[1];
    launch_seg(L, st);
    return hipGetLastError() == hipSuccess ? 0 : lrl_set_error(LRL_E_HIP, "lrl_gemm_f32: launch failed");
  }
  GemmP p{};
  p.A = A; p.lda = lda; p.B = B; p.ldb = ldb; p.C = C; p.ldc = ldc; p.bias = bias; p.aux = aux; p.ld_aux = ld_aux;
// ... 122 lines not shown
```

Before: 4.151 million env-steps/s.

## Rework fused act kernel with x6 bf16-split MFMA body and enable by default

Restructures the fused policy-act kernel. Each block now handles 32 rows with 512 threads and the grid is doubled so actor and critic groups run in separate blocks. The actor/critic body layers use x6 three-way bf16 split MFMA tiles staged in LDS, while the encoder tiles process multiple 16-row blocks per wave. The fused path, previously opt-in, now runs by default for 2048 to 4096 rows, replacing the multi-kernel GEMM act path to cut launch count and global round trips. The cost is higher LDS use per block, a tighter shape envelope, and duplicated encoder work per group.

Result: faster. 4.197 million env-steps/s (median of 6 runs) (+1.1%).

```diff
diff --git a/rapid-locomotion-rl_amd/csrc/lrl_gemm.h b/rapid-locomotion-rl_amd/csrc/lrl_gemm.h
--- a/rapid-locomotion-rl_amd/csrc/lrl_gemm.h
+++ b/rapid-locomotion-rl_amd/csrc/lrl_gemm.h
@@ -80,4 +80,53 @@
 
 int gemm_pick_splits(int M, int N, int K, int groups);
 
+bool gemm_x6_enabled();
+constexpr int X6_MIN_M = 64;
+
+#ifdef __HIPCC__
+typedef float f32x16 __attribute__((ext_vector_type(16)));
+typedef short bf16x8_t __attribute__((ext_vector_type(8)));
+constexpr int XBK = 16;
+
+__device__ __forceinline__ float elu_f(float x) { return x > 0.f ? x : expm1f(x); }
+__device__ __forceinline__ float tanh_f(float x) { return tanhf(x); }
+__host__ __device__ constexpr bool epi_bias(int e) { return e == EPI_BIAS || e == EPI_BIAS_ELU || e == EPI_BIAS_TANH; }
+__host__ __device__ constexpr bool epi_aux(int e) { return e == EPI_DELU || e == EPI_DTANH; }
+template <int EPI>
+__device__ __forceinline__ float epi_apply(float v, float bj, float x) {
+  if constexpr (EPI == EPI_BIAS) return v + bj;
+  else if constexpr (EPI == EPI_BIAS_ELU) return elu_f(v + bj);
+  else if constexpr (EPI == EPI_BIAS_TANH) return tanh_f(v + bj);
+  else if constexpr (EPI == EPI_DELU) return x > 0.f ? v : v * (x + 1.f);
+  else if constexpr (EPI == EPI_DTANH) return v * (1.f - x * x);
+  else return v;
 }
+
+__device__ __forceinline__ uint32_t x6_hi_pair(uint32_t u0, uint32_t u1) {
+  return __builtin_amdgcn_perm(u1, u0, 0x07060302u);
+}
+__device__ __forceinline__ void x6_split2(float x0, float x1, uint32_t& h, uint32_t& m, uint32_t& l) {
+  uint32_t u0 = __float_as_uint(x0), u1 = __float_as_uint(x1);
+  h = x6_hi_pair(u0, u1);
+  float r0 = x0 - __uint_as_float(u0 & 0xffff0000u), r1 = x1 - __uint_as_float(u1 & 0xffff0000u);
+  u0 = __float_as_uint(r0);
+  u1 = __float_as_uint(r1);
+  m = x6_hi_pair(u0, u1);
+  r0 = r0 - __uint_as_float(u0 & 0xffff0000u);
+  r1 = r1 - __uint_as_float(u1 & 0xffff0000u);
+  l = x6_hi_pair(__float_as_uint(r0), __float_as_uint(r1));
+}
+__device__ __forceinline__ int x6_off(int r, int c) { return r * XBK + 8 * (c ^ ((r >> 3) & 1)); }
+
+__device__ __forceinline__ f32x16 x6_mma(const bf16x8_t (&a)[3], const bf16x8_t (&b)[3], f32x16 c) {
+  c = __builtin_amdgcn_mfma_f32_32x32x16_bf16(a[2], b[0], c, 0, 0, 0);
+  c = __builtin_amdgcn_mfma_f32_32x32x16_bf16(a[1], b[1], c, 0, 0, 0);
+  c = __builtin_amdgcn_mfma_f32_32x32x16_bf16(a[0], b[2], c, 0, 0, 0);
+  c = __builtin_amdgcn_mfma_f32_32x32x16_bf16(a[1], b[0], c, 0, 0, 0);
+  c = __builtin_amdgcn_mfma_f32_32x32x16_bf16(a[0], b[1], c, 0, 0, 0);
+  c = __builtin_amdgcn_mfma_f32_32x32x16_bf16(a[0], b[0], c, 0, 0, 0);
+  return c;
+}
+#endif
+
+}
diff --git a/rapid-locomotion-rl_amd/csrc/lrl_gemm.hip b/rapid-locomotion-rl_amd/csrc/lrl_gemm.hip
--- a/rapid-locomotion-rl_amd/csrc/lrl_gemm.hip
+++ b/rapid-locomotion-rl_amd/csrc/lrl_gemm.hip
@@ -13,7 +13,6 @@
 
 namespace lrl {
 
-typedef float f32x16 __attribute__((ext_vector_type(16)));
 
 #ifndef LRL_GBK
 #define LRL_GBK 16
@@ -60,19 +59,6 @@
   return 0;
 }
 
-__device__ __forceinline__ float elu_f(float x) { return x > 0.f ? x : expm1f(x); }
-__device__ __forceinline__ float tanh_f(float x) { return tanhf(x); }
-__host__ __device__ constexpr bool epi_bias(int e) { return e == EPI_BIAS || e == EPI_BIAS_ELU || e == EPI_BIAS_TANH; }
-__host__ __device__ constexpr bool epi_aux(int e) { return e == EPI_DELU || e == EPI_DTANH; }
-template <int EPI>
-__device__ __forceinline__ float epi_apply(float v, float bj, float x) {
-  if constexpr (EPI == EPI_BIAS) return v + bj;
-  else if constexpr (EPI == EPI_BIAS_ELU) return elu_f(v + bj);
-  else if constexpr (EPI == EPI_BIAS_TANH) return tanh_f(v + bj);
-  else if constexpr (EPI == EPI_DELU) return x > 0.f ? v : v * (x + 1.f);
-  else if constexpr (EPI == EPI_DTANH) return v * (1.f - x * x);
-  else return v;
-}
 
 template <int V>
 using Int = std::integral_constant<int, V>;
@@ -849,7 +835,6 @@
   }
 }
 
-constexpr int XBK = 16;
 #ifndef LRL_X6_PIPE
 #define LRL_X6_PIPE 1
 #endif
@@ -857,33 +842,6 @@
 #define LRL_X6_PIPE_VALU 4
 #endif
 
-__device__ __forceinline__ uint32_t x6_hi_pair(uint32_t u0, uint32_t u1) {
-  return __builtin_amdgcn_perm(u1, u0, 0x07060302u);
-}
-__device__ __forceinline__ void x6_split2(float x0, float x1, uint32_t& h, uint32_t& m, uint32_t& l) {
-  uint32_t u0 = __float_as_uint(x0), u1 = __float_as_uint(x1);
-  h = x6_hi_pair(u0, u1);
-  float r0 = x0 - __uint_as_float(u0 & 0xffff0000u), r1 = x1 - __uint_as_float(u1 & 0xffff0000u);
-  u0 = __float_as_uint(r0);
-  u1 = __float_as_uint(r1);
-  m = x6_hi_pair(u0, u1);
-  r0 = r0 - __uint_as_float(u0 & 0xffff0000u);
-  r1 = r1 - __uint_as_float(u1 & 0xffff0000u);
-  l = x6_hi_pair(__float_as_uint(r0), __float_as_uint(r1));
-}
-__device__ __forceinline__ int x6_off(int r, int c) { return r * XBK + 8 * (c ^ ((r >> 3) & 1)); }
-
-typedef short bf16x8_t __attribute__((ext_vector_type(8)));
-
-__device__ __forceinline__ f32x16 x6_mma(const bf16x8_t (&a)[3], const bf16x8_t (&b)[3], f32x16 c) {
-  c = __builtin_amdgcn_mfma_f32_32x32x16_bf16(a[2], b[0], c, 0, 0, 0);
-  c = __builtin_amdgcn_mfma_f32_32x32x16_bf16(a[1], b[1], c, 0, 0, 0);
-  c = __builtin_amdgcn_mfma_f32_32x32x16_bf16(a[0], b[2], c, 0, 0, 0);
-  c = __builtin_amdgcn_mfma_f32_32x32x16_bf16(a[1], b[0], c, 0, 0, 0);
-  c = __builtin_amdgcn_mfma_f32_32x32x16_bf16(a[0], b[1], c, 0, 0, 0);
-  c = __builtin_amdgcn_mfma_f32_32x32x16_bf16(a[0], b[0], c, 0, 0, 0);
-  return c;
-}
 
 template <int R, bool KC, bool KGATHER = false>
 struct X6Op {
@@ -1232,6 +1190,7 @@
   static const int on = env_switch("LRL_GEMM_X6", 1);
   return on != 0 && !(path_off() & 16);
 }
+bool gemm_x6_enabled() { return x6_enabled(); }
 
 static int try_x6d(const GemmP& p, int layout, int epi, int groups, int bm, int bn, hipStream_t st);
 static bool x6d_fits(const GemmP& p, int layout, int bm, int bn);
@@ -1250,7 +1209,7 @@
     bn = p.N <= 64 ? 64 : 128;
     return true;
   }
-  if (p.splits != 1 || p.N < 16 || p.M < 64 || epi == EPI_PARTIAL) return false;
+  if (p.splits != 1 || p.N < 16 || p.M < X6_MIN_M || epi == EPI_PARTIAL) return false;
   if (p.K < 32) return false;
   if (p.N <= 32 && p.K % 128 == 0 && (p.K / 128 == 4 || p.K / 128 == 8) && p.avec == 4 && p.M >= 256) return false;
   static const int small_wg = getenv("LRL_X6_SMALL_WG") ? atoi(getenv("LRL_X6_SMALL_WG")) : 1024;
diff --git a/rapid-locomotion-rl_amd/csrc/lrl_ppo.hip b/rapid-locomotion-rl_amd/csrc/lrl_ppo.hip
--- a/rapid-locomotion-rl_amd/csrc/lrl_ppo.hip
+++ b/rapid-locomotion-rl_amd/csrc/lrl_ppo.hip
@@ -323,39 +323,57 @@
   float* xa_out;
 };
 
+template <int NT = HEAD_THREADS>
 __device__ __forceinline__ void copy_rows(const float* __restrict__ src, int64_t sld, float* __restrict__ dst,
                                           int64_t dld, int nrows, int cols, int t) {
   if (((((uintptr_t)src | (uintptr_t)dst) & 7) == 0) && (((sld | dld | cols) & 1) == 0)) {
     const int c2 = cols / 2, n = nrows * c2;
-    for (int i0 = t; i0 < n; i0 += 8 * HEAD_THREADS) {
+    for (int i0 = t; i0 < n; i0 += 8 * NT) {
       float2 v[8];
 #pragma unroll
       for (int u = 0; u < 8; ++u) {
-        const int i = i0 + u * HEAD_THREADS, r = i / c2, c = i - r * c2;
+        const int i = i0 + u * NT, r = i / c2, c = i - r * c2;
         if (i < n) v[u] = reinterpret_cast<const float2*>(src + r * sld)[c];
       }
 #pragma unroll
       for (int u = 0; u < 8; ++u) {
-        const int i = i0 + u * HEAD_THREADS, r = i / c2, c = i - r * c2;
+        const int i = i0 + u * NT, r = i / c2, c = i - r * c2;
         if (i < n) reinterpret_cast<float2*>(dst + r * dld)[c] = v[u];
       }
     }
   } else {
     const int n = nrows * cols;
-    for (int i0 = t; i0 < n; i0 += 8 * HEAD_THREADS) {
+    for (int i0 = t; i0 < n; i0 += 8 * NT) {
       float v[8];
 #pragma unroll
       for (int u = 0; u < 8; ++u) {
-        const int i = i0 + u * HEAD_THREADS, r = i / cols, c = i - r * cols;
+        const int i = i0 + u * NT, r = i / cols, c = i - r * cols;
         if (i < n) v[u] = src[r * sld + c];
       }
 #pragma unroll
       for (int u = 0; u < 8; ++u) {
-        const int i = i0 + u * HEAD_THREADS, r = i / cols, c = i - r * cols;
+        const int i = i0 + u * NT, r = i / cols, c = i - r * cols;
         if (i < n) dst[r * dld + c] = v[u];
       }
     }
   }
+}
+
+__device__ __forceinline__ float act_draw(const float* eps, int64_t row_offset, uint64_t seed, uint64_t counter, int g,
+                                          int j, int na, float m, float sd, float& act) {
+  float e;
+  if (eps) {
+    e = eps[(int64_t)g * na + j];
+  } else {
+    lrl_u32x4 u = lrl_philox((uint32_t)(row_offset + g), (uint32_t)counter, (LRL_RNG_POLICY << 16) ^ (uint32_t)(counter >> 32),
+                             (uint32_t)(j >> 1), seed);
+    const float u1 = fmaxf(lrl_u01(u.v[0]), 1e-7f), u2 = lrl_u01(u.v[1]);
+    const float rad = sqrtf(-2.f * logf(u1)), th = 6.283185307179586f * u2;
+    e = (j & 1) ? rad * sinf(th) : rad * cosf(th);
+  }
+  act = m + sd * e;
+  const float d = act - m;
+  return -(d * d) / (2.f * (sd * sd)) - logf(sd) - LOG_SQRT_2PI;
 }
 
 constexpr int ACT_ROWS = 16, ACT_Q = HEAD_THREADS / ACT_ROWS;
@@ -403,20 +421,9 @@
   const int64_t so = (int64_t)a.store_row * a.n;
   for (int i = t; i < nrows * na; i += HEAD_THREADS) {
     const int r = i / na, j = i - r * na, g = r0 + r;
-    float e;
-    if (a.eps) {
-      e = a.eps[(int64_t)g * na + j];
-    } else {
-      lrl_u32x4 u = lrl_philox((uint32_t)(a.row_offset + g), (uint32_t)a.counter, (LRL_RNG_POLICY << 16) ^ (uint32_t)(a.counter >> 32),
-                               (uint32_t)(j >> 1), a.seed);
-      const float u1 = fmaxf(lrl_u01(u.v[0]), 1e-7f), u2 = lrl_u01(u.v[1]);
-      const float rad = sqrtf(-2.f * logf(u1)), th = 6.283185307179586f * u2;
-      e = (j & 1) ? rad * sinf(th) : rad * cosf(th);
-    }
     const float m = MU[r][j], sd = a.stdv[j];
-    const float act = m + sd * e;
-    const float d = act - m;
-    MU[r][j] = -(d * d) / (2.f * (sd * sd)) - logf(sd) - LOG_SQRT_2PI;
+    float act;
+    MU[r][j] = act_draw(a.eps, a.row_offset, a.seed, a.counter, g, j, na, m, sd, act);
     a.actions[(int64_t)g * na + j] = act;
     if (a.mu) a.mu[(int64_t)g * na + j] = m;
     if (a.do_store) {
@@ -461,16 +468,22 @@
 constexpr int FA_R = 16, FA_THREADS = 256;
 constexpr int FA_D = 2;
 constexpr int FA_XP = 260;
-constexpr int FA_BIGP = 1028;
-constexpr int FA_MIDP = 516;
-constexpr int FA_HW_FLOATS = (HEAD_NA + 1) * HEAD_W;
-constexpr int FA_LDS_FLOATS = FA_R * (FA_XP + FA_BIGP + FA_MIDP) + FA_HW_FLOATS;
 constexpr int FA_ENC_MIDP = 260;
 constexpr int FA_ENC_LDS_FLOATS = FA_R * (FA_XP + FA_XP + FA_ENC_MIDP);
+constexpr int OA_R = 32, OA_THREADS = 512;
+constexpr int OA_MAX_H0 = 512, OA_MAX_H1 = 256, OA_MAX_XS = 256;
+constexpr int OA_PLANE = OA_R * XBK;
+constexpr int OA_SLICE = 3 * OA_PLANE;
+constexpr int OA_A_BYTES = OA_R * OA_MAX_H0 * 6, OA_B_BYTES = OA_R * OA_MAX_H1 * 6;
+constexpr int OA_LDS_BYTES = OA_A_BYTES + OA_B_BYTES;
+constexpr int OA_H3P = HEAD_W + 1;
+static_assert(OA_R * OA_MAX_XS * 6 <= OA_B_BYTES && OA_R * OA_H3P * 4 <= OA_A_BYTES, "overlays");
+static_assert(OA_R * (2 * FA_XP + FA_ENC_MIDP) * 4 <= OA_A_BYTES + 2048, "encoder tiles");
+static_assert(((HEAD_NA * HEAD_W) + 2 * OA_R * 16) * 4 <= OA_B_BYTES, "head scratch");
 
 #ifdef LRL_ACT_PROFILE
 __device__ unsigned long long g_act_prof[12];
-#define FA_PROF_DECL unsigned long long fa_t = clock64();
+#define FA_PROF_INIT clock64()
 #define FA_PROF(i)                                                  \
   if (threadIdx.x == 0) {                                           \
     const unsigned long long t_ = clock64();                        \
@@ -478,7 +491,7 @@
     fa_t = t_;                                                      \
   }
 #else
-#define FA_PROF_DECL
+#define FA_PROF_INIT 0ull
 #define FA_PROF(i)
 #endif
 
@@ -486,33 +499,32 @@
 
 struct FaLayer {
   const float* A;
-  int pa, ga, K;
+  int pa, K;
   const float* W;
   int ldw, Kw, Nw;
-  int64_t gw;
   const float* b;
   float* C;
-  int pc, coff, Ng, groups;
-  int elu, vec;
+  int pc, coff, Ng;
+  int elu;
 };
 
-template <int NB, bool VEC>
+template <int NB, bool VEC, int RB>
 __device__ __forceinline__ void fa_tiles(const FaLayer& L, int t0) {
   const int lane = threadIdx.x & 63, i = lane & 15, q = lane >> 4;
-  const int tpg = L.Ng >> 4, g = t0 / tpg;
-  const float* A = L.A + i * L.pa + g * L.ga + 8 * q;
-  const float* W = L.W + g * L.gw;
+  const float* A = L.A + i * L.pa + 8 * q;
   const float* rowp[NB];
   bool rok[NB];
 #pragma unroll
   for (int j = 0; j < NB; ++j) {
-    const int n = (t0 + j - g * tpg) * 16 + i;
+    const int n = (t0 + j) * 16 + i;
     rok[j] = n < L.Nw;
-    rowp[j] = W + (int64_t)(rok[j] ? n : L.Nw - 1) * L.ldw;
-  }
-  fa_f32x4 acc[NB];
-#pragma unroll
-  for (int j = 0; j < NB; ++j) acc[j] = fa_f32x4{0.f, 0.f, 0.f, 0.f};
+    rowp[j] = L.W + (int64_t)(rok[j] ? n : L.Nw - 1) * L.ldw;
+  }
+  fa_f32x4 acc[RB][NB];
+#pragma unroll
+  for (int b = 0; b < RB; ++b)
+#pragma unroll
+    for (int j = 0; j < NB; ++j) acc[b][j] = fa_f32x4{0.f, 0.f, 0.f, 0.f};
   auto load_b = [&](float4 (&bv)[NB][2], int k0) {
     const int k = k0 + 8 * q;
 #pragma unroll
@@ -545,16 +557,22 @@
     for (int d = 0; d < FA_D; ++d) {
       const int c = c0 + d;
       if (c < nck) {
-        const float4 a0 = *reinterpret_cast<const float4*>(A + 32 * c);
-        const float4 a1 = *reinterpret_cast<const float4*>(A + 32 * c + 4);
-        const float av[8] = {a0.x, a0.y, a0.z, a0.w, a1.x, a1.y, a1.z, a1.w};
+        float av[RB][8];
+#pragma unroll
+        for (int b = 0; b < RB; ++b) {
+          const float4 a0 = *reinterpret_cast<const float4*>(A + 16 * b * L.pa + 32 * c);
+          const float4 a1 = *reinterpret_cast<const float4*>(A + 16 * b * L.pa + 32 * c + 4);
+          av[b][0] = a0.x; av[b][1] = a0.y; av[b][2] = a0.z; av[b][3] = a0.w;
+          av[b][4] = a1.x; av[b][5] = a1.y; av[b][6] = a1.z; av[b][7] = a1.w;
+        }
 #pragma unroll
         for (int u = 0; u < 8; ++u) {
 #pragma unroll
           for (int j = 0; j < NB; ++j) {
             const float4& bq = ring[d][j][u >> 2];
-            const float b = (u & 3) == 0 ? bq.x : (u & 3) == 1 ? bq.y : (u & 3) == 2 ? bq.z : bq.w;
-            acc[j] = __builtin_amdgcn_mfma_f32_16x16x4f32(av[u], b, acc[j], 0, 0, 0);
+            const float bw = (u & 3) == 0 ? bq.x : (u & 3) == 1 ? bq.y : (u & 3) == 2 ? bq.z : bq.w;
+#pragma unroll
+            for (int b = 0; b < RB; ++b) acc[b][j] = __builtin_amdgcn_mfma_f32_16x16x4f32(av[b][u], bw, acc[b][j], 0, 0, 0);
           }
         }
         load_b(ring[d], 32 * min(c + FA_D, nck - 1));
@@ -563,40 +581,39 @@
   }
 #pragma unroll
   for (int j = 0; j < NB; ++j) {
-    const int n = (t0 + j - g * tpg) * 16 + i;
+    const int n = (t0 + j) * 16 + i;
     if (n < L.Nw) {
-      const float bias = L.b[g * L.Nw + n];
-      float* c = L.C + (4 * q) * L.pc + L.coff + g * L.Ng + n;
-#pragma unroll
-      for (int r = 0; r < 4; ++r) {
-        float v = acc[j][r] + bias;
-        if (L.elu) v = v > 0.f ? v : expm1f(v);
-        c[r * L.pc] = v;
-      }
-    }
-  }
-}
-
-template <int NBC, bool VEC>
+      const float bias = L.b[n];
+#pragma unroll
+      for (int b = 0; b < RB; ++b) {
+        float* c = L.C + (16 * b + 4 * q) * L.pc + L.coff + n;
+#pragma unroll
+        for (int r = 0; r < 4; ++r) {
+          float v = acc[b][j][r] + bias;
+          if (L.elu) v = v > 0.f ? v : expm1f(v);
+          c[r * L.pc] = v;
+        }
+      }
+    }
+  }
+}
+
+template <int NBC, bool VEC, int RB>
 __device__ __forceinline__ void fa_layer(const FaLayer& L) {
-  const int w = threadIdx.x >> 6, T = L.groups * (L.Ng >> 4);
-  const int tpw = T >= 4 ? T / 4 : 1;
+  constexpr int NW = 4 * RB;
+  const int w = threadIdx.x >> 6, T = L.Ng >> 4;
+  const int tpw = T >= NW ? T / NW : 1;
   if (w * tpw >= T) return;
   const int t0 = w * tpw;
-  if constexpr (NBC == 16) {
-    fa_tiles<8, VEC>(L, t0);
-    fa_tiles<8, VEC>(L, t0 + 8);
-  } else if constexpr (NBC > 0) {
-    fa_tiles<NBC, VEC>(L, t0);
+  if constexpr (NBC > 0) {
+    fa_tiles<NBC, VEC, RB>(L, t0);
   } else {
     switch (tpw) {
-      case 1: fa_tiles<1, VEC>(L, t0); break;
-      case 2: fa_tiles<2, VEC>(L, t0); break;
-      case 4: fa_tiles<4, VEC>(L, t0); break;
-      case 8: fa_tiles<8, VEC>(L, t0); break;
-      case 16: fa_tiles<8, VEC>(L, t0); fa_tiles<8, VEC>(L, t0 + 8); break;
+      case 1: fa_tiles<1, VEC, RB>(L, t0); break;
+      case 2: fa_tiles<2, VEC, RB>(L, t0); break;
+      case 4: fa_tiles<4, VEC, RB>(L, t0); break;
       default:
-        for (int t = t0; t < t0 + tpw; ++t) fa_tiles<1, VEC>(L, t);
+        for (int t = t0; t < t0 + tpw; ++t) fa_tiles<1, VEC, RB>(L, t);
     }
   }
 }
@@ -615,141 +632,318 @@
   float* xa_out;
 };
 
-template <bool PRESET, bool ENC_ONLY = false>
-__global__ __launch_bounds__(FA_THREADS) void act_fused_kernel(FusedActArgs a) {
-  extern __shared__ __attribute__((aligned(16))) float fa_lds[];
-  float* X = fa_lds;
-  float* BIG = X + FA_R * FA_XP;
-  float* MID = BIG + FA_R * (ENC_ONLY ? FA_XP : FA_BIGP);
-  float* HW = MID + FA_R * FA_MIDP;
-  FA_PROF_DECL
+template <bool PRESET, int RB>
+__device__ __forceinline__ void fa_encoder(const FusedActArgs& a, float* X, float* HE1, float* MID, int r0, int nrows,
+                                           unsigned long long& fa_t) {
+  constexpr int R = 16 * RB, NT = 256 * RB;
   const lrl_ppo_net& nt = a.net;
-  const int t = threadIdx.x, r0 = blockIdx.x * FA_R, nrows = min(FA_R, a.n - r0);
+  const int t = threadIdx.x;
   const int no = nt.num_obs, np = nt.num_priv, PP = 36, EP2 = nt.enc_h1 + 4;
-  for (int e = t; e < FA_R * a.xs; e += FA_THREADS) {
+  for (int e = t; e < R * a.xs; e += NT) {
     const int r = e / a.xs, c = e - r * a.xs;
     X[r * FA_XP + c] = (r < nrows && c < no) ? a.obs[(int64_t)(r0 + r) * no + c] : 0.f;
   }
-  for (int e = t; e < FA_R * 32; e += FA_THREADS) {
+  for (int e = t; e < R * 32; e += NT) {
     const int r = e >> 5, c = e & 31;
     MID[r * PP + c] = (r < nrows && c < np) ? a.priv[(int64_t)(r0 + r) * np + c] : 0.f;
   }
-  if constexpr (!ENC_ONLY)
-    for (int e = t; e < FA_HW_FLOATS; e += FA_THREADS)
-      HW[e] = e < HEAD_NA * HEAD_W ? a.w[nt.w4a + e] : a.w[nt.w4c + (e - HEAD_NA * HEAD_W)];
   __syncthreads();
   FA_PROF(0)
   const float* w = a.w;
   FaLayer L;
-  L = FaLayer{MID, PP, 0, 32, w + nt.e1w, np, np, nt.enc_h0, 0, w + nt.e1b, BIG, FA_XP, 0, nt.enc_h0, 1, 1, 0};
-  fa_layer<PRESET ? 4 : 0, false>(L);
+  L = FaLayer{MID, PP, 32, w + nt.e1w, np, np, nt.enc_h0, w + nt.e1b, HE1, FA_XP, 0, nt.enc_h0, 1};
+  fa_layer<PRESET ? 4 / RB : 0, false, RB>(L);
   __syncthreads();
   FA_PROF(1)
-  L = FaLayer{BIG, FA_XP, 0, nt.enc_h0, w + nt.e2w, nt.enc_h0, nt.enc_h0, nt.enc_h1, 0, w + nt.e2b, MID, EP2, 0,
-              nt.enc_h1, 1, 1, (int)(a.vec >> 1) & 1};
-  if (PRESET || (a.vec & 2u)) fa_layer<PRESET ? 2 : 0, true>(L);
-  else fa_layer<0, false>(L);
+  L = FaLayer{HE1, FA_XP, nt.enc_h0, w + nt.e2w, nt.enc_h0, nt.enc_h0, nt.enc_h1, w + nt.e2b, MID, EP2, 0, nt.enc_h1, 1};
+  if (PRESET || (a.vec & 2u)) fa_layer<PRESET ? 2 / RB : 0, true, RB>(L);
+  else fa_layer<0, false, RB>(L);
   __syncthreads();
   FA_PROF(2)
-  L = FaLayer{MID, EP2, 0, nt.enc_h1, w + nt.e3w, nt.enc_h1, nt.enc_h1, nt.latent, 0, w + nt.e3b, X, FA_XP, no,
-              (nt.latent + 15) / 16 * 16, 1, 0, (int)(a.vec >> 2) & 1};
-  if (PRESET || (a.vec & 4u)) fa_layer<PRESET ? 1 : 0, true>(L);
-  else fa_layer<0, false>(L);
+  L = FaLayer{MID, EP2, nt.enc_h1, w + nt.e3w, nt.enc_h1, nt.enc_h1, nt.latent, w + nt.e3b, X, FA_XP, no,
+              (nt.latent + 15) / 16 * 16, 0};
+  if (PRESET || (a.vec & 4u)) fa_layer<PRESET ? 1 : 0, true, RB>(L);
+  else fa_layer<0, false, RB>(L);
   __syncthreads();
   FA_PROF(3)
+}
+
+struct OaLayer {
+  const uint16_t* A;
+  int K;
+  const float* W;
+  int ldw, Kw, N;
+  const float* b;
+  uint16_t* Cp;
+  float* Cf;
+};
+
+template <int NB, int D, int MODE>
+__device__ __forceinline__ void oa_tiles(const OaLayer& L, int t0) {
+  const int lane = threadIdx.x & 63, li = lane & 31, h = lane >> 5;
+  const float* rowp[NB];
+  bool rok[NB];
+#pragma unroll
+  for (int j = 0; j < NB; ++j) {
+    const int n = (t0 + j) * 32 + li;
+    rok[j] = n < L.N;
+    rowp[j] = L.W + (int64_t)(rok[j] ? n : L.N - 1) * L.ldw;
+  }
+  f32x16 acc[NB];
+#pragma unroll
+  for (int j = 0; j < NB; ++j)
+#pragma unroll
+    for (int r = 0; r < 16; ++r) acc[j][r] = 0.f;
+  auto load_b = [&](float4 (&bv)[NB][4], int k0) {
+#pragma unroll
+    for (int j = 0; j < NB; ++j)
+#pragma unroll
+      for (int s = 0; s < 2; ++s) {
+        const int k = k0 + 16 * s + 8 * h;
+        if constexpr (MODE == 2) {
+          bv[j][2 * s] = *reinterpret_cast<const float4*>(rowp[j] + k);
+          bv[j][2 * s + 1] = *reinterpret_cast<const float4*>(rowp[j] + k + 4);
+        } else if constexpr (MODE == 1) {
+          const int k1 = min(k, L.Kw - 4), k2 = min(k + 4, L.Kw - 4);
+          float4 v0 = *reinterpret_cast<const float4*>(rowp[j] + k1);
+          float4 v1 = *reinterpret_cast<const float4*>(rowp[j] + k2);
+          const bool o0 = rok[j] && k < L.Kw, o1 = rok[j] && k + 4 < L.Kw;
+          bv[j][2 * s] = o0 ? v0 : make_float4(0.f, 0.f, 0.f, 0.f);
+          bv[j][2 * s + 1] = o1 ? v1 : make_float4(0.f, 0.f, 0.f, 0.f);
+        } else {
+          float v[8];
+#pragma unroll
+          for (int u = 0; u < 8; ++u) {
+            const float x = rowp[j][min(k + u, L.Kw - 1)];
+            v[u] = (rok[j] && k + u < L.Kw) ? x : 0.f;
+          }
+          bv[j][2 * s] = make_float4(v[0], v[1], v[2], v[3]);
+          bv[j][2 * s + 1] = make_float4(v[4], v[5], v[6], v[7]);
+        }
+      }
+  };
+  const int nck = L.K >> 5;
+  const uint16_t* Ap = L.A + x6_off(li, h);
+  float4 ring[D][NB][4];
+#pragma unroll
+  for (int d = 0; d < D; ++d) load_b(ring[d], 32 * min(d, nck - 1));
+  for (int c0 = 0; c0 < nck; c0 += D) {
+#pragma unroll
+    for (int d = 0; d < D; ++d) {
+      const int c = c0 + d;
+      if (c < nck) {
+#pragma unroll
+        for (int s = 0; s < 2; ++s) {
+          bf16x8_t av[3];
+#pragma unroll
+          for (int pl = 0; pl < 3; ++pl)
+            av[pl] = *reinterpret_cast<const bf16x8_t*>(Ap + (2 * c + s) * OA_SLICE + pl * OA_PLANE);
+#pragma unroll
+          for (int j = 0; j < NB; ++j) {
+            const float4 x0 = ring[d][j][2 * s], x1 = ring[d][j][2 * s + 1];
+            uint32_t hh[4], mm[4], ll[4];
+            x6_split2(x0.x, x0.y, hh[0], mm[0], ll[0]);
+            x6_split2(x0.z, x0.w, hh[1], mm[1], ll[1]);
+            x6_split2(x1.x, x1.y, hh[2], mm[2], ll[2]);
+            x6_split2(x1.z, x1.w, hh[3], mm[3], ll[3]);
+            uint4 vh = make_uint4(hh[0], hh[1], hh[2], hh[3]), vm = make_uint4(mm[0], mm[1], mm[2], mm[3]),
+                  vl = make_uint4(ll[0], ll[1], ll[2], ll[3]);
+            bf16x8_t bv[3];
+            bv[0] = *reinterpret_cast<bf16x8_t*>(&vh);
+            bv[1] = *reinterpret_cast<bf16x8_t*>(&vm);
+            bv[2] = *reinterpret_cast<bf16x8_t*>(&vl);
+            acc[j] = x6_mma(av, bv, acc[j]);
+          }
+        }
+        load_b(ring[d], 32 * min(c + D, nck - 1));
+      }
+    }
+  }
+#pragma unroll
+  for (int j = 0; j < NB; ++j) {
+    const int n = (t0 + j) * 32 + li;
+    if (n < L.N) {
+      const float bj = L.b[n];
+#pragma unroll
+      for (int q = 0; q < 4; ++q) {
+        const int row0 = 8 * q + 4 * h;
+        float v[4];
+#pragma unroll
+        for (int r = 0; r < 4; ++r) v[r] = epi_apply<EPI_BIAS_ELU>(acc[j][4 * q + r], bj, 0.f);
+        if (L.Cp) {
+          uint16_t* cp = L.Cp + (n >> 4) * OA_SLICE + (n & 7);
+#pragma unroll
+          for (int r = 0; r < 4; r += 2) {
+            uint32_t hh, mm, ll;
+            x6_split2(v[r], v[r + 1], hh, mm, ll);
+            const int o0 = x6_off(row0 + r, (n >> 3) & 1), o1 = x6_off(row0 + r + 1, (n >> 3) & 1);
+            cp[o0] = (uint16_t)hh;
+            cp[o1] = (uint16_t)(hh >> 16);
+            cp[OA_PLANE + o0] = (uint16_t)mm;
+            cp[OA_PLANE + o1] = (uint16_t)(mm >> 16);
+            cp[2 * OA_PLANE + o0] = (uint16_t)ll;
+            cp[2 * OA_PLANE + o1] = (uint16_t)(ll >> 16);
+          }
+        } else {
+#pragma unroll
+          for (int r = 0; r < 4; ++r) L.Cf[(row0 + r) * OA_H3P + n] = v[r];
+        }
+      }
+    }
+  }
+}
+
+template <int MODE>
+__device__ __forceinline__ void oa_layer(const OaLayer& L) {
+  const int w = threadIdx.x >> 6, T = L.N >> 5, tpw = (T + 7) >> 3;
+  int t = w * tpw;
+  const int t1 = min(T, t + tpw);
+  for (; t + 2 <= t1; t += 2) oa_tiles<2, 2, MODE>(L, t);
+  if (t < t1) oa_tiles<1, 4, MODE>(L, t);
+}
+
+template <bool PRESET, bool ENC_ONLY = false>
+__global__ __launch_bounds__(ENC_ONLY ? FA_THREADS : OA_THREADS) void act_fused_kernel(FusedActArgs a) {
+  extern __shared__ __attribute__((aligned(16))) float fa_lds[];
+  unsigned long long fa_t = FA_PROF_INIT;
+  const lrl_ppo_net& nt = a.net;
+  const int t = threadIdx.x;
   if constexpr (ENC_ONLY) {
+    float* X = fa_lds;
+    float* HE1 = X + FA_R * FA_XP;
+    float* MID = HE1 + FA_R * FA_XP;
+    const int r0 = blockIdx.x * FA_R, nrows = min(FA_R, a.n - r0);
+    fa_encoder<PRESET, 1>(a, X, HE1, MID, r0, nrows, fa_t);
     const int q4 = a.xs >> 2;
     for (int e = t; e < nrows * q4; e += FA_THREADS) {
       const int r = e / q4, c = 4 * (e - r * q4);
       *reinterpret_cast<float4*>(a.xa_out + (int64_t)(r0 + r) * a.xs + c) = *reinterpret_cast<const float4*>(X + r * FA_XP + c);
     }
-    return;
-  }
-  const int nx = no + nt.latent;
-  L = FaLayer{X, FA_XP, 0, a.xs, w + nt.w1, nx, nx, 2 * nt.ac_h0, 0, w + nt.b1, BIG, FA_BIGP, 0, 2 * nt.ac_h0, 1, 1,
-              (int)(a.vec >> 3) & 1};
-  if (PRESET || (a.vec & 8u)) fa_layer<PRESET ? 16 : 0, true>(L);
-  else fa_layer<0, false>(L);
-  __syncthreads();
-  FA_PROF(4)
-  L = FaLayer{BIG, FA_BIGP, nt.ac_h0, nt.ac_h0, w + nt.w2, nt.ac_h0, nt.ac_h0, nt.ac_h1, (int64_t)nt.ac_h1 * nt.ac_h0,
-              w + nt.b2, MID, FA_MIDP, 0, nt.ac_h1, 2, 1, (int)(a.vec >> 4) & 1};
-  if (PRESET || (a.vec & 16u)) fa_layer<PRESET ? 8 : 0, true>(L);
-  else fa_layer<0, false>(L);
-  __syncthreads();
-  FA_PROF(5)
-  L = FaLayer{MID, FA_MIDP, nt.ac_h1, nt.ac_h1, w + nt.w3, nt.ac_h1, nt.ac_h1, nt.ac_h2, (int64_t)nt.ac_h2 * nt.ac_h1,
-              w + nt.b3, BIG, FA_XP, 0, nt.ac_h2, 2, 1, (int)(a.vec >> 5) & 1};
-  if (PRESET || (a.vec & 32u)) fa_layer<PRESET ? 4 : 0, true>(L);
-  else fa_layer<0, false>(L);
-  __syncthreads();
-  FA_PROF(6)
-  constexpr int NA = HEAD_NA;
-  float* MU = X;
-  if (t < FA_R * (NA + 1)) {
-    const int r = t / (NA + 1), j = t - r * (NA + 1);
-    const float* h = BIG + r * FA_XP + (j < NA ? 0 : HEAD_W);
-    const float* wr = HW + j * HEAD_W;
-    float s = 0.f;
-#pragma unroll 8
-    for (int k = 0; k < HEAD_W; ++k) s = fmaf(h[k], wr[k], s);
-    s += j < NA ? w[nt.b4a + j] : w[nt.b4c];
-    MU[r * 16 + j] = s;
-  }
-  __syncthreads();
-  FA_PROF(7)
-  const int64_t so = (int64_t)a.store_row * a.n;
-  if (t < FA_R * NA) {
-    const int r = t / NA, j = t - r * NA, g = r0 + r;
-    if (r < nrows) {
-      float e;
-      if (a.eps) {
-        e = a.eps[(int64_t)g * NA + j];
-      } else {
-        lrl_u32x4 u = lrl_philox((uint32_t)(a.row_offset + g), (uint32_t)a.counter,
-                                 (LRL_RNG_POLICY << 16) ^ (uint32_t)(a.counter >> 32), (uint32_t)(j >> 1), a.seed);
-        const float u1 = fmaxf(lrl_u01(u.v[0]), 1e-7f), u2 = lrl_u01(u.v[1]);
-        const float rad = sqrtf(-2.f * logf(u1)), th = 6.283185307179586f * u2;
-        e = (j & 1) ? rad * sinf(th) : rad * cosf(th);
-      }
-      const float m = MU[r * 16 + j], sd = w[nt.std_off + j];
-      const float act = m + sd * e;
-      const float d = act - m;
-      MU[r * 16 + j] = -(d * d) / (2.f * (sd * sd)) - logf(sd) - LOG_SQRT_2PI;
-      a.actions[(int64_t)g * NA + j] = act;
-      if (a.mu) a.mu[(int64_t)g * NA + j] = m;
-      if (a.do_store) {
-        const int64_t o = (so + g) * NA + j;
-        a.store.actions[o] = act;
-        a.store.mu[o] = m;
-        a.store.sigma[o] = sd;
-      }
-    }
-  }
-  __syncthreads();
-  if (t < nrows) {
-    const int g = r0 + t;
-    float lp = 0.f;
-    for (int j = 0; j < NA; ++j) lp += MU[t * 16 + j];
-    const float v = MU[t * 16 + NA];
-    if (a.values) a.values[g] = v;
-    if (a.logp) a.logp[g] = lp;
+  } else {
+    constexpr int NA = HEAD_NA;
+    uint8_t* lds = reinterpret_cast<uint8_t*>(fa_lds);
+    float* X = fa_lds;
+    float* HE1 = X + OA_R * FA_XP;
+    float* MID = HE1 + OA_R * FA_XP;
+    uint16_t* H1 = reinterpret_cast<uint16_t*>(lds);
+    float* H3 = fa_lds;
+    uint16_t* XP = reinterpret_cast<uint16_t*>(lds + OA_A_BYTES);
+    float* HW = reinterpret_cast<float*>(lds + OA_A_BYTES);
+    float* MU = HW + NA * HEAD_W;
+    float* VP = MU + OA_R * 16;
+    const int grp = blockIdx.x & 1, r0 = (blockIdx.x >> 1) * OA_R, nrows = min(OA_R, a.n - r0);
+    const int no = nt.num_obs, np = nt.num_priv;
+    const float* w = a.w;
+    fa_encoder<PRESET, 2>(a, X, HE1, MID, r0, nrows, fa_t);
+    {
+      const int c8 = a.xs >> 3;
+      for (int e = t; e < OA_R * c8; e += OA_THREADS) {
+        const int r = e / c8, c = e - r * c8;
+        const float4 x0 = *reinterpret_cast<const float4*>(X + r * FA_XP + 8 * c);
+        const float4 x1 = *reinterpret_cast<const float4*>(X + r * FA_XP + 8 * c + 4);
+        uint32_t hh[4], mm[4], ll[4];
+        x6_split2(x0.x, x0.y, hh[0], mm[0], ll[0]);
+        x6_split2(x0.z, x0.w, hh[1], mm[1], ll[1]);
+        x6_split2(x1.x, x1.y, hh[2], mm[2], ll[2]);
+        x6_split2(x1.z, x1.w, hh[3], mm[3], ll[3]);
+        uint16_t* p = XP + (c >> 1) * OA_SLICE + x6_off(r, c & 1);
+        *reinterpret_cast<uint4*>(p) = make_uint4(hh[0], hh[1], hh[2], hh[3]);
+        *reinterpret_cast<uint4*>(p + OA_PLANE) = make_uint4(mm[0], mm[1], mm[2], mm[3]);
+        *reinterpret_cast<uint4*>(p + 2 * OA_PLANE) = make_uint4(ll[0], ll[1], ll[2], ll[3]);
+      }
+    }
+    __syncthreads();
+    FA_PROF(4)
+    const int nx = no + nt.latent;
+#pragma unroll 1
+    for (int l = 0; l < 3; ++l) {
+      OaLayer L;
+      if (l == 0)
+        L = OaLayer{XP, a.xs, w + nt.w1 + (int64_t)grp * nt.ac_h0 * nx, nx, nx, nt.ac_h0, w + nt.b1 + grp * nt.ac_h0, H1, nullptr};
+      else if (l == 1)
+        L = OaLayer{H1, nt.ac_h0, w + nt.w2 + (int64_t)grp * nt.ac_h1 * nt.ac_h0, nt.ac_h0, nt.ac_h0, nt.ac_h1,
+                    w + nt.b2 + grp * nt.ac_h1, XP, nullptr};
+      else
+        L = OaLayer{XP, nt.ac_h1, w + nt.w3 + (int64_t)grp * nt.ac_h2 * nt.ac_h1, nt.ac_h1, nt.ac_h1, nt.ac_h2,
+                    w + nt.b3 + grp * nt.ac_h2, nullptr, H3};
+      if (!((a.vec >> (3 + l)) & 1u)) oa_layer<0>(L);
+      else if (L.Kw == L.K) oa_layer<2>(L);
+      else oa_layer<1>(L);
+      __syncthreads();
+      FA_PROF(5 + l)
+    }
+    const int64_t so = (int64_t)a.store_row * a.n;
+    if (grp == 0) {
+      for (int e = t; e < NA * HEAD_W; e += OA_THREADS) HW[e] = w[nt.w4a + e];
+      __syncthreads();
+      for (int e = t; e < OA_R * NA; e += OA_THREADS) {
+        const int r = e & (OA_R - 1), j = e / OA_R;
+        float s = 0.f;
+        for (int k = 0; k < HEAD_W; ++k) s = fmaf(H3[r * OA_H3P + k], HW[j * HEAD_W + k], s);
+        MU[r * 16 + j] = s + w[nt.b4a + j];
+      }
+      __syncthreads();
+      FA_PROF(8)
+      for (int i = t; i < nrows * NA; i += OA_THREADS) {
+        const int r = i / NA, j = i - r * NA, g = r0 + r;
+        const float m = MU[r * 16 + j], sd = w[nt.std_off + j];
+        float act;
+        MU[r * 16 + j] = act_draw(a.eps, a.row_offset, a.seed, a.counter, g, j, NA, m, sd, act);
+        a.actions[(int64_t)g * NA + j] = act;
+        if (a.mu) a.mu[(int64_t)g * NA + j] = m;
+        if (a.do_store) {
+          const int64_t o = (so + g) * NA + j;
+          a.store.actions[o] = act;
+          a.store.mu[o] = m;
+          a.store.sigma[o] = sd;
+        }
+      }
+      __syncthreads();
+      if (t < nrows) {
+        const int g = r0 + t;
+        float lp = 0.f;
+        for (int j = 0; j < NA; ++j) lp += MU[t * 16 + j];
+        if (a.logp) a.logp[g] = lp;
+        if (a.do_store) a.store.logp[so + g] = lp;
+      }
+    } else {
+      for (int e = t; e < HEAD_W; e += OA_THREADS) HW[e] = w[nt.w4c + e];
+      __syncthreads();
+      for (int e = t; e < OA_R * 16; e += OA_THREADS) {
+        const int r = e & (OA_R - 1), q = e / OA_R;
+        float s = 0.f;
+        for (int k = q * (HEAD_W / 16); k < (q + 1) * (HEAD_W / 16); ++k) s = fmaf(H3[r * OA_H3P + k], HW[k], s);
+        VP[r * 16 + q] = s;
+      }
+      __syncthreads();
+      FA_PROF(8)
+      if (t < nrows) {
+        const int g = r0 + t;
+        float vs[16];
+#pragma unroll
+        for (int q = 0; q < 16; ++q) vs[q] = VP[t * 16 + q];
+#pragma unroll
+        for (int wd = 8; wd >= 1; wd /= 2)
+#pragma unroll
+          for (int q = 0; q < wd; ++q) vs[q] = vs[2 * q] + vs[2 * q + 1];
+        const float v = vs[0] + w[nt.b4c];
+        if (a.values) a.values[g] = v;
+        if (a.do_store) a.store.values[so + g] = v;
+      }
+    }
+    FA_PROF(9)
     if (a.do_store) {
-      a.store.values[so + g] = v;
-      a.store.logp[so + g] = lp;
-    }
-  }
-  FA_PROF(8)
-  if (a.do_store) {
-    const int64_t b = so + r0;
-    copy_rows(a.obs + (int64_t)r0 * no, no, a.store.obs + b * no, no, nrows, no, t);
-    copy_rows(a.priv + (int64_t)r0 * np, np, a.store.priv + b * np, np, nrows, np, t);
-    if (a.hist && a.store.hist) {
-      const int hd = a.store.hist_dim, ld = a.store.hist_ld > hd ? a.store.hist_ld : hd;
-      copy_rows(a.hist + (int64_t)r0 * hd, hd, a.store.hist + b * ld, ld, nrows, hd, t);
-    }
-  }
-  FA_PROF(9)
+      const int64_t b = so + r0;
+      if (grp == 0) copy_rows<OA_THREADS>(a.obs + (int64_t)r0 * no, no, a.store.obs + b * no, no, nrows, no, t);
+      else copy_rows<OA_THREADS>(a.priv + (int64_t)r0 * np, np, a.store.priv + b * np, np, nrows, np, t);
+      if (a.hist && a.store.hist) {
+        const int hd = a.store.hist_dim, ld = a.store.hist_ld > hd ? a.store.hist_ld : hd;
+        const int h0 = grp * (OA_R / 2), hn = min(nrows, h0 + OA_R / 2) - h0;
+        if (hn > 0) copy_rows<OA_THREADS>(a.hist + (int64_t)(r0 + h0) * hd, hd, a.store.hist + (b + h0) * ld, ld, hn, hd, t);
+      }
+    }
+    FA_PROF(10)
+  }
 }
 
 struct AdaptHeadArgs {
@@ -1412,27 +1606,28 @@
 }
 
 static bool fused_envelope(const lrl_ppo_net& n, bool body) {
-  auto run_ok = [](int groups, int Ng) {
+  auto run_ok = [](int Ng) {
     if (Ng % 16) return false;
-    const int T = groups * (Ng / 16), tpg = Ng / 16;
-    const int tpw = T >= 4 ? T / 4 : 1;
-    if (T >= 4 && T % 4) return false;
-    return tpg % std::min(tpw, 8) == 0;
+    const int T = Ng / 16;
+    return T < 4 || T % 4 == 0;
   };
   if (!(xs_of(n) % 32 == 0 && xs_of(n) <= 256 && n.num_priv <= 32 && n.enc_h0 <= 256 && n.enc_h0 % 32 == 0 &&
-        n.enc_h1 % 32 == 0 && n.enc_h1 + 4 <= (body ? FA_MIDP : FA_ENC_MIDP) && n.latent <= 32 && run_ok(1, n.enc_h0) &&
-        run_ok(1, n.enc_h1) && run_ok(1, (n.latent + 15) / 16 * 16)))
+        n.enc_h1 % 32 == 0 && n.enc_h1 + 4 <= FA_ENC_MIDP && n.latent <= 32 && run_ok(n.enc_h0) && run_ok(n.enc_h1)))
     return false;
-  return !body || (n.ac_h0 % 32 == 0 && n.ac_h1 % 32 == 0 && 2 * n.ac_h0 <= 1024 && 2 * n.ac_h1 <= 512 &&
-                   2 * n.ac_h2 <= 256 && run_ok(1, 2 * n.ac_h0) && run_ok(2, n.ac_h1) && run_ok(2, n.ac_h2));
+  auto run8_ok = [](int Ng) { return Ng / 16 < 8 || (Ng / 16) % 8 == 0; };
+  return !body || (run8_ok(n.enc_h0) && run8_ok(n.enc_h1) && xs_of(n) <= OA_MAX_XS && n.num_obs + n.latent >= 4 && n.ac_h0 % 32 == 0 && n.ac_h0 <= OA_MAX_H0 &&
+                   n.ac_h1 % 32 == 0 && n.ac_h1 <= OA_MAX_H1 && n.ac_h2 == HEAD_W && n.num_actions == HEAD_NA);
 }
 static bool act_enc_fused(const lrl_ppo_net& n) {
   const char* e = getenv("LRL_ACT_ENC_FUSED");
   return !(e && e[0] == '0') && fused_envelope(n, false);
 }
-static bool fused_act_fits(const lrl_ppo_net& n) {
+constexpr int ACT_FUSED_MIN_ROWS = 2048, ACT_FUSED_MAX_ROWS = 4096;
+static bool fused_act_fits(const lrl_ppo_net& n, int rows) {
   const char* e = getenv("LRL_ACT_FUSED");
-  return e && e[0] == '1' && fused_envelope(n, true);
+  if (e && e[0] == '0') return false;
+  if (rows < X6_MIN_M || !gemm_x6_enabled() || !fused_envelope(n, true)) return false;
+  return (e && e[0] == '1') || (rows >= ACT_FUSED_MIN_ROWS && rows <= ACT_FUSED_MAX_ROWS);
 }
 static void launch_act_fused(FusedActArgs& fa, bool body, hipStream_t st) {
   const lrl_ppo_net& n = fa.net;
@@ -1440,14 +1635,18 @@
   fa.vec = (al(n.e2w, n.enc_h0) ? 2u : 0u) | (al(n.e3w, n.enc_h1) ? 4u : 0u);
   if (body)
     fa.vec |= (al(n.w1, n.num_obs + n.latent) ? 8u : 0u) | (al(n.w2, n.ac_h0) ? 16u : 0u) | (al(n.w3, n.ac_h1) ? 32u : 0u);
-  const bool preset = n.enc_h0 == 256 && n.enc_h1 == 128 && n.latent <= 32 &&
-                      (body ? n.ac_h0 == 512 && n.ac_h1 == 256 && n.ac_h2 == 128 && fa.vec == 62u : fa.vec == 6u);
-  const dim3 grid((fa.n + FA_R - 1) / FA_R), block(FA_THREADS);
-  const size_t lds = (body ? FA_LDS_FLOATS : FA_ENC_LDS_FLOATS) * sizeof(float);
-  if (body && preset) hipLaunchKernelGGL(act_fused_kernel<true>, grid, block, lds, st, fa);
-  else if (body) hipLaunchKernelGGL(act_fused_kernel<false>, grid, block, lds, st, fa);
-  else if (preset) hipLaunchKernelGGL((act_fused_kernel<true, true>), grid, block, lds, st, fa);
-  else hipLaunchKernelGGL((act_fused_kernel<false, true>), grid, block, lds, st, fa);
+  const bool preset = n.enc_h0 == 256 && n.enc_h1 == 128 && n.latent <= 32 && (fa.vec & 6u) == 6u;
+  const dim3 block(body ? OA_THREADS : FA_THREADS);
+  if (body) {
+    const dim3 grid(2 * ((fa.n + OA_R - 1) / OA_R));
+    if (preset) hipLaunchKernelGGL(act_fused_kernel<true>, grid, block, OA_LDS_BYTES, st, fa);
+    else hipLaunchKernelGGL(act_fused_kernel<false>, grid, block, OA_LDS_BYTES, st, fa);
+  } else {
+    const dim3 grid((fa.n + FA_R - 1) / FA_R);
+    const size_t lds = FA_ENC_LDS_FLOATS * sizeof(float);
+    if (preset) hipLaunchKernelGGL((act_fused_kernel<true, true>), grid, block, lds, st, fa);
+    else hipLaunchKernelGGL((act_fused_kernel<false, true>), grid, block, lds, st, fa);
+  }
 }
 
 extern "C" int64_t lrl_ppo_act_workspace_bytes(const lrl_ppo_net* net, int32_t n) {
@@ -1491,11 +1690,10 @@
     a.store_row = store_row; a.do_store = store ? 1 : 0;
   };
   const bool full = !nt.plain;
-  if (full && fused_act_fits(nt)) {
+  if (full && fused_act_fits(nt, n)) {
     static const bool ok = [] {
       auto set = [](const void* f) {
-        return hipFuncSetAttribute(f, hipFuncAttributeMaxDynamicSharedMemorySize, FA_LDS_FLOATS * sizeof(float)) ==
-               hipSuccess;
+        return hipFuncSetAttribute(f, hipFuncAttributeMaxDynamicSharedMemorySize, OA_LDS_BYTES) == hipSuccess;
       };
       return set(reinterpret_cast<const void*>(act_fused_kernel<true>)) &&
              set(reinterpret_cast<const void*>(act_fused_kernel<false>));
```
